# andi611/ZeroSpeech-TTS-without-T

Hardware: AMD Instinct MI355X
Metric: mel-frames/sec (train_ae, seg_len=128, enc_size=1024) (higher is better)
Workload: dtype bf16; 1 GPU; train_ae english hps seg_len=128 enc_size=1024 emb_size=1024 n_speakers=102 F=513, batch=256/GPU, dropout+Gumbel on, fwd+bwd+clip+Adam; global_batch=256, parallelism=dp1

## Files before the change

include/zs_amd.h:

```cpp
#ifndef ZS_AMD_H
#define ZS_AMD_H
#include <stddef.h>
#include <stdint.h>

#ifdef __cplusplus
extern "C" {
#endif

#define ZS_ABI_VERSION 1

enum { ZS_F32 = 0, ZS_BF16 = 1 };
enum { ZS_OK = 0, ZS_EINVAL = -1, ZS_ELAUNCH = -2, ZS_EWORKSPACE = -3 };
enum { ZS_PAD_ZERO = 0, ZS_PAD_REFLECT = 1 };
enum { ZS_ACT_NONE = 0, ZS_ACT_LRELU = 1, ZS_ACT_SIGMOID = 2, ZS_ACT_TANH = 3 };
enum { ZS_STORE_ROWS = 0, ZS_STORE_SPLIT2 = 1 };
enum { ZS_RES_NONE = 0, ZS_RES_IDENTITY = 1, ZS_RES_AVGPOOL2 = 2, ZS_RES_UPSAMPLE2 = 3 };

int zs_abi_version(void);
const char* zs_last_error(void);
int zs_set_option(const char* key, int value);
int zs_get_option(const char* key);

typedef struct {
  int32_t dtype;
  const void* A; int64_t lda; int64_t a_batch_stride;
  int32_t B, T_in, T_out;
  int32_t taps, stride, pad_left, pad_mode, gather;
  int32_t cin_pad;
  const void* W; int64_t ldw;
  int32_t N, n_pad;
  const float* bias;
  const float* pre_vec; int64_t pre_vec_ld; const int64_t* vec_idx;
  int32_t act; float slope;
  const void* dact_src; int64_t dact_ld;
  const void* add_src; int64_t add_ld; int32_t add_f32;
  void* out; int64_t ldc; int32_t out_f32; int32_t out_cols; int32_t store_mode;
  void* out2; int64_t ldc2; int32_t out2_cols; int32_t store_mode2;
  const float* vec2; int64_t vec2_ld;
  int32_t groups; int64_t a_gstride, w_gstride, out_gstride, bias_gstride;
  float* colsum; int64_t colsum_ld; int32_t colsum_col0;
  int32_t colsum_post;
  const int32_t* lengths; int32_t pad_right;
  int32_t w_in, w_out, taps_h;
} ZsGemmConv;
int zs_gemm_conv(const ZsGemmConv* p, void* stream);
enum { ZS_GEMM_PATH_P8 = 0, ZS_GEMM_PATH_RING_PP = 1, ZS_GEMM_PATH_RING = 2, ZS_GEMM_PATH_DMA64 = 3, ZS_GEMM_PATH_DMA128 = 4,
       ZS_GEMM_PATH_REG = 5 };
int zs_gemm_conv_path(const ZsGemmConv* p);

typedef struct {
  int32_t dtype;
  const void* dY; int64_t ldy; int32_t y_cols;
  const void* X; int64_t ldx; int64_t x_batch_stride; int32_t x_cols;
  int32_t B, T_in, T_out;
  int32_t taps, stride, pad_left, pad_mode;
  int32_t Cout, Cin;
  float* dW; int64_t so, si, sj;
  float* db;
  int32_t co_split2; int32_t accumulate;
  int32_t splits;
  void* workspace; size_t workspace_bytes;
  int32_t w_in, w_out, taps_h;
} ZsGemmWgrad;
size_t zs_gemm_wgrad_workspace_bytes(const ZsGemmWgrad* p);
int zs_gemm_wgrad(const ZsGemmWgrad* p, void* stream);
enum { ZS_WGRAD_PATH_P8 = 0, ZS_WGRAD_PATH_DMA = 1, ZS_WGRAD_PATH_REG = 2 };
int zs_gemm_wgrad_path(const ZsGemmWgrad* p, int32_t* splits, int32_t* rows_per_split);

typedef struct {
  int32_t dtype;
  const float* W; int64_t so, si, sj;
  int32_t Cout, Cin, taps;
  int32_t transpose, co_split2;
  int32_t inner_pad;
  void* dst; int64_t ldw;
  int32_t n_rows, n_cols, row_offset, col_offset;
  const int32_t* row_perm;
} ZsPackWeight;
int zs_pack_weight(const ZsPackWeight* p, void* stream);
int zs_pack_weight_batch(const ZsPackWeight* jobs, int32_t n, int32_t max_blocks, void* stream);

typedef struct {
  const float* src; float* dst;
  int32_t len, src_stride, dst_stride;
} ZsVecCopy;
int zs_copy_vec_batch(const ZsVecCopy* jobs, int32_t n, void* stream);

typedef struct {
  int32_t dtype;
  const void* src; int64_t ld_src; int32_t src_f32;
  void* dst; int64_t ld_dst; int32_t dst_f32; int32_t col_off;
  int64_t rows; int32_t cols, fill_cols;
  int32_t act; float slope;
  void* dst2; int64_t ld_dst2; int32_t col_off2, fill_cols2; int32_t act2; float slope2;
} ZsCastRows;
int zs_cast_rows(const ZsCastRows* p, void* stream);

typedef struct {
  int32_t dtype;
  const void* x; int64_t ldx;
  const float* vec; int64_t vec_ld; const int64_t* idx;
  void* out; int64_t ldo; int32_t B, T, C, fill_cols;
} ZsAddRowvec;
int zs_add_rowvec(const ZsAddRowvec* p, void* stream);

typedef struct {
  int32_t dtype;
  const void* x; int64_t ldx;
  void* out; int64_t ldo;
  void* out2; int64_t ldo2; const float* vec2; int64_t vec2_ld; int32_t vec2_cols; const int64_t* idx;
  float* mean; float* rstd;
  int32_t B, T, C; float eps;
  float drop_p; uint64_t seed; uint32_t stream_id; const uint8_t* mask; int64_t mask_ld;
  int32_t res_mode; const void* res; int64_t ldres; int32_t T_res; int32_t res_pad_mode;
  const uint64_t* seed_ptr;
  const int32_t* lengths; const int32_t* res_lengths;
  int32_t stats_given;
} ZsInstNormFwd;
int zs_instnorm_fwd(const ZsInstNormFwd* p, void* stream);

typedef struct {
  int32_t dtype;
  const void* dout; int64_t ldd;
  const void* x; int64_t ldx;
  const float* mean; const float* rstd;
  void* dz; int64_t ldz;
  int32_t B, T, C;
  float drop_p; uint64_t seed; uint32_t stream_id; const uint8_t* mask; int64_t mask_ld;
  float slope;
  const uint64_t* seed_ptr;
} ZsInstNormBwd;
int zs_instnorm_bwd(const ZsInstNormBwd* p, void* stream);

typedef struct {
  int32_t dtype;
  const void* gp; int64_t ldg; int32_t pad_left, pad_right, pad_mode;
  int32_t B, T, C;
  float* emb_sum; int64_t emb_ld; int32_t emb_cols;
  int32_t res_mode; const void* res; int64_t ldres;
  const void* dact_src; int64_t dact_ld; float slope;
  void* out; int64_t ldo; int32_t unshuffle;
} ZsGradCombine;
int zs_grad_combine(const ZsGradCombine* p, void* stream);
int zs_norm_decomposition(int32_t kernel, int32_t dtype, int32_t T, int32_t C);

typedef struct {
  const float* emb_sum; int64_t emb_ld; const int64_t* idx; int32_t B;
  float* demb; int64_t demb_ld; int32_t n_rows, C; int32_t accumulate;
} ZsEmbScatter;
int zs_emb_scatter(const ZsEmbScatter* p, void* stream);

typedef struct {
  int32_t dtype;
  const void* logits; int64_t ld; int32_t logits_f32;
  const float* noise; int32_t noise_kind; uint64_t seed;
  int64_t rows; int32_t E; float tau;
  void* bits; int64_t ld_bits; int32_t bits_fill_cols;
  float* bits_f32;
  float* y0;
  const uint64_t* seed_ptr;
} ZsMbvFwd;
int zs_mbv_fwd(const ZsMbvFwd* p, void* stream);
typedef struct {
  int32_t dtype;
  const void* dbits; int64_t ld_dbits;
  const float* y0; int64_t rows; int32_t E; float tau;
  void* dlogits; int64_t ld; int32_t fill_cols;
} ZsMbvBwd;
int zs_mbv_bwd(const ZsMbvBwd* p, void* stream);

enum { ZS_ENC_ONE_HOT = 0, ZS_ENC_BINARY = 1, ZS_ENC_CONTINUES = 2 };
typedef struct {
  int32_t dtype; int32_t mode;
  const void* logits; int64_t ld; int32_t logits_f32;
  const float* noise; int32_t noise_kind; uint64_t seed;
  int64_t rows; int32_t E; float tau; float slope;
  void* bits; int64_t ld_bits; int32_t bits_fill_cols;
  float* bits_f32;
  float* y;
  float* s;
  const uint64_t* seed_ptr;
} ZsGumbelStFwd;
int zs_gumbel_st_fwd(const ZsGumbelStFwd* p, void* stream);
typedef struct {
  int32_t dtype; int32_t mode;
  const void* dbits; int64_t ld_dbits;
  const float* y; int64_t ld_y;
  const float* s;
  int64_t rows; int32_t E; float tau; float slope;
  void* dlogits; int64_t ld; int32_t fill_cols;
} ZsGumbelStBwd;
int zs_gumbel_st_bwd(const ZsGumbelStBwd* p, void* stream);

typedef struct {
  int32_t dtype;
  int32_t B, T, H;
  const void* gi; int64_t ldgi;
  const void* whh; int64_t ldw; int32_t n_pad; int64_t w_gstride;
  const float* bhh; int64_t bhh_gstride;
  void* out; int64_t ldo; int32_t out_col;
  void* gates;
  float* work; size_t work_bytes;
  int32_t whh_interleaved;
  uint32_t* status;
  const float* bcast_vec; int64_t bcast_ld; const int64_t* bcast_idx; int32_t bcast_col;
  int32_t dir1_forward;
} ZsGruFwd;
size_t zs_gru_work_bytes(int32_t B, int32_t H);
int zs_gru_fwd(const ZsGruFwd* p, void* stream);
int zs_gru_check(const float* work, int32_t B, int32_t H, void* stream);

typedef struct {
  int32_t dtype;
  void* x; int64_t ld; int32_t col0, cols;
  int32_t B, T; const int32_t* lengths;
} ZsRowsReverse;
int zs_rows_reverse(const ZsRowsReverse* p, void* stream);
typedef struct {
  int32_t dtype;
  int32_t B, T, H;
  const void* dout; int64_t ldd; int32_t dout_col;
  const void* out; int64_t ldo; int32_t out_col;
  const void* gates;
  const void* whh_t; int64_t ldw; int32_t n_pad; int64_t w_gstride;
  void* dgi; int64_t ldgi;
  void* dgh; int64_t ldgh;
  float* work; size_t work_bytes;
  uint32_t* status;
} ZsGruBwd;
int zs_gru_bwd(const ZsGruBwd* p, void* stream);
enum { ZS_GRU_PATH_WIDE = 0, ZS_GRU_PATH_PERSIST = 1, ZS_GRU_PATH_STEP_FUSED = 2, ZS_GRU_PATH_STEP_GEMM = 3 };
int zs_gru_path(int32_t pass, int32_t dtype, int32_t B, int32_t T, int32_t H, int32_t whh_interleaved, int32_t wide_aligned);

typedef struct {
  int32_t dtype;
  const float* x_dec; int64_t ld_dec;
  const float* x; int64_t ldx;
  int64_t rows; int32_t F;
  void* dlogits; int64_t ldg; int32_t fill_cols;
  float* partial; float* loss_out; float grad_scale;
} ZsL1Loss;
int zs_l1_loss(const ZsL1Loss* p, void* stream);

int zs_sqnorm(const float* g, int64_t n, double* partial, float* out_sq, void* stream);

typedef struct {
  float* p; float* g; float* m; float* v; int64_t n;
  float lr, beta1, beta2, eps, bc1, bc2;
  const float* sumsq; float max_norm; int32_t write_clipped_grad;
  const int32_t* step_ptr;
  float grad_scale;
  int32_t max_blocks;
  float* ema;
  float ema_decay;
} ZsAdam;
int zs_adam_clip(const ZsAdam* p, void* stream);

int zs_sqnorm_stage1(const float* g, int64_t n, double* partial, void* stream);

enum { ZS_APJ_WEIGHT = 0, ZS_APJ_VECTOR = 1, ZS_APJ_RANGE = 2 };
typedef struct {
  void* dst; int64_t ldw; int64_t dst_elems;
  int32_t transpose, inner_pad, row_offset, col_offset, parity;
  int32_t vlen, src_offset, src_stride;
  const int32_t* row_inv;
} ZsAdamPackView;
typedef struct {
  int32_t kind, dtype;
  int64_t off, len;
  int32_t Cout, Cin, taps, co_split2;
  int32_t n_views, tile_start;
  ZsAdamPackView view[2];
} ZsAdamPackJob;
int zs_adam_pack_tiles(const ZsAdamPackJob* job);
int zs_adam_pack(const ZsAdam* a, const ZsAdamPackJob* jobs, const ZsAdamPackJob* jobs_dev, int32_t n, const double* sq_partial,
                 int32_t n_partial, void* stream);

int zs_host_fetch(const void* src, void* dst, size_t bytes, int32_t workgroups, void* stream);

typedef struct {
  const float* pool; const int32_t* speaker; const int64_t* first;
  int64_t* cursor;
  int64_t n; int32_t B, seg_len, F, rank, world;
  float* x; int64_t* c;
  int32_t advance;
} ZsPoolGather;
int zs_pool_gather(const ZsPoolGather* p, void* stream);

int zs_step_counters(uint64_t* seed, int32_t* step, void* stream);

typedef struct {
  const float* logits; int64_t ld; const int64_t* target; int32_t B, n_class;
  float* loss_out; float* dlogits; int64_t ldg; float grad_scale; int32_t* correct_out;
} ZsSoftmaxCE;
// ... 222 lines not shown
```

zerospeech-tts-without-t_amd/csrc/zs_gemm.hip:

```cpp
#include <stdlib.h>

#include <atomic>
#include <mutex>

#include "zs_common.h"

namespace {

constexpr int BM = 128, BN = 128, NT = 256;
constexpr int ROWB = 128;
constexpr int PITCH = 144;
constexpr int TILE_BYTES = BM * PITCH;

__device__ const uint4 zs_zero_line[8] = {};

__device__ __forceinline__ int xcd_remap(int bid, int nwg) {
  const int q = nwg >> 3, r = nwg & 7, xcd = bid & 7;
  return (xcd < r ? xcd * (q + 1) : r * (q + 1) + (xcd - r) * q) + (bid >> 3);
}

__device__ __forceinline__ int conv_src_row(int gather, int pad_mode, int stride, int pad_left, int T_in, int t,
                                            int j, bool& ok) {
  if (gather == 0) {
    int s = t * stride + j - pad_left;
    if (pad_mode == ZS_PAD_REFLECT) s = zs_reflect(s, T_in);
    ok = (s >= 0) && (s < T_in);
    return s;
  }
  int s = t - j;
  ok = false;
  if (s < 0) return 0;
  int q = s / stride;
  ok = (q * stride == s) && (q < T_in);
  return q;
}

struct Geom2 { int w_in, w_out, taps_h, h_in; unsigned mw, mt; };
__device__ __forceinline__ Geom2 make_geom2(int w_in, int w_out, int taps_h, int T_in) {
  Geom2 g;
  g.w_in = w_in; g.w_out = w_out; g.taps_h = taps_h;
  g.h_in = w_in > 0 ? T_in / w_in : 0;
  g.mw = w_in > 0 ? 0xffffffffu / (unsigned)w_out + 1u : 0u;
  g.mt = w_in > 0 ? 0xffffffffu / (unsigned)taps_h + 1u : 0u;
  return g;
}
__device__ __forceinline__ int conv_src_row_g(int gather, int pad_mode, int stride, int pad_left, int T_in, int t, int j, bool& ok,
                                              const Geom2& g) {
  if (g.w_in == 0) return conv_src_row(gather, pad_mode, stride, pad_left, T_in, t, j, ok);
  const int ho = g.w_out == 1 ? t : (int)__umulhi((unsigned)t, g.mw), wo = t - ho * g.w_out;
  const int kw = g.taps_h == 1 ? j : (int)__umulhi((unsigned)j, g.mt), kh = j - kw * g.taps_h;
  bool ok_h, ok_w;
  const int h = conv_src_row(gather, pad_mode, stride, pad_left, g.h_in, ho, kh, ok_h);
  const int w = conv_src_row(gather, pad_mode, stride, pad_left, g.w_in, wo, kw, ok_w);
  ok = ok_h && ok_w;
  return h * g.w_in + w;
}

__device__ __forceinline__ void conv_row_setup(const ZsGemmConv& p, int m, int M, int& rb, int& rt) {
  if (m >= M) { rb = -1; rt = 0; return; }
  const int b = m / p.T_out;
  rt = m - b * p.T_out;
  rb = b;
  if (p.lengths) {
    const int len = p.lengths[b];
    const int len_out = (len + p.pad_left + p.pad_right - p.taps) / p.stride + 1;
    rb = (rt < len_out) ? ((len << 16) | b) : -1;
  }
}
__device__ __forceinline__ int conv_row_b(const ZsGemmConv& p, int rb) { return p.lengths ? (rb & 0xffff) : rb; }
__device__ __forceinline__ int conv_row_tin(const ZsGemmConv& p, int rb) { return p.lengths ? (rb >> 16) : p.T_in; }

template <typename T> struct Mma;
template <> struct Mma<bf16_t> {
  static __device__ __forceinline__ void run(const uint4& a, const uint4& b, f32x16& c) {
    c = __builtin_amdgcn_mfma_f32_32x32x16_bf16(__builtin_bit_cast(bf16x8, a), __builtin_bit_cast(bf16x8, b), c, 0, 0, 0);
  }
};
template <> struct Mma<float> {
  static __device__ __forceinline__ void run(const uint4& a, const uint4& b, f32x16& c) {
    c = __builtin_amdgcn_mfma_f32_32x32x2f32(__uint_as_float(a.x), __uint_as_float(b.x), c, 0, 0, 0);
    c = __builtin_amdgcn_mfma_f32_32x32x2f32(__uint_as_float(a.y), __uint_as_float(b.y), c, 0, 0, 0);
    c = __builtin_amdgcn_mfma_f32_32x32x2f32(__uint_as_float(a.z), __uint_as_float(b.z), c, 0, 0, 0);
    c = __builtin_amdgcn_mfma_f32_32x32x2f32(__uint_as_float(a.w), __uint_as_float(b.w), c, 0, 0, 0);
  }
};

constexpr int CPITCH = 132;
constexpr int EPI_LDS_BYTES = BM * CPITCH * 4;

template <typename T, typename OT>
__device__ __forceinline__ void store_group(OT* base, int64_t row, int64_t ld, int col, int limit, bool aligned,
                                            const float (&v)[8]) {
  OT* d = base + row * ld + col;
  if (aligned && col + 8 <= limit) {
    store8<OT>(d, v);
  } else {
#pragma unroll
    for (int j = 0; j < 8; ++j)
      if (col + j < limit) Elem<OT>::st(d + j, v[j]);
  }
}

template <typename T, int NTHREADS, int ROWS = NTHREADS / 2>
__device__ __forceinline__ void epilogue_finish(const ZsGemmConv& p, const float* sC, int M, int m0, int n0, int tid, int g);

template <int NTHREADS, int ROWS = NTHREADS / 2>
__device__ __forceinline__ void epilogue_colsum(const ZsGemmConv& p, const float* sC, int M, int m0, int n0, int tid) {
  if (p.colsum == nullptr) return;
  const int ns = ROWS / p.T_out;
  for (int w = tid; w < ns * 128; w += NTHREADS) {
    const int col = w & 127, r0 = (w >> 7) * p.T_out;
    const int n = n0 + col, m = m0 + r0;
    if (n >= p.N || n < p.colsum_col0 || m >= M) continue;
    const float* q = sC + r0 * CPITCH + col;
    float a0 = 0.f, a1 = 0.f, a2 = 0.f, a3 = 0.f;
    int r = 0;
    if (p.colsum_post && (p.dact_src || p.add_src)) {
      for (; r < p.T_out; ++r) {
        float v = q[r * CPITCH];
        const int64_t mm = (int64_t)m + r;
        if (p.dact_src) v *= dlrelu_f(p.dtype == ZS_F32 ? ((const float*)p.dact_src)[mm * p.dact_ld + n] : bf2f(((const bf16_t*)p.dact_src)[mm * p.dact_ld + n]), p.slope);
        if (p.add_src) v += (p.add_f32 || p.dtype == ZS_F32) ? ((const float*)p.add_src)[mm * p.add_ld + n] : bf2f(((const bf16_t*)p.add_src)[mm * p.add_ld + n]);
        a0 += v;
      }
    }
    for (; r + 4 <= p.T_out; r += 4) {
      a0 += q[(r + 0) * CPITCH]; a1 += q[(r + 1) * CPITCH]; a2 += q[(r + 2) * CPITCH]; a3 += q[(r + 3) * CPITCH];
    }
    for (; r < p.T_out; ++r) a0 += q[r * CPITCH];
    p.colsum[(int64_t)(m / p.T_out) * p.colsum_ld + (n - p.colsum_col0)] += (a0 + a1) + (a2 + a3);
  }
}

template <typename T, int NTHREADS, int MI = 2>
__device__ __forceinline__ void gemm_epilogue(const ZsGemmConv& p, f32x16 (&acc)[MI][2], float* sC, int M, int m0, int n0,
                                              int wm, int wn, int tid, int g) {
  constexpr int ROWS = (NTHREADS / 2) * MI / 2;
  const int lane = tid & 63;
#pragma unroll
  for (int mi = 0; mi < MI; ++mi)
#pragma unroll
    for (int ni = 0; ni < 2; ++ni)
#pragma unroll
      for (int r = 0; r < 16; ++r) {
        const int row = wm * (32 * MI) + mi * 32 + (r & 3) + 8 * (r >> 2) + 4 * (lane >> 5);
        const int col = wn * 64 + ni * 32 + (lane & 31);
        sC[row * CPITCH + col] = acc[mi][ni][r];
      }
  __syncthreads();
  epilogue_colsum<NTHREADS, ROWS>(p, sC, M, m0, n0, tid);
  epilogue_finish<T, NTHREADS, ROWS>(p, sC, M, m0, n0, tid, g);
}

template <typename T, int NTHREADS, int ROWS>
__device__ __forceinline__ void epilogue_finish(const ZsGemmConv& p, const float* sC, int M, int m0, int n0, int tid, int g) {
  constexpr int ROWS_PER_PASS = NTHREADS / 16;
  constexpr int PASSES = ROWS / ROWS_PER_PASS;
  const int cg = tid & 15, rr0 = tid >> 4;
  const int n = n0 + cg * 8;
  if (n >= p.N && n >= p.out_cols && n >= p.out2_cols) return;
  const int half = p.N >> 1;
  const bool need_b = (p.pre_vec != nullptr) || (p.vec2 != nullptr);
  const int es = (int)sizeof(T);
  const bool al_out = p.out && ((((uintptr_t)p.out) | (uintptr_t)(p.ldc * (p.out_f32 ? 4 : es)) | (uintptr_t)(p.out_gstride * (p.out_f32 ? 4 : es))) & 15) == 0;
  const bool al_out2 = p.out2 && ((((uintptr_t)p.out2) | (uintptr_t)(p.ldc2 * es)) & 15) == 0;
  const bool al_dact = p.dact_src && ((((uintptr_t)p.dact_src) | (uintptr_t)(p.dact_ld * es)) & 15) == 0;
  const bool al_add = p.add_src && ((((uintptr_t)p.add_src) | (uintptr_t)(p.add_ld * (p.add_f32 ? 4 : es))) & 15) == 0;
  const bool split_ok = (half & 7) == 0;
  float bias[8];
#pragma unroll
  for (int j = 0; j < 8; ++j) bias[j] = (p.bias != nullptr && n + j < p.N) ? p.bias[(int64_t)g * p.bias_gstride + n + j] : 0.f;
  float* outf = (float*)p.out + (p.out_f32 ? (int64_t)g * p.out_gstride : 0);
  T* outt = (T*)p.out + (p.out_f32 ? 0 : (int64_t)g * p.out_gstride);

#pragma unroll 2
  for (int it = 0; it < PASSES; ++it) {
    const int row = rr0 + ROWS_PER_PASS * it;
    const int m = m0 + row;
    if (m >= M) break;
    float v[8];
    {
      const float4 x0 = *reinterpret_cast<const float4*>(sC + row * CPITCH + cg * 8);
      const float4 x1 = *reinterpret_cast<const float4*>(sC + row * CPITCH + cg * 8 + 4);
      v[0] = x0.x; v[1] = x0.y; v[2] = x0.z; v[3] = x0.w; v[4] = x1.x; v[5] = x1.y; v[6] = x1.z; v[7] = x1.w;
    }
    int b = 0;
    if (need_b) b = m / p.T_out;
#pragma unroll
    for (int j = 0; j < 8; ++j) v[j] += bias[j];
    if (p.pre_vec) {
      const float* pv = p.pre_vec + p.vec_idx[b] * p.pre_vec_ld + n;
#pragma unroll
      for (int j = 0; j < 8; ++j) if (n + j < p.N) v[j] += pv[j];
    }
    if (p.act == ZS_ACT_LRELU) {
#pragma unroll
      for (int j = 0; j < 8; ++j) v[j] = lrelu_f(v[j], p.slope);
    } else if (p.act == ZS_ACT_SIGMOID) {
#pragma unroll
      for (int j = 0; j < 8; ++j) v[j] = 1.f / (1.f + expf(-v[j]));
    } else if (p.act == ZS_ACT_TANH) {
#pragma unroll
      for (int j = 0; j < 8; ++j) v[j] = tanhf(v[j]);
    }
    if (p.dact_src) {
      const T* dp = (const T*)p.dact_src + (int64_t)m * p.dact_ld + n;
      float y[8];
      if (al_dact && n + 8 <= p.N) load8<T>(dp, y);
      else {
#pragma unroll
        for (int j = 0; j < 8; ++j) y[j] = (n + j < p.N) ? Elem<T>::ld(dp + j) : 0.f;
      }
#pragma unroll
      for (int j = 0; j < 8; ++j) v[j] *= dlrelu_f(y[j], p.slope);
    }
    if (p.add_src) {
      float y[8];
      if (p.add_f32) {
        const float* ap = (const float*)p.add_src + (int64_t)m * p.add_ld + n;
        if (al_add && n + 8 <= p.N) load8<float>(ap, y);
        else {
#pragma unroll
          for (int j = 0; j < 8; ++j) y[j] = (n + j < p.N) ? ap[j] : 0.f;
        }
      } else {
        const T* ap = (const T*)p.add_src + (int64_t)m * p.add_ld + n;
        if (al_add && n + 8 <= p.N) load8<T>(ap, y);
        else {
#pragma unroll
          for (int j = 0; j < 8; ++j) y[j] = (n + j < p.N) ? Elem<T>::ld(ap + j) : 0.f;
        }
      }
#pragma unroll
      for (int j = 0; j < 8; ++j) v[j] += y[j];
    }
#pragma unroll
    for (int j = 0; j < 8; ++j) if (n + j >= p.N) v[j] = 0.f;

    if (p.out) {
      if (p.store_mode == ZS_STORE_SPLIT2) {
        if (split_ok) {
          const int hi = n >= half;
          if (p.out_f32) store_group<T, float>(outf, 2 * (int64_t)m + hi, p.ldc, n - hi * half, half, al_out, v);
          else store_group<T, T>(outt, 2 * (int64_t)m + hi, p.ldc, n - hi * half, half, al_out, v);
        } else {
#pragma unroll
          for (int j = 0; j < 8; ++j)
            if (n + j < p.N) {
              const int hi = (n + j) >= half;
              const int64_t o = (2 * (int64_t)m + hi) * p.ldc + (n + j - hi * half);
              if (p.out_f32) outf[o] = v[j]; else Elem<T>::st(outt + o, v[j]);
            }
        }
      } else {
        if (p.out_f32) store_group<T, float>(outf, m, p.ldc, n, p.out_cols, al_out, v);
        else store_group<T, T>(outt, m, p.ldc, n, p.out_cols, al_out, v);
      }
    }
    if (p.out2) {
      const bool sp = p.store_mode2 == ZS_STORE_SPLIT2;
      if (sp && !split_ok) {
#pragma unroll
        for (int j = 0; j < 8; ++j)
          if (n + j < p.N) {
            const int hi = (n + j) >= half;
            const int oc = n + j - hi * half;
            float w = v[j];
            if (p.vec2) w += p.vec2[p.vec_idx[b] * p.vec2_ld + oc];
            Elem<T>::st((T*)p.out2 + (2 * (int64_t)m + hi) * p.ldc2 + oc, w);
          }
      } else {
        const int hi = sp ? (n >= half) : 0;
        const int oc = n - hi * half;
        const int64_t orow = sp ? (2 * (int64_t)m + hi) : (int64_t)m;
        const int limit = sp ? half : p.out2_cols;
        float w[8];
#pragma unroll
        for (int j = 0; j < 8; ++j) w[j] = v[j];
        if (p.vec2) {
          const float* pv = p.vec2 + p.vec_idx[b] * p.vec2_ld + oc;
#pragma unroll
          for (int j = 0; j < 8; ++j) if (n + j < p.N) w[j] += pv[j];
        }
        store_group<T, T>((T*)p.out2, orow, p.ldc2, oc, limit, al_out2, w);
      }
    }
  }
}

template <typename T>
__global__ __launch_bounds__(NT, 2) void gemm_conv_kernel(const ZsGemmConv p) {
  const Geom2 g2 = make_geom2(p.w_in, p.w_out, p.taps_h, p.T_in);
  constexpr int EPS = 16 / (int)sizeof(T);
  constexpr int KC = ROWB / (int)sizeof(T);
  extern __shared__ __attribute__((aligned(16))) unsigned char smem[];
  unsigned char* sA = smem;
  unsigned char* sB = smem + 2 * TILE_BYTES;

  const int tid = threadIdx.x, lane = tid & 63, wave = tid >> 6;
  const int wm = wave >> 1, wn = wave & 1;
  const int g = blockIdx.z;
  const T* __restrict__ A = (const T*)p.A + (int64_t)g * p.a_gstride;
  const T* __restrict__ W = (const T*)p.W + (int64_t)g * p.w_gstride;
  const int M = p.B * p.T_out;
  const int ntn = (p.N + BN - 1) / BN;
  const int ntm = (M + BM - 1) / BM;
  const int wg = xcd_remap(blockIdx.x, ntm * ntn);
  constexpr int GM = 8;
  const int per_group = GM * ntn;
  const int grp = wg / per_group;
  const int gm = min(GM, ntm - grp * GM);
  const int in_g = wg - grp * per_group;
  const int m0 = (grp * GM + in_g % gm) * BM, n0 = (in_g / gm) * BN;

  const int seg = tid & 7, r0 = tid >> 3;
  int rb[4], rt[4];
#pragma unroll
  for (int i = 0; i < 4; ++i) {
    int m = m0 + r0 + 32 * i;
    conv_row_setup(p, m, M, rb[i], rt[i]);
  }
  const int chunks_per_tap = p.cin_pad / KC;
  const T* zline = reinterpret_cast<const T*>(zs_zero_line) + seg * EPS;
  const T *pa0, *pa1, *pa2, *pa3;
  int inc0, inc1, inc2, inc3;
#define ZS_SET_TAP(i, ptr, inc)                                                                         \
  {                                                                                                     \
    bool ok = false; int srow = 0;                                                                      \
    if (rb[i] >= 0) srow = conv_src_row_g(p.gather, p.pad_mode, p.stride, p.pad_left, conv_row_tin(p, rb[i]), rt[i], tap, ok, g2); \
    ptr = ok ? (A + (int64_t)conv_row_b(p, rb[i]) * p.a_batch_stride + (int64_t)srow * p.lda + seg * EPS) : zline;       \
    inc = ok ? KC : 0;                                                                                  \
  }
  const T* pw0 = W + (int64_t)(n0 + r0) * p.ldw + seg * EPS;
  const int64_t wstep = (int64_t)32 * p.ldw;

  const int nk = p.taps * chunks_per_tap;
  uint4 Pa0, Pa1, Pa2, Pa3, Pb0, Pb1, Pb2, Pb3, Qa0, Qa1, Qa2, Qa3, Qb0, Qb1, Qb2, Qb3;
  int tap = 0, cit = 0;
  { ZS_SET_TAP(0, pa0, inc0) ZS_SET_TAP(1, pa1, inc1) ZS_SET_TAP(2, pa2, inc2) ZS_SET_TAP(3, pa3, inc3) }
  auto advance = [&]() {
    pw0 += KC;
    if (++cit == chunks_per_tap) {
      cit = 0; ++tap;
      if (tap < p.taps) { ZS_SET_TAP(0, pa0, inc0) ZS_SET_TAP(1, pa1, inc1) ZS_SET_TAP(2, pa2, inc2) ZS_SET_TAP(3, pa3, inc3) }
    } else {
      pa0 += inc0; pa1 += inc1; pa2 += inc2; pa3 += inc3;
    }
  };
#define ZS_GLOAD(S)                                                                                      \
  S##a0 = *reinterpret_cast<const uint4*>(pa0); S##a1 = *reinterpret_cast<const uint4*>(pa1);            \
  S##a2 = *reinterpret_cast<const uint4*>(pa2); S##a3 = *reinterpret_cast<const uint4*>(pa3);            \
  S##b0 = *reinterpret_cast<const uint4*>(pw0); S##b1 = *reinterpret_cast<const uint4*>(pw0 + wstep);    \
  S##b2 = *reinterpret_cast<const uint4*>(pw0 + 2 * wstep); S##b3 = *reinterpret_cast<const uint4*>(pw0 + 3 * wstep); \
  advance();
#define ZS_SWRITE(S, buf)                                                                                \
  {                                                                                                      \
// ... 287 lines not shown
      const int fly = (grp1 ? min(nk, 3) : min(nk, 2)) - 1;
      if (fly == 2) asm volatile("s_waitcnt vmcnt(12)" ::: "memory");
      else if (fly == 1) asm volatile("s_waitcnt vmcnt(6)" ::: "memory");
      else asm volatile("s_waitcnt vmcnt(0)" ::: "memory");
    }
    __builtin_amdgcn_s_barrier();
    if (grp1) __builtin_amdgcn_s_barrier();
    int stage = 0;
    for (int kt = 0; kt < nk; ++kt) {
      const unsigned sa = a_lane + (unsigned)(stage * RSTAGE), sb = b_lane + (unsigned)(stage * RSTAGE);
      u32x4_t fa[4][2], fb[4][2];
#pragma unroll
      for (int ks = 0; ks < 4; ++ks) {
        asm volatile("ds_read_b128 %0, %1" : "=v"(fa[ks][0]) : "v"(sa + koff[ks]));
        asm volatile("ds_read_b128 %0, %1 offset:4096" : "=v"(fa[ks][1]) : "v"(sa + koff[ks]));
        asm volatile("ds_read_b128 %0, %1" : "=v"(fb[ks][0]) : "v"(sb + koff[ks]));
        asm volatile("ds_read_b128 %0, %1 offset:4096" : "=v"(fb[ks][1]) : "v"(sb + koff[ks]));
      }
      int s2 = stage + 2; if (s2 >= 3) s2 -= 3;
      if (!grp1 && kt + 2 < nk) dma(s2);
      asm volatile("s_waitcnt lgkmcnt(0)" ::: "memory");
      if (grp1) {
        if (kt + 2 < nk) asm volatile("s_waitcnt vmcnt(6)" ::: "memory");
        else asm volatile("s_waitcnt vmcnt(0)" ::: "memory");
      }
      __builtin_amdgcn_s_barrier();
      __builtin_amdgcn_sched_barrier(0);
      const bool more1 = grp1 && (kt + 3 < nk);
      __builtin_amdgcn_s_setprio(1);
#pragma unroll
      for (int ks = 0; ks < 4; ++ks) {
#pragma unroll
        for (int mi = 0; mi < 2; ++mi)
#pragma unroll
          for (int ni = 0; ni < 2; ++ni) {
            const uint4 ua = make_uint4(fa[ks][mi].x, fa[ks][mi].y, fa[ks][mi].z, fa[ks][mi].w);
            const uint4 ub = make_uint4(fb[ks][ni].x, fb[ks][ni].y, fb[ks][ni].z, fb[ks][ni].w);
            Mma<T>::run(ua, ub, acc[mi][ni]);
          }
        if (more1 && ks < 3) {
          __builtin_amdgcn_sched_barrier(0);
          dma_piece(stage, 2 * ks);
          dma_piece(stage, 2 * ks + 1);
          __builtin_amdgcn_sched_barrier(0);
        }
      }
      __builtin_amdgcn_s_setprio(0);
      if (more1) dma_advance();
      if (!grp1) {
        if (kt + 2 < nk) asm volatile("s_waitcnt vmcnt(6)" ::: "memory");
        else asm volatile("s_waitcnt vmcnt(0)" ::: "memory");
      }
      __builtin_amdgcn_s_barrier();
      __builtin_amdgcn_sched_barrier(0);
      if (++stage == 3) stage = 0;
    }
    if (!grp1) __builtin_amdgcn_s_barrier();
  } else {
  dma(0);
  if (nk > 1) dma(1);
  int stage = 0;
  for (int kt = 0; kt < nk; ++kt) {
    if (kt + 1 < nk) asm volatile("s_waitcnt vmcnt(6)" ::: "memory");
    else asm volatile("s_waitcnt vmcnt(0)" ::: "memory");
    __builtin_amdgcn_s_barrier();
    const unsigned sa = a_lane + (unsigned)(stage * RSTAGE), sb = b_lane + (unsigned)(stage * RSTAGE);
    u32x4_t fa[4][2], fb[4][2];
#pragma unroll
    for (int ks = 0; ks < 4; ++ks) {
      asm volatile("ds_read_b128 %0, %1" : "=v"(fa[ks][0]) : "v"(sa + koff[ks]));
      asm volatile("ds_read_b128 %0, %1 offset:4096" : "=v"(fa[ks][1]) : "v"(sa + koff[ks]));
      asm volatile("ds_read_b128 %0, %1" : "=v"(fb[ks][0]) : "v"(sb + koff[ks]));
      asm volatile("ds_read_b128 %0, %1 offset:4096" : "=v"(fb[ks][1]) : "v"(sb + koff[ks]));
    }
    const bool more = kt + 2 < nk;
    int s2 = stage + 2; if (s2 >= 3) s2 -= 3;
    asm volatile("s_waitcnt lgkmcnt(0)" ::: "memory");
    __builtin_amdgcn_sched_barrier(0);
#pragma unroll
    for (int ks = 0; ks < 4; ++ks) {
#pragma unroll
      for (int mi = 0; mi < 2; ++mi)
#pragma unroll
        for (int ni = 0; ni < 2; ++ni) {
          const uint4 ua = make_uint4(fa[ks][mi].x, fa[ks][mi].y, fa[ks][mi].z, fa[ks][mi].w);
          const uint4 ub = make_uint4(fb[ks][ni].x, fb[ks][ni].y, fb[ks][ni].z, fb[ks][ni].w);
          Mma<T>::run(ua, ub, acc[mi][ni]);
        }
      if (more && ks < 3) {
        __builtin_amdgcn_sched_barrier(0);
        dma_piece(s2, 2 * ks);
        dma_piece(s2, 2 * ks + 1);
        __builtin_amdgcn_sched_barrier(0);
      }
    }
    if (more) dma_advance();
    __builtin_amdgcn_sched_barrier(0);
    if (++stage == 3) stage = 0;
  }
  }
  asm volatile("s_waitcnt vmcnt(0)" ::: "memory");
  __syncthreads();
  gemm_epilogue<T, RNT>(p, acc, reinterpret_cast<float*>(smem), M, m0, n0, wm, wn, tid, g);
}

constexpr int PBM = 256, PBN = 256, PNT = 512;
constexpr int PSTAGE = (PBM + PBN) * 128;
constexpr int P8_EPI = 256 * CPITCH * 4;
constexpr int P8_LDS = (2 * PSTAGE > P8_EPI) ? 2 * PSTAGE : P8_EPI;

#define ZS_DSR(dst, addr, off) asm volatile("ds_read_b128 %0, %1 offset:" #off : "=v"(dst) : "v"(addr))
#define ZS_P8_DMA(cond, src, dst)                                                \
  __builtin_amdgcn_sched_barrier(0);                                             \
  if (cond) __builtin_amdgcn_global_load_lds((gptr_t)(src), (lptr_t)(dst), 16, 0, 0); \
  __builtin_amdgcn_sched_barrier(0);
typedef __attribute__((ext_vector_type(4))) float f32x4_m;
template <typename T> struct Mma16;
template <> struct Mma16<bf16_t> {
  static __device__ __forceinline__ void run(const uint4& a, const uint4& b, f32x4_m& c) {
    c = __builtin_amdgcn_mfma_f32_16x16x32_bf16(__builtin_bit_cast(bf16x8, a), __builtin_bit_cast(bf16x8, b), c, 0, 0, 0);
  }
};
template <> struct Mma16<float> {
  static __device__ __forceinline__ void run(const uint4& a, const uint4& b, f32x4_m& c) {
    c = __builtin_amdgcn_mfma_f32_16x16x4f32(__uint_as_float(a.x), __uint_as_float(b.x), c, 0, 0, 0);
    c = __builtin_amdgcn_mfma_f32_16x16x4f32(__uint_as_float(a.y), __uint_as_float(b.y), c, 0, 0, 0);
    c = __builtin_amdgcn_mfma_f32_16x16x4f32(__uint_as_float(a.z), __uint_as_float(b.z), c, 0, 0, 0);
    c = __builtin_amdgcn_mfma_f32_16x16x4f32(__uint_as_float(a.w), __uint_as_float(b.w), c, 0, 0, 0);
  }
};
#define ZS_M16_READ_A(o0, o1, o2, o3)                                            \
  ZS_DSR(fa00, sa + koff0, o0); ZS_DSR(fa01, sa + koff1, o0); ZS_DSR(fa10, sa + koff0, o1); ZS_DSR(fa11, sa + koff1, o1); \
  ZS_DSR(fa20, sa + koff0, o2); ZS_DSR(fa21, sa + koff1, o2); ZS_DSR(fa30, sa + koff0, o3); ZS_DSR(fa31, sa + koff1, o3);
#define ZS_M16_READ_B(f0, f1, f2, f3, o0, o1)                                    \
  ZS_DSR(f0, sb + koff0, o0); ZS_DSR(f1, sb + koff1, o0); ZS_DSR(f2, sb + koff0, o1); ZS_DSR(f3, sb + koff1, o1);
#define ZS_M16_MMA(a, b, cc) Mma16<T>::run(make_uint4(a.x, a.y, a.z, a.w), make_uint4(b.x, b.y, b.z, b.w), cc)
#define ZS_M16_QUAD(cq, b0, b1, b2, b3, cond, src0, dst0, src1, dst1)            \
  __builtin_amdgcn_s_setprio(1);                                                 \
  ZS_M16_MMA(fa00, b0, cq[0][0]); ZS_M16_MMA(fa00, b2, cq[0][1]); ZS_M16_MMA(fa10, b0, cq[1][0]); ZS_M16_MMA(fa10, b2, cq[1][1]); \
  ZS_P8_DMA(cond, src0, dst0)                                                    \
  ZS_M16_MMA(fa20, b0, cq[2][0]); ZS_M16_MMA(fa20, b2, cq[2][1]); ZS_M16_MMA(fa30, b0, cq[3][0]); ZS_M16_MMA(fa30, b2, cq[3][1]); \
  ZS_M16_MMA(fa01, b1, cq[0][0]); ZS_M16_MMA(fa01, b3, cq[0][1]);                \
  ZS_P8_DMA(cond, src1, dst1)                                                    \
  ZS_M16_MMA(fa11, b1, cq[1][0]); ZS_M16_MMA(fa11, b3, cq[1][1]); ZS_M16_MMA(fa21, b1, cq[2][0]); ZS_M16_MMA(fa21, b3, cq[2][1]); \
  ZS_M16_MMA(fa31, b1, cq[3][0]); ZS_M16_MMA(fa31, b3, cq[3][1]);                \
  __builtin_amdgcn_s_setprio(0);

__host__ __device__ __forceinline__ bool al16(const void* q, int64_t pitch_bytes) { return ((((uintptr_t)q) | (uintptr_t)pitch_bytes) & 15) == 0; }

__host__ __device__ __forceinline__ bool p8_regs_epilogue_ok(const ZsGemmConv& p) {
  const int half = p.N >> 1;
  const bool split = (p.out && p.store_mode == ZS_STORE_SPLIT2) || (p.out2 && p.store_mode2 == ZS_STORE_SPLIT2);
  return (p.out == nullptr || (!p.out_f32 && al16(p.out, p.ldc * 2) && ((p.out_gstride * 2) & 15) == 0 && (p.out_cols & 7) == 0)) &&
         (p.out2 == nullptr || (al16(p.out2, p.ldc2 * 2) && (p.out2_cols & 7) == 0 && p.dact_src == nullptr && p.add_src == nullptr)) &&
         (p.dact_src == nullptr || al16(p.dact_src, p.dact_ld * 2)) &&
         (p.add_src == nullptr || (!p.add_f32 && al16(p.add_src, p.add_ld * 2))) &&
         ((p.pre_vec == nullptr && p.vec2 == nullptr) || (p.T_out & 15) == 0) && (!split || (half & 7) == 0) &&
         (p.act == ZS_ACT_NONE || p.act == ZS_ACT_LRELU) &&
         (p.colsum == nullptr || ((PBM % p.T_out) == 0 && p.out2 == nullptr));
}

template <bool HAS2>
__device__ __forceinline__ void p8_regs_epilogue(const ZsGemmConv& p, f32x4_m (&c)[2][2][4][2], unsigned char* smem, int M, int m0, int n0,
                                                 int tid, int lane, int wr, int wc, int g) {
  constexpr int PT = 264;
  unsigned short* sT = reinterpret_cast<unsigned short*>(smem);
  const int colb = wc * 64 + (lane & 15);
  const int rbase = wr * 128 + 4 * (lane >> 4);
  const int half = p.N >> 1;
  int64_t bsel[2][4];
  const bool need_b = p.pre_vec != nullptr || p.vec2 != nullptr;
#pragma unroll
  for (int mq = 0; mq < 2; ++mq)
#pragma unroll
    for (int mt = 0; mt < 4; ++mt) {
      const int mb = m0 + wr * 128 + mq * 64 + mt * 16;
      bsel[mq][mt] = (need_b && mb < M) ? p.vec_idx[mb / p.T_out] : 0;
    }
#pragma unroll
  for (int nq = 0; nq < 2; ++nq)
#pragma unroll
    for (int nt = 0; nt < 2; ++nt) {
      const int col = colb + nq * 32 + nt * 16;
      const int n = n0 + col;
      const bool cval = n < p.N;
      const float bv = (p.bias != nullptr && cval) ? p.bias[(int64_t)g * p.bias_gstride + n] : 0.f;
      float pv[2][4];
#pragma unroll
      for (int mq = 0; mq < 2; ++mq)
#pragma unroll
        for (int mt = 0; mt < 4; ++mt) pv[mq][mt] = bv;
      if (p.pre_vec != nullptr && cval) {
#pragma unroll
        for (int mq = 0; mq < 2; ++mq)
#pragma unroll
          for (int mt = 0; mt < 4; ++mt) pv[mq][mt] += p.pre_vec[bsel[mq][mt] * p.pre_vec_ld + n];
      }
#pragma unroll
      for (int mq = 0; mq < 2; ++mq)
#pragma unroll
        for (int mt = 0; mt < 4; ++mt)
#pragma unroll
          for (int i4 = 0; i4 < 4; ++i4) {
            float v = c[mq][nq][mt][nt][i4] + pv[mq][mt];
            if (p.act == ZS_ACT_LRELU) v = lrelu_f(v, p.slope);
            if (!cval) v = 0.f;
            if constexpr (HAS2) c[mq][nq][mt][nt][i4] = v;
            sT[(rbase + mq * 64 + mt * 16 + i4) * PT + col] = f2bf(v);
          }
    }
  __syncthreads();

  const bool cs_post = !HAS2 && p.colsum != nullptr && p.colsum_post && (p.dact_src != nullptr || p.add_src != nullptr);
  auto colsum_pass = [&]() {
    const int ns = PBM / p.T_out;
    const int col = tid & 255, n = n0 + col, hs = tid >> 8;
    const int s0 = ns >= 2 ? hs * (ns >> 1) : 0, s1 = ns >= 2 ? s0 + (ns >> 1) : (hs == 0 ? 1 : 0);
    if (n < p.N && n >= p.colsum_col0) {
      for (int s = s0; s < s1; ++s) {
        const int r0 = s * p.T_out, m = m0 + r0;
        if (m >= M) break;
        float a0 = 0.f, a1 = 0.f, a2 = 0.f, a3 = 0.f;
        const unsigned short* q = sT + r0 * PT + col;
        int r = 0;
        for (; r + 4 <= p.T_out; r += 4) {
          a0 += bf2f(q[(r + 0) * PT]); a1 += bf2f(q[(r + 1) * PT]); a2 += bf2f(q[(r + 2) * PT]); a3 += bf2f(q[(r + 3) * PT]);
        }
        for (; r < p.T_out; ++r) a0 += bf2f(q[r * PT]);
        float* d = p.colsum + (int64_t)(m / p.T_out) * p.colsum_ld + (n - p.colsum_col0);
        *d += (a0 + a1) + (a2 + a3);
      }
    }
  };
  if (!HAS2 && p.colsum != nullptr && !cs_post) colsum_pass();

  const int c8 = (tid & 31) * 8, r0 = tid >> 5;
  const int n = n0 + c8;
  if (p.out != nullptr) {
    unsigned short* outp = (unsigned short*)p.out + (int64_t)g * p.out_gstride;
    const bool sp = p.store_mode == ZS_STORE_SPLIT2;
    const int hi = sp ? (n >= half) : 0;
    const int oc = n - hi * half;
    const bool cok = sp ? (n < p.N) : (n < p.out_cols);
    const bool second = p.dact_src != nullptr || p.add_src != nullptr;
    if (cok && !second) {
#pragma unroll 8
      for (int it = 0; it < 16; ++it) {
        const int row = r0 + 16 * it;
        const int m = m0 + row;
        if (m < M) {
          const uint4 w = *reinterpret_cast<const uint4*>(sT + row * PT + c8);
          const int64_t orow = sp ? 2 * (int64_t)m + hi : (int64_t)m;
          *reinterpret_cast<uint4*>(outp + orow * p.ldc + oc) = w;
        }
      }
    } else if (!HAS2 && cok) {
      const bf16_t* dsrc = (const bf16_t*)p.dact_src;
      const bf16_t* asrc = (const bf16_t*)p.add_src;
      const bool tail = n + 8 > p.N;
#pragma unroll 1
      for (int it0 = 0; it0 < 16; it0 += 8) {
        Raw8<bf16_t> rd[8], ra[8];
        uint4 w[8];
#pragma unroll
        for (int u = 0; u < 8; ++u) {
          const int row = r0 + 16 * (it0 + u);
          const int m = min(m0 + row, M - 1);
          if (dsrc) rd[u].ld(dsrc + (int64_t)m * p.dact_ld + n);
          if (asrc) ra[u].ld(asrc + (int64_t)m * p.add_ld + n);
          w[u] = *reinterpret_cast<const uint4*>(sT + row * PT + c8);
        }
#pragma unroll
        for (int u = 0; u < 8; ++u) {
          const int row = r0 + 16 * (it0 + u);
          const int m = m0 + row;
          if (m < M) {
            float v[8], y[8];
            Raw8<bf16_t> rw; rw.a = w[u]; rw.cvt(v);
            if (dsrc) {
              rd[u].cvt(y);
#pragma unroll
              for (int j = 0; j < 8; ++j) v[j] *= dlrelu_f(y[j], p.slope);
            }
            if (asrc) {
              ra[u].cvt(y);
#pragma unroll
              for (int j = 0; j < 8; ++j) v[j] += y[j];
            }
            if (tail) {
#pragma unroll
              for (int j = 0; j < 8; ++j) if (n + j >= p.N) v[j] = 0.f;
            }
            const int64_t orow = sp ? 2 * (int64_t)m + hi : (int64_t)m;
            store8<bf16_t>(outp + orow * p.ldc + oc, v);
            if (cs_post) store8<bf16_t>(sT + row * PT + c8, v);
          }
        }
      }
    }
  }
  if (cs_post) {
    __syncthreads();
    colsum_pass();
  }
  if constexpr (HAS2) {
    __syncthreads();
    const bool sp = p.store_mode2 == ZS_STORE_SPLIT2;
#pragma unroll
    for (int nq = 0; nq < 2; ++nq)
#pragma unroll
      for (int nt = 0; nt < 2; ++nt) {
        const int col = colb + nq * 32 + nt * 16;
        const int nn = n0 + col;
        const bool cval = nn < p.N;
        const int ocv = sp ? (nn >= half ? nn - half : nn) : nn;
        float ev[2][4];
#pragma unroll
        for (int mq = 0; mq < 2; ++mq)
#pragma unroll
          for (int mt = 0; mt < 4; ++mt) ev[mq][mt] = 0.f;
        if (p.vec2 != nullptr && cval) {
#pragma unroll
          for (int mq = 0; mq < 2; ++mq)
#pragma unroll
            for (int mt = 0; mt < 4; ++mt) ev[mq][mt] = p.vec2[bsel[mq][mt] * p.vec2_ld + ocv];
        }
#pragma unroll
        for (int mq = 0; mq < 2; ++mq)
#pragma unroll
          for (int mt = 0; mt < 4; ++mt)
#pragma unroll
            for (int i4 = 0; i4 < 4; ++i4)
              sT[(rbase + mq * 64 + mt * 16 + i4) * PT + col] = f2bf(c[mq][nq][mt][nt][i4] + ev[mq][mt]);
      }
    __syncthreads();
    unsigned short* outp = (unsigned short*)p.out2;
    const int hi = sp ? (n >= half) : 0;
    const int oc = n - hi * half;
    const bool cok = sp ? (n < p.N) : (n < p.out2_cols);
    if (cok) {
#pragma unroll 8
      for (int it = 0; it < 16; ++it) {
        const int row = r0 + 16 * it;
        const int m = m0 + row;
        if (m < M) {
          const uint4 w = *reinterpret_cast<const uint4*>(sT + row * PT + c8);
          const int64_t orow = sp ? 2 * (int64_t)m + hi : (int64_t)m;
          *reinterpret_cast<uint4*>(outp + orow * p.ldc2 + oc) = w;
        }
      }
    }
  }
}

template <typename T>
__global__ __launch_bounds__(PNT, 2) void gemm_conv_p8m16_kernel(const ZsGemmConv p) {
  const Geom2 g2 = make_geom2(p.w_in, p.w_out, p.taps_h, p.T_in);
  constexpr int EPS = 16 / (int)sizeof(T);
  constexpr int KC = ROWB / (int)sizeof(T);
  extern __shared__ __attribute__((aligned(16))) unsigned char smem[];
  typedef __attribute__((address_space(1))) const void* gptr_t;
  typedef __attribute__((address_space(3))) void* lptr_t;
  const int tid = threadIdx.x, lane = tid & 63, wave = __builtin_amdgcn_readfirstlane(tid >> 6);
  const int wr = wave >> 2, wc = wave & 3;
  const int g = blockIdx.z;
  const T* __restrict__ A = (const T*)p.A + (int64_t)g * p.a_gstride;
  const T* __restrict__ W = (const T*)p.W + (int64_t)g * p.w_gstride;
  const int M = p.B * p.T_out;
  const int ntn = (p.N + PBN - 1) / PBN;
  const int ntm = (M + PBM - 1) / PBM;
  const int wg = xcd_remap(blockIdx.x, ntm * ntn);
  constexpr int GM = 4;
  const int per_group = GM * ntn;
  const int grp = wg / per_group;
  const int gm = min(GM, ntm - grp * GM);
  const int in_g = wg - grp * per_group;
  const int m0 = (grp * GM + in_g % gm) * PBM, n0 = (in_g / gm) * PBN;

  const int lrow = lane >> 3, slot = lane & 7;
  int rb[4], rt[4], lseg[4];
#pragma unroll
  for (int j = 0; j < 4; ++j) {
    const int r = (j >> 1) * 128 + wave * 16 + (j & 1) * 8 + lrow;
    lseg[j] = slot ^ ((r >> 1) & 7);
    const int m = m0 + r;
    conv_row_setup(p, m, M, rb[j], rt[j]);
  }
  const int chunks_per_tap = p.cin_pad / KC;
  const T* zline = reinterpret_cast<const T*>(zs_zero_line);
  const T *pa0, *pa1, *pa2, *pa3;
  int inc0, inc1, inc2, inc3;
#define ZS_SET_TAP(i, ptr, inc)                                                                         \
  {                                                                                                     \
    bool ok = false; int srow = 0;                                                                      \
    if (rb[i] >= 0) srow = conv_src_row_g(p.gather, p.pad_mode, p.stride, p.pad_left, conv_row_tin(p, rb[i]), rt[i], tap, ok, g2); \
    ptr = ok ? (A + (int64_t)conv_row_b(p, rb[i]) * p.a_batch_stride + (int64_t)srow * p.lda + lseg[i] * EPS) : (zline + lseg[i] * EPS); \
    inc = ok ? KC : 0;                                                                                  \
  }
  const int nk = p.taps * chunks_per_tap;
  int tap = 0, cit = 0;
  { ZS_SET_TAP(0, pa0, inc0) ZS_SET_TAP(1, pa1, inc1) ZS_SET_TAP(2, pa2, inc2) ZS_SET_TAP(3, pa3, inc3) }
  auto advance_a = [&]() {
    if (++cit == chunks_per_tap) {
      cit = 0; ++tap;
      if (tap < p.taps) { ZS_SET_TAP(0, pa0, inc0) ZS_SET_TAP(1, pa1, inc1) ZS_SET_TAP(2, pa2, inc2) ZS_SET_TAP(3, pa3, inc3) }
    } else {
      pa0 += inc0; pa1 += inc1; pa2 += inc2; pa3 += inc3;
    }
  };
#undef ZS_SET_TAP
  const T* pw0 = W + (int64_t)(n0 + wave * 16 + lrow) * p.ldw + lseg[0] * EPS;
  const T* pw1 = W + (int64_t)(n0 + wave * 16 + 8 + lrow) * p.ldw + lseg[1] * EPS;
  const int64_t whalf = (int64_t)128 * p.ldw;

  unsigned char* const ldsA = smem + wave * 2048;
  unsigned char* const ldsB = smem + 32768 + wave * 2048;

  f32x4_m c[2][2][4][2];
#pragma unroll
  for (int i0 = 0; i0 < 2; ++i0)
#pragma unroll
    for (int i1 = 0; i1 < 2; ++i1)
#pragma unroll
      for (int i2 = 0; i2 < 4; ++i2)
#pragma unroll
        for (int i3 = 0; i3 < 2; ++i3) c[i0][i1][i2][i3] = f32x4_m{0.f, 0.f, 0.f, 0.f};

  const int frow = lane & 15, fh = lane >> 4, fx = (frow >> 1) & 7;
  const unsigned lds0 = (unsigned)(uintptr_t)(__attribute__((address_space(3))) unsigned char*)smem;
  const unsigned a_lane = lds0 + (unsigned)((wr * 128 + frow) * 128);
  const unsigned b_lane = lds0 + (unsigned)(32768 + (wc * 64 + frow) * 128);
  const unsigned koff0 = (unsigned)(((0 + fh) ^ fx) * 16), koff1 = (unsigned)(((4 + fh) ^ fx) * 16);
  const int grp1 = wr;

  __builtin_amdgcn_global_load_lds((gptr_t)pa0, (lptr_t)(ldsA), 16, 0, 0);
  __builtin_amdgcn_global_load_lds((gptr_t)pa1, (lptr_t)(ldsA + 1024), 16, 0, 0);
  __builtin_amdgcn_global_load_lds((gptr_t)pa2, (lptr_t)(ldsA + 16384), 16, 0, 0);
  __builtin_amdgcn_global_load_lds((gptr_t)pa3, (lptr_t)(ldsA + 16384 + 1024), 16, 0, 0);
  advance_a();
  __builtin_amdgcn_global_load_lds((gptr_t)pw0, (lptr_t)(ldsB), 16, 0, 0);
  __builtin_amdgcn_global_load_lds((gptr_t)pw1, (lptr_t)(ldsB + 1024), 16, 0, 0);
  __builtin_amdgcn_global_load_lds((gptr_t)(pw0 + whalf), (lptr_t)(ldsB + 16384), 16, 0, 0);
  __builtin_amdgcn_global_load_lds((gptr_t)(pw1 + whalf), (lptr_t)(ldsB + 16384 + 1024), 16, 0, 0);
  pw0 += KC; pw1 += KC;
  if (nk > 1) {
    __builtin_amdgcn_global_load_lds((gptr_t)pw0, (lptr_t)(ldsB + PSTAGE), 16, 0, 0);
    __builtin_amdgcn_global_load_lds((gptr_t)pw1, (lptr_t)(ldsB + PSTAGE + 1024), 16, 0, 0);
    __builtin_amdgcn_global_load_lds((gptr_t)(pw0 + whalf), (lptr_t)(ldsB + PSTAGE + 16384), 16, 0, 0);
    __builtin_amdgcn_global_load_lds((gptr_t)(pw1 + whalf), (lptr_t)(ldsB + PSTAGE + 16384 + 1024), 16, 0, 0);
    pw0 += KC; pw1 += KC;
    asm volatile("s_waitcnt vmcnt(4)" ::: "memory");
  } else {
    asm volatile("s_waitcnt vmcnt(0)" ::: "memory");
  }
  __builtin_amdgcn_s_barrier();
  if (grp1) __builtin_amdgcn_s_barrier();

  u32x4_t fa00, fa01, fa10, fa11, fa20, fa21, fa30, fa31;
  u32x4_t fb00, fb01, fb02, fb03, fb10, fb11, fb12, fb13;
// ... 824 lines not shown
  for (int e = 0; e < 4; ++e) {
    const int ci = c4 * 4 + e;
    if (ci < p.Cin) {
      float* q = d + (int64_t)ci * p.si;
      *q = p.accumulate ? (*q + r[e]) : r[e];
    }
  }
}

constexpr int WRT_LDS_FLOATS = 1024;

__global__ __launch_bounds__(256) void wgrad_reduce_taps_kernel(const ZsGemmWgrad p, int splits, int cout_r, int cin_r, int c4n,
                                                                int nblk, int nmain) {
  __shared__ float sT[WRT_LDS_FLOATS];
  const int64_t sstride = (int64_t)cout_r * p.taps * cin_r;
  if ((int)blockIdx.x >= nmain) { wgrad_reduce_bias(p, splits, cout_r, sstride, (int)blockIdx.x - nmain); return; }
  const int co = (int)blockIdx.x / nblk, blk = (int)blockIdx.x - co * nblk;
  const int ci0 = blk * 4 * c4n;
  const int taps = p.taps;
  const float* wrow = (const float*)p.workspace + (int64_t)wgrad_co_perm(p, co) * taps * cin_r + ci0;
  for (int it = (int)threadIdx.x; it < c4n * taps; it += 256) {
    const int j = it / c4n, c = it - j * c4n;
    if (ci0 + 4 * c >= p.Cin) continue;
    const float4 acc = wgrad_sum_splits(wrow + (int64_t)j * cin_r + 4 * c, splits, sstride);
    sT[(4 * c + 0) * taps + j] = acc.x; sT[(4 * c + 1) * taps + j] = acc.y;
    sT[(4 * c + 2) * taps + j] = acc.z; sT[(4 * c + 3) * taps + j] = acc.w;
  }
  __syncthreads();
  const int n = min(4 * c4n, p.Cin - ci0) * taps;
  float* d = p.dW + (int64_t)co * p.so + (int64_t)ci0 * taps;
  for (int i = (int)threadIdx.x; i < n; i += 256) d[i] = p.accumulate ? (d[i] + sT[i]) : sT[i];
}

Knob g_dma64("gemm_dma64", "ZS_GEMM_DMA64", 1);
Knob g_dma64_max_tiles("gemm_dma64_max_tiles", "ZS_GEMM_DMA64_MAX_TILES", 256);
Knob g_wgrad_p8("wgrad_p8", "ZS_WGRAD_P8", 1);
Knob g_wgrad_wgs("wgrad_wgs", "ZS_WGRAD_WGS", 256);
Knob g_wgrad_wgs128("wgrad_wgs128", "ZS_WGRAD_WGS128", 448);
Knob g_wgrad_slab_cost("wgrad_slab_cost", "ZS_WGRAD_SLAB_COST", 13);
Knob g_wgrad_alone("wgrad_alone", "ZS_WGRAD_ALONE", 0);
Knob g_wgrad_wgs128_alone("wgrad_wgs128_alone", "ZS_WGRAD_WGS128_ALONE", 448);
Knob g_wgrad_slab_cost_alone("wgrad_slab_cost_alone", "ZS_WGRAD_SLAB_COST_ALONE", 13);
Knob g_wgrad_dma("wgrad_dma", "ZS_WGRAD_DMA", 1);
Knob g_wgrad_reduce_taps("wgrad_reduce_taps", "ZS_WGRAD_REDUCE_TAPS", 1);
Knob g_wgrad_waste("wgrad_p8_waste", "ZS_WGRAD_P8_WASTE", 135);

struct WgradPlan { int p8, dma, splits, tile, co_tiles, ci_tiles, cout_r, cin_r, rows_per_split; };

WgradPlan wgrad_plan(const ZsGemmWgrad* p) {
  WgradPlan w;
  const int wgrad_p8 = g_wgrad_p8.get();
  const bool alone = g_wgrad_alone.get() != 0;
  const int64_t M = (int64_t)p->B * p->T_out;
  const int64_t t256 = (int64_t)((p->Cout + 255) / 256) * p->taps * ((p->Cin + 255) / 256);
  const double waste = (double)(((p->Cout + 255) / 256) * 256) * (((p->Cin + 255) / 256) * 256) / ((double)p->Cout * p->Cin);
  w.p8 = wgrad_p8 && p->dtype == ZS_BF16 && waste <= 0.01 * (double)g_wgrad_waste.get() && M >= 2048 && (wgrad_p8 > 1 || t256 * M >= (int64_t)16 * 8192);
  if (wgrad_p8 > 1 && p->dtype == ZS_BF16) w.p8 = 1;
  w.dma = !w.p8 && p->dtype == ZS_BF16 && g_wgrad_dma.get() != 0;
  w.tile = w.p8 ? 256 : 128;
  w.co_tiles = (p->Cout + w.tile - 1) / w.tile; w.ci_tiles = (p->Cin + w.tile - 1) / w.tile;
  w.cout_r = w.co_tiles * w.tile; w.cin_r = w.ci_tiles * w.tile;
  const int64_t tiles = (int64_t)w.co_tiles * p->taps * w.ci_tiles;
  if (p->splits > 0) {
    w.splits = p->splits;
  } else if (w.p8) {
    const int64_t kt = (M + 63) / 64;
    const int wgs_knob = g_wgrad_wgs.get();
    const int64_t wgs = wgs_knob > 0 ? wgs_knob : 256;
    const double slab_cost = (double)(alone ? g_wgrad_slab_cost_alone.get() : g_wgrad_slab_cost.get());
    double best = 1e30; int bs = 1;
    for (int sp = 1; sp <= 64 && (int64_t)sp * 4 <= kt; ++sp) {
      const double rounds = (double)((tiles * sp + wgs - 1) / wgs);
      const double cost = rounds * ((double)((kt + sp - 1) / sp) + slab_cost);
      if (cost < best - 1e-9) { best = cost; bs = sp; }
    }
    w.splits = bs;
  } else {
    const int knob = alone ? g_wgrad_wgs128_alone.get() : g_wgrad_wgs128.get();
    const int64_t target = knob > 0 ? knob : 448;
    int64_t sp = (target + tiles - 1) / tiles;
    int64_t maxs = (M + 255) / 256;
    if (sp > maxs) sp = maxs;
    if (sp > 1024) sp = 1024;
    if (sp < 1) sp = 1;
    w.splits = (int)sp;
  }
  const int gran = w.p8 ? 64 : WK;
  int rps = (int)((M + w.splits - 1) / w.splits);
  w.rows_per_split = ((rps + gran - 1) / gran) * gran;
  return w;
}

bool aligned16(const void* p) { return (((uintptr_t)p) & 15) == 0; }

Knob g_use_dma("gemm_dma", "ZS_GEMM_DMA", 1), g_use_ring("gemm_ring", "ZS_GEMM_RING", 1),
    g_ring_min_tiles("gemm_ring_min_tiles", "ZS_GEMM_RING_MIN_TILES", 256), g_use_pp("gemm_pp", "ZS_GEMM_PP", 1), g_use_p8("gemm_p8", "ZS_GEMM_P8", 1),
    g_p8_min_tiles("gemm_p8_min_tiles", "ZS_GEMM_P8_MIN_TILES", 200);

std::once_flag g_lds_attr_once;
void set_lds_attrs() {
  const void* big[] = {reinterpret_cast<const void*>(gemm_conv_p8m16_kernel<float>), reinterpret_cast<const void*>(gemm_conv_p8m16_kernel<bf16_t>),
                       reinterpret_cast<const void*>(gemm_wgrad_p8_kernel)};
  for (const void* f : big) (void)hipFuncSetAttribute(f, hipFuncAttributeMaxDynamicSharedMemorySize, P8_LDS);
  const void* ring[] = {reinterpret_cast<const void*>(gemm_conv_ring_kernel<float, 0>), reinterpret_cast<const void*>(gemm_conv_ring_kernel<bf16_t, 0>),
                        reinterpret_cast<const void*>(gemm_conv_ring_kernel<float, 1>), reinterpret_cast<const void*>(gemm_conv_ring_kernel<bf16_t, 1>)};
  for (const void* f : ring) (void)hipFuncSetAttribute(f, hipFuncAttributeMaxDynamicSharedMemorySize, RING_LDS);
}

struct ConvPlan {
  int path;
  int regs;
  int64_t wgs;
  int groups;
};
int gemm_conv_plan(const ZsGemmConv* p, ConvPlan& pl) {
  ZS_REQUIRE(p && p->A && p->W && (p->out || p->out2), "zs_gemm_conv: null operand");
  ZS_REQUIRE(p->dtype == ZS_F32 || p->dtype == ZS_BF16, "zs_gemm_conv: bad dtype %d", p->dtype);
  const int es = p->dtype == ZS_F32 ? 4 : 2;
  const int kc = 128 / es;
  ZS_REQUIRE(p->B > 0 && p->T_in > 0 && p->T_out > 0 && p->N > 0 && p->taps > 0 && p->stride > 0, "zs_gemm_conv: bad sizes");
  ZS_REQUIRE(p->cin_pad > 0 && p->cin_pad % kc == 0, "zs_gemm_conv: cin_pad %d must be a multiple of %d (one 128-byte chunk)", p->cin_pad, kc);
  ZS_REQUIRE(p->ldw >= (int64_t)p->taps * p->cin_pad && (p->ldw * es) % 16 == 0, "zs_gemm_conv: ldw %lld < taps*cin_pad",
             (long long)p->ldw);
  ZS_REQUIRE(p->n_pad % 128 == 0 && p->n_pad >= p->N, "zs_gemm_conv: n_pad %d must be a multiple of 128 >= N %d", p->n_pad, p->N);
  ZS_REQUIRE(aligned16(p->A) && aligned16(p->W) && (p->lda * es) % 16 == 0 && (p->a_batch_stride * es) % 16 == 0 &&
                 (p->a_gstride * es) % 16 == 0 && (p->w_gstride * es) % 16 == 0,
             "zs_gemm_conv: operands must be 16-byte aligned (A=%p lda=%lld)", p->A, (long long)p->lda);
  if (p->w_in > 0) {
    ZS_REQUIRE((int64_t)p->T_out * p->w_out < (1ll << 32), "zs_gemm_conv: 2-D image too large (T_out %d x w_out %d)", p->T_out, p->w_out);
    ZS_REQUIRE(p->w_out > 0 && p->taps_h > 0 && p->taps % p->taps_h == 0 && p->T_in % p->w_in == 0 && p->T_out % p->w_out == 0 && !p->lengths,
               "zs_gemm_conv: 2-D geometry (w_in %d, w_out %d, taps_h %d, taps %d, T_in %d, T_out %d)", p->w_in, p->w_out, p->taps_h, p->taps,
               p->T_in, p->T_out);
    if (p->gather == 0 && p->pad_mode == ZS_PAD_REFLECT) {
      const int h_in = p->T_in / p->w_in, h_out = p->T_out / p->w_out, taps_w = p->taps / p->taps_h;
      const int pr_h = (h_out - 1) * p->stride + p->taps_h - 1 - p->pad_left - (h_in - 1);
      const int pr_w = (p->w_out - 1) * p->stride + taps_w - 1 - p->pad_left - (p->w_in - 1);
      ZS_REQUIRE(p->pad_left < h_in && pr_h < h_in && p->pad_left < p->w_in && pr_w < p->w_in,
                 "zs_gemm_conv: Padding size should be less than the corresponding input dimension (2-D: pad %d, H %d, W %d)", p->pad_left, h_in, p->w_in);
    }
  } else if (p->gather == 0 && p->pad_mode == ZS_PAD_REFLECT) {
    const int pad_r = (p->T_out - 1) * p->stride + p->taps - 1 - p->pad_left - (p->T_in - 1);
    ZS_REQUIRE(p->pad_left < p->T_in && pad_r < p->T_in,
               "zs_gemm_conv: Padding size should be less than the corresponding input dimension (pad %d/%d, T %d)",
               p->pad_left, pad_r, p->T_in);
  }
  if (p->store_mode == ZS_STORE_SPLIT2 || (p->out2 && p->store_mode2 == ZS_STORE_SPLIT2))
    ZS_REQUIRE(p->N % 2 == 0, "zs_gemm_conv: SPLIT2 needs even N");
  ZS_REQUIRE(!(p->pre_vec || p->vec2) || p->vec_idx, "zs_gemm_conv: vec_idx missing");
  ZS_REQUIRE(!p->colsum || (128 % p->T_out == 0 && p->colsum_col0 >= 0 && p->colsum_col0 < p->N && !p->bias && !p->pre_vec &&
                            p->act == ZS_ACT_NONE && p->groups <= 1),
             "zs_gemm_conv: colsum needs T_out (%d) to divide 128, 0 <= colsum_col0 < N and no bias / pre_vec / activation / groups", p->T_out);
  ZS_REQUIRE(!p->lengths || (p->gather == 0 && p->B < 65536 && p->T_in < 32768 && p->pad_right >= 0 && p->colsum == nullptr),
             "zs_gemm_conv: lengths (ragged batch) needs gather 0, B < 65536, T_in < 32768, pad_right >= 0 and no colsum");
  pl.groups = p->groups > 0 ? p->groups : 1;
  pl.regs = 0;
  const int64_t M = (int64_t)p->B * p->T_out;
  const int64_t ntn = (p->N + BN - 1) / BN;
  const int64_t tiles = ((M + BM - 1) / BM) * ntn;
  ZS_REQUIRE(tiles < (1ll << 31), "zs_gemm_conv: grid too large");
  const int use_dma = g_use_dma.get(), use_ring = g_use_ring.get(), use_p8 = g_use_p8.get(), use_pp = g_use_pp.get();
  const int64_t ring_tiles = ((M + RBM - 1) / RBM) * ntn;
  const int64_t p8_tiles = ((M + PBM - 1) / PBM) * ((p->N + PBN - 1) / PBN);
  const int64_t tiles64 = ((M + 63) / 64) * ntn;
  if (use_dma && use_p8 && p->n_pad % PBN == 0 && p8_tiles >= g_p8_min_tiles.get() && p8_tiles < (1ll << 31)) {
    pl.path = ZS_GEMM_PATH_P8; pl.wgs = p8_tiles;
    pl.regs = p->dtype == ZS_BF16 && p8_regs_epilogue_ok(*p);
  } else if (use_dma && use_ring && ring_tiles >= g_ring_min_tiles.get() && ring_tiles < (1ll << 31)) {
    pl.path = use_pp ? ZS_GEMM_PATH_RING_PP : ZS_GEMM_PATH_RING; pl.wgs = ring_tiles;
  } else if (use_dma && g_dma64.get() && tiles * 2 <= g_dma64_max_tiles.get() && tiles64 < (1ll << 31) &&
             (p->colsum == nullptr || 64 % p->T_out == 0)) {
    pl.path = ZS_GEMM_PATH_DMA64; pl.wgs = tiles64;
  } else {
    pl.path = use_dma ? ZS_GEMM_PATH_DMA128 : ZS_GEMM_PATH_REG; pl.wgs = tiles;
  }
  return ZS_OK;
}

struct WgradLaunch {
  WgradPlan w;
  int kernel;
  int reduce_taps;
  int64_t wgs;
  int c4n, nblk;
  int nmain, nbias;
};
int gemm_wgrad_plan(const ZsGemmWgrad* p, WgradLaunch& pl) {
  ZS_REQUIRE(p && p->dY && p->X && p->dW && p->workspace, "zs_gemm_wgrad: null operand");
  ZS_REQUIRE(aligned16(p->workspace), "zs_gemm_wgrad: workspace must be 16-byte aligned");
  ZS_REQUIRE(p->dtype == ZS_F32 || p->dtype == ZS_BF16, "zs_gemm_wgrad: bad dtype");
  const int es = p->dtype == ZS_F32 ? 4 : 2;
  ZS_REQUIRE(p->B > 0 && p->T_in > 0 && p->T_out > 0 && p->Cout > 0 && p->Cin > 0 && p->taps > 0 && p->stride > 0,
             "zs_gemm_wgrad: bad sizes");
  ZS_REQUIRE(aligned16(p->dY) && aligned16(p->X) && (p->ldy * es) % 16 == 0 && (p->ldx * es) % 16 == 0 &&
                 (p->x_batch_stride * es) % 16 == 0 && (p->y_cols * es) % 16 == 0 && (p->x_cols * es) % 16 == 0,
             "zs_gemm_wgrad: operands must be 16-byte aligned");
  ZS_REQUIRE(p->y_cols <= p->ldy && p->x_cols <= p->ldx && p->Cout <= p->y_cols && p->Cin <= p->x_cols, "zs_gemm_wgrad: column bounds");
  ZS_REQUIRE(!p->co_split2 || p->Cout % 2 == 0, "zs_gemm_wgrad: SPLIT2 needs even Cout");
  ZS_REQUIRE(p->w_in == 0 || (p->w_in > 0 && p->w_out > 0 && p->taps_h > 0 && p->taps % p->taps_h == 0 && p->T_in % p->w_in == 0 &&
                              p->T_out % p->w_out == 0 && (int64_t)p->T_out * p->w_out < (1ll << 32)),
             "zs_gemm_wgrad: 2-D geometry (w_in %d, w_out %d, taps_h %d, taps %d, T_in %d, T_out %d)", p->w_in, p->w_out, p->taps_h, p->taps,
             p->T_in, p->T_out);
  pl.w = wgrad_plan(p);
  const WgradPlan& w = pl.w;
  pl.kernel = w.p8 ? ZS_WGRAD_PATH_P8 : (w.dma ? ZS_WGRAD_PATH_DMA : ZS_WGRAD_PATH_REG);
  pl.wgs = (int64_t)w.co_tiles * p->taps * w.ci_tiles * w.splits;
  ZS_REQUIRE(pl.wgs < (1ll << 31), "zs_gemm_wgrad: grid too large");
  pl.nbias = p->db ? (p->Cout + 255) / 256 : 0;
  pl.reduce_taps = g_wgrad_reduce_taps.get() && p->taps > 1 && p->taps <= 256 && p->si == p->taps && p->sj == 1;
  pl.c4n = pl.nblk = 0;
  if (pl.reduce_taps) {
    pl.c4n = 256 / p->taps;
    pl.nblk = (p->Cin + 4 * pl.c4n - 1) / (4 * pl.c4n);
    ZS_REQUIRE((int64_t)p->Cout * pl.nblk + pl.nbias < (1ll << 31), "zs_gemm_wgrad: reduce grid too large");
    pl.nmain = p->Cout * pl.nblk;
  } else {
    const int64_t relems = (int64_t)p->Cout * p->taps * ((p->Cin + 3) / 4);
    const int64_t nmain = (relems + 255) / 256;
    ZS_REQUIRE(nmain + pl.nbias < (1ll << 31), "zs_gemm_wgrad: reduce grid too large");
    pl.nmain = (int)nmain;
  }
  return ZS_OK;
}

}

extern "C" int zs_gemm_conv_path(const ZsGemmConv* p) {
  ConvPlan pl;
  const int rc = gemm_conv_plan(p, pl);
  return rc != ZS_OK ? rc : (pl.path | pl.regs << 8);
}

extern "C" int zs_gemm_conv(const ZsGemmConv* p, void* stream) {
  ConvPlan pl;
  const int rc = gemm_conv_plan(p, pl);
  if (rc != ZS_OK) return rc;
  const dim3 grid((unsigned)pl.wgs, 1, (unsigned)pl.groups);
  const bool f32 = p->dtype == ZS_F32;
  hipStream_t s = (hipStream_t)stream;
  std::call_once(g_lds_attr_once, set_lds_attrs);
  switch (pl.path) {
    case ZS_GEMM_PATH_P8:
      if (f32) hipLaunchKernelGGL(gemm_conv_p8m16_kernel<float>, grid, dim3(PNT), P8_LDS, s, *p);
      else hipLaunchKernelGGL(gemm_conv_p8m16_kernel<bf16_t>, grid, dim3(PNT), P8_LDS, s, *p);
      break;
    case ZS_GEMM_PATH_RING_PP:
      if (f32) hipLaunchKernelGGL((gemm_conv_ring_kernel<float, 1>), grid, dim3(RNT), RING_LDS, s, *p);
      else hipLaunchKernelGGL((gemm_conv_ring_kernel<bf16_t, 1>), grid, dim3(RNT), RING_LDS, s, *p);
      break;
    case ZS_GEMM_PATH_RING:
      if (f32) hipLaunchKernelGGL((gemm_conv_ring_kernel<float, 0>), grid, dim3(RNT), RING_LDS, s, *p);
      else hipLaunchKernelGGL((gemm_conv_ring_kernel<bf16_t, 0>), grid, dim3(RNT), RING_LDS, s, *p);
      break;
    case ZS_GEMM_PATH_DMA64: {
      const size_t lds = (2 * 64 * 128 + 2 * DTILE > EPI_LDS_BYTES / 2) ? 2 * 64 * 128 + 2 * DTILE : EPI_LDS_BYTES / 2;
      if (f32) hipLaunchKernelGGL((gemm_conv_dma_kernel<float, 64>), grid, dim3(NT), lds, s, *p);
      else hipLaunchKernelGGL((gemm_conv_dma_kernel<bf16_t, 64>), grid, dim3(NT), lds, s, *p);
      break;
    }
    case ZS_GEMM_PATH_DMA128: {
      const size_t lds = (4 * DTILE > EPI_LDS_BYTES) ? 4 * DTILE : EPI_LDS_BYTES;
      if (f32) hipLaunchKernelGGL((gemm_conv_dma_kernel<float, 128>), grid, dim3(NT), lds, s, *p);
      else hipLaunchKernelGGL((gemm_conv_dma_kernel<bf16_t, 128>), grid, dim3(NT), lds, s, *p);
      break;
    }
    default: {
      const size_t lds = 4 * TILE_BYTES;
      if (f32) hipLaunchKernelGGL(gemm_conv_kernel<float>, grid, dim3(NT), lds, s, *p);
      else hipLaunchKernelGGL(gemm_conv_kernel<bf16_t>, grid, dim3(NT), lds, s, *p);
    }
  }
  return zs_check_launch("zs_gemm_conv");
}

extern "C" size_t zs_gemm_wgrad_workspace_bytes(const ZsGemmWgrad* p) {
  if (!p) return 0;
  const WgradPlan w = wgrad_plan(p);
  return (size_t)w.splits * ((size_t)w.cout_r * p->taps * w.cin_r + w.cout_r) * sizeof(float);
}

extern "C" int zs_gemm_wgrad_path(const ZsGemmWgrad* p, int32_t* splits, int32_t* rows_per_split) {
  WgradLaunch pl;
  const int rc = gemm_wgrad_plan(p, pl);
  if (rc != ZS_OK) return rc;
  if (splits) *splits = pl.w.splits;
  if (rows_per_split) *rows_per_split = pl.w.rows_per_split;
  return pl.kernel | pl.reduce_taps << 8;
}

extern "C" int zs_gemm_wgrad(const ZsGemmWgrad* p, void* stream) {
  WgradLaunch pl;
  int rc = gemm_wgrad_plan(p, pl);
  if (rc != ZS_OK) return rc;
  const WgradPlan& w = pl.w;
  const int splits = w.splits, ci_tiles = w.ci_tiles, cout_r = w.cout_r, cin_r = w.cin_r;
  const int rows_per_split = w.rows_per_split;
  const size_t need = (size_t)splits * ((size_t)cout_r * p->taps * cin_r + cout_r) * sizeof(float);
  if (p->workspace_bytes < need) {
    zs_set_error("zs_gemm_wgrad: workspace %zu < %zu bytes", p->workspace_bytes, need);
    return ZS_EWORKSPACE;
  }
  hipStream_t s = (hipStream_t)stream;
  const dim3 grid((unsigned)pl.wgs, 1, 1);
  std::call_once(g_lds_attr_once, set_lds_attrs);
  if (pl.kernel == ZS_WGRAD_PATH_P8) {
    hipLaunchKernelGGL(gemm_wgrad_p8_kernel, grid, dim3(PNT), P8_LDS, s, *p, ci_tiles, rows_per_split, cout_r, cin_r);
  } else if (p->dtype == ZS_F32) {
// ... 30 lines not shown
```

zerospeech-tts-without-t_amd/csrc/zs_norm.hip:

```cpp
#include <stdlib.h>

#include "zs_common.h"

namespace {

constexpr int RPT = 8;
struct Narrow { static constexpr int NTN = 256, CHUNK = 64, RG = 32; };
struct Wide8 { static constexpr int NTN = 256, CHUNK = 256, RG = 8; };
constexpr int RGN = 32;

template <typename S>
__device__ __forceinline__ void colreduce(const float (&pv)[RGN / S::RG][8], float (&out)[8], float* red, float* tot, int cg, int rg, int tid) {
  constexpr int CHUNK = S::CHUNK, RG = S::RG, NP = RGN / RG;
#pragma unroll
  for (int j = 0; j < NP; ++j)
#pragma unroll
    for (int k = 0; k < 8; ++k) red[(rg + RG * j) * CHUNK + cg * 8 + k] = pv[j][k];
  __syncthreads();
  for (int c = tid; c < CHUNK; c += S::NTN) {
    float s = 0.f;
#pragma unroll 8
    for (int r = 0; r < RGN; ++r) s += red[r * CHUNK + c];
    tot[c] = s;
  }
// ... 141 lines not shown
    }
  }
}

template <typename T, typename S>
__global__ __launch_bounds__(S::NTN) void instnorm_bwd_kernel(const ZsInstNormBwd p) {
  constexpr int CHUNK = S::CHUNK, RG = S::RG, CGN = S::CHUNK / 8, NP = RGN / RG;
  __shared__ float red[RGN * CHUNK];
  __shared__ float tot[CHUNK];
  const int tid = threadIdx.x, cg = tid % CGN, rg = tid / CGN;
  const int b = blockIdx.y, c0 = blockIdx.x * CHUNK + cg * 8;
  const bool cvalid = c0 < p.C;
  float mean[8], rstd[8];
#pragma unroll
  for (int k = 0; k < 8; ++k) {
    mean[k] = cvalid ? p.mean[(int64_t)b * p.C + c0 + k] : 0.f;
    rstd[k] = cvalid ? p.rstd[(int64_t)b * p.C + c0 + k] : 0.f;
  }
  const float inv_keep = p.drop_p > 0.f ? 1.f / (1.f - p.drop_p) : 1.f;
  const uint64_t seed = p.seed + (p.seed_ptr ? *p.seed_ptr : 0ull);
  Raw8<T> g[RPT], xv[RPT];
  float pg[NP][8], pgx[NP][8], sg[8], sgx[8];
#pragma unroll
  for (int j = 0; j < NP; ++j)
#pragma unroll
    for (int k = 0; k < 8; ++k) { pg[j][k] = 0.f; pgx[j][k] = 0.f; }
#pragma unroll
  for (int i = 0; i < RPT; ++i) {
    const int t = rg + RG * i;
    g[i].zero(); xv[i].zero();
    if (cvalid && t < p.T) {
      const int64_t row = (int64_t)b * p.T + t;
      g[i].ld((const T*)p.dout + row * p.ldd + c0);
      xv[i].ld((const T*)p.x + row * p.ldx + c0);
    }
  }
#pragma unroll
  for (int i = 0; i < RPT; ++i) {
    const int t = rg + RG * i;
    if (cvalid && t < p.T) {
      const int64_t row = (int64_t)b * p.T + t;
      float gf[8], xf[8];
      g[i].cvt(gf); xv[i].cvt(xf);
#pragma unroll
      for (int k = 0; k < 8; ++k) {
        gf[k] *= keep_scale(p.mask, p.mask_ld, p.drop_p, seed, p.stream_id, row, c0 + k, p.C, inv_keep);
        const float xh = (xf[k] - mean[k]) * rstd[k];
        pg[i % NP][k] += gf[k]; pgx[i % NP][k] += gf[k] * xh;
      }
    }
  }
  colreduce<S>(pg, sg, red, tot, cg, rg, tid);
  colreduce<S>(pgx, sgx, red, tot, cg, rg, tid);
  if (!cvalid) return;
  const float invT = 1.f / (float)p.T;
#pragma unroll
  for (int i = 0; i < RPT; ++i) {
    const int t = rg + RG * i;
    if (t >= p.T) continue;
    const int64_t row = (int64_t)b * p.T + t;
    float o[8], gf[8], xf[8];
    g[i].cvt(gf); xv[i].cvt(xf);
#pragma unroll
    for (int k = 0; k < 8; ++k) {
      gf[k] *= keep_scale(p.mask, p.mask_ld, p.drop_p, seed, p.stream_id, row, c0 + k, p.C, inv_keep);
      const float xh = (xf[k] - mean[k]) * rstd[k];
      const float dx = rstd[k] * (gf[k] - sg[k] * invT - xh * (sgx[k] * invT));
      o[k] = dx * dlrelu_f(xf[k], p.slope);
    }
    store8<T>((T*)p.dz + row * p.ldz + c0, o);
  }
}

template <typename T, typename S>
__global__ __launch_bounds__(S::NTN) void grad_combine_kernel(const ZsGradCombine p) {
  constexpr int CHUNK = S::CHUNK, RG = S::RG, CGN = S::CHUNK / 8, NP = RGN / RG;
  __shared__ float red[RGN * CHUNK];
  __shared__ float tot[CHUNK];
  const int tid = threadIdx.x, cg = tid % CGN, rg = tid / CGN;
  const int b = blockIdx.y, c0 = blockIdx.x * CHUNK + cg * 8;
  const bool cvalid = c0 < p.C;
  const int Tp = p.T + p.pad_left + p.pad_right;
  const T* gp = (const T*)p.gp;
  float v[RPT][8];
  float ps[NP][8], s[8];
#pragma unroll
  for (int j = 0; j < NP; ++j)
#pragma unroll
    for (int k = 0; k < 8; ++k) ps[j][k] = 0.f;
#pragma unroll
  for (int i = 0; i < RPT; ++i) {
    const int t = rg + RG * i;
#pragma unroll
    for (int k = 0; k < 8; ++k) v[i][k] = 0.f;
    if (cvalid && t < p.T) {
      const T* base = gp + (int64_t)b * Tp * p.ldg + c0;
      load8<T>(base + (int64_t)(t + p.pad_left) * p.ldg, v[i]);
      if (p.pad_mode == ZS_PAD_REFLECT) {
        if (t >= 1 && t <= p.pad_left) {
          float r[8]; load8<T>(base + (int64_t)(p.pad_left - t) * p.ldg, r);
#pragma unroll
          for (int k = 0; k < 8; ++k) v[i][k] += r[k];
        }
        if (t <= p.T - 2 && t >= p.T - 1 - p.pad_right) {
          float r[8]; load8<T>(base + (int64_t)(p.pad_left + 2 * (p.T - 1) - t) * p.ldg, r);
#pragma unroll
          for (int k = 0; k < 8; ++k) v[i][k] += r[k];
        }
      }
#pragma unroll
      for (int k = 0; k < 8; ++k) ps[i % NP][k] += v[i][k];
    }
  }
  if (p.emb_sum) {
    colreduce<S>(ps, s, red, tot, cg, rg, tid);
    if (cvalid && rg == 0) {
#pragma unroll
      for (int k = 0; k < 8; ++k)
        if (c0 + k < p.emb_cols) p.emb_sum[(int64_t)b * p.emb_ld + c0 + k] += s[k];
    }
  }
  if (!cvalid || p.out == nullptr) return;
  const T* res = (const T*)p.res;
  const T* da = (const T*)p.dact_src;
#pragma unroll
  for (int i = 0; i < RPT; ++i) {
    const int t = rg + RG * i;
    if (t >= p.T) continue;
    float o[8];
#pragma unroll
    for (int k = 0; k < 8; ++k) o[k] = v[i][k];
    if (p.res_mode == ZS_RES_IDENTITY) {
      float r[8]; load8<T>(res + ((int64_t)b * p.T + t) * p.ldres + c0, r);
#pragma unroll
      for (int k = 0; k < 8; ++k) o[k] += r[k];
    } else if (p.res_mode == ZS_RES_AVGPOOL2) {
      float r[8]; load8<T>(res + ((int64_t)b * (p.T >> 1) + (t >> 1)) * p.ldres + c0, r);
#pragma unroll
      for (int k = 0; k < 8; ++k) o[k] += 0.5f * r[k];
    } else if (p.res_mode == ZS_RES_UPSAMPLE2) {
      float r0[8], r1[8];
      load8<T>(res + ((int64_t)b * 2 * p.T + 2 * t) * p.ldres + c0, r0);
      load8<T>(res + ((int64_t)b * 2 * p.T + 2 * t + 1) * p.ldres + c0, r1);
#pragma unroll
      for (int k = 0; k < 8; ++k) o[k] += r0[k] + r1[k];
    }
    int64_t orow = (int64_t)b * p.T + t; int ocol = c0;
    if (p.unshuffle) { orow = (int64_t)b * (p.T >> 1) + (t >> 1); ocol = (t & 1) * p.C + c0; }
    if (da) {
      float y[8]; load8<T>(da + orow * p.dact_ld + ocol, y);
#pragma unroll
      for (int k = 0; k < 8; ++k) o[k] *= dlrelu_f(y[k], p.slope);
    }
    store8<T>((T*)p.out + orow * p.ldo + ocol, o);
  }
}

bool al16(const void* p) { return (((uintptr_t)p) & 15) == 0; }

Knob g_norm_wide("norm_wide", nullptr, 1, knob_flag);
Knob g_norm_lim0("norm_lim0", nullptr, 64, knob_raw), g_norm_lim1("norm_lim1", nullptr, 32, knob_raw), g_norm_lim2("norm_lim2", nullptr, 64, knob_raw);
bool norm_wide(int dtype, int T, int C, int max_T) {
  return g_norm_wide.get() != 0 && dtype == ZS_BF16 && T <= max_T && T <= Wide8::RG * RPT && C >= Wide8::CHUNK;
}

#define ZS_NORM_LAUNCH(KERNEL, MAXT)                                                                                        \
  do {                                                                                                                      \
    if (norm_wide(p->dtype, p->T, p->C, MAXT)) {                                                                            \
      dim3 grid((p->C + Wide8::CHUNK - 1) / Wide8::CHUNK, p->B);                                                            \
      hipLaunchKernelGGL((KERNEL<bf16_t, Wide8>), grid, dim3(Wide8::NTN), 0, (hipStream_t)stream, *p);                      \
    } else {                                                                                                                \
      dim3 grid((p->C + Narrow::CHUNK - 1) / Narrow::CHUNK, p->B);                                                          \
      if (p->dtype == ZS_F32) hipLaunchKernelGGL((KERNEL<float, Narrow>), grid, dim3(Narrow::NTN), 0, (hipStream_t)stream, *p); \
      else hipLaunchKernelGGL((KERNEL<bf16_t, Narrow>), grid, dim3(Narrow::NTN), 0, (hipStream_t)stream, *p);                \
    }                                                                                                                       \
  } while (0)

}

extern "C" int zs_instnorm_fwd(const ZsInstNormFwd* p, void* stream) {
  ZS_REQUIRE(p && p->x && p->out, "zs_instnorm_fwd: null operand");
  ZS_REQUIRE(!p->stats_given || (p->mean && p->rstd), "zs_instnorm_fwd: stats_given needs mean and rstd");
  ZS_REQUIRE(p->dtype == ZS_F32 || p->dtype == ZS_BF16, "zs_instnorm_fwd: bad dtype");
  const int es = p->dtype == ZS_F32 ? 4 : 2;
  ZS_REQUIRE(p->B > 0 && p->T > 0 && p->T <= Narrow::RG * RPT && p->C > 0 && p->C % 8 == 0, "zs_instnorm_fwd: need 0<T<=256 (T=%d), C%%8==0 (C=%d)", p->T, p->C);
  ZS_REQUIRE(al16(p->x) && al16(p->out) && (p->ldx * es) % 16 == 0 && (p->ldo * es) % 16 == 0, "zs_instnorm_fwd: alignment");
  ZS_REQUIRE(!p->out2 || (al16(p->out2) && (p->ldo2 * es) % 16 == 0 && (!p->vec2 || p->idx)), "zs_instnorm_fwd: out2");
  ZS_REQUIRE((p->mean == nullptr) == (p->rstd == nullptr), "zs_instnorm_fwd: mean/rstd");
  if (p->res_mode != ZS_RES_NONE) {
    ZS_REQUIRE(p->res && al16(p->res) && (p->ldres * es) % 16 == 0, "zs_instnorm_fwd: residual");
    if (p->res_mode == ZS_RES_UPSAMPLE2) ZS_REQUIRE(p->T_res * 2 == p->T, "zs_instnorm_fwd: upsample T_res %d vs T %d", p->T_res, p->T);
    if (p->res_mode == ZS_RES_AVGPOOL2) ZS_REQUIRE((p->T_res + 1) / 2 == p->T && p->T_res >= 2, "zs_instnorm_fwd: avgpool T_res %d vs T %d", p->T_res, p->T);
  }
  ZS_REQUIRE(p->drop_p >= 0.f && p->drop_p < 1.f, "zs_instnorm_fwd: drop_p");
  ZS_NORM_LAUNCH(instnorm_fwd_kernel, g_norm_lim0.get());
  return zs_check_launch("zs_instnorm_fwd");
}

extern "C" int zs_instnorm_bwd(const ZsInstNormBwd* p, void* stream) {
  ZS_REQUIRE(p && p->dout && p->x && p->mean && p->rstd && p->dz, "zs_instnorm_bwd: null operand");
  ZS_REQUIRE(p->dtype == ZS_F32 || p->dtype == ZS_BF16, "zs_instnorm_bwd: bad dtype");
  const int es = p->dtype == ZS_F32 ? 4 : 2;
  ZS_REQUIRE(p->B > 0 && p->T > 0 && p->T <= Narrow::RG * RPT && p->C > 0 && p->C % 8 == 0, "zs_instnorm_bwd: sizes");
  ZS_REQUIRE(al16(p->dout) && al16(p->x) && al16(p->dz) && (p->ldd * es) % 16 == 0 && (p->ldx * es) % 16 == 0 && (p->ldz * es) % 16 == 0,
             "zs_instnorm_bwd: alignment");
  ZS_NORM_LAUNCH(instnorm_bwd_kernel, g_norm_lim1.get());
  return zs_check_launch("zs_instnorm_bwd");
}

extern "C" int zs_grad_combine(const ZsGradCombine* p, void* stream) {
  ZS_REQUIRE(p && p->gp && (p->out || p->emb_sum), "zs_grad_combine: null operand");
  ZS_REQUIRE(p->dtype == ZS_F32 || p->dtype == ZS_BF16, "zs_grad_combine: bad dtype");
  const int es = p->dtype == ZS_F32 ? 4 : 2;
  ZS_REQUIRE(p->B > 0 && p->T > 0 && p->T <= Narrow::RG * RPT && p->C > 0 && p->C % 8 == 0, "zs_grad_combine: sizes T=%d C=%d", p->T, p->C);
  ZS_REQUIRE(p->pad_left >= 0 && p->pad_right >= 0 && (p->pad_mode != ZS_PAD_REFLECT || (p->pad_left < p->T && p->pad_right < p->T)),
             "zs_grad_combine: pads");
  ZS_REQUIRE(al16(p->gp) && (p->ldg * es) % 16 == 0 && (!p->out || (al16(p->out) && (p->ldo * es) % 16 == 0)), "zs_grad_combine: alignment");
  if (p->res_mode != ZS_RES_NONE) {
    ZS_REQUIRE(p->res && al16(p->res) && (p->ldres * es) % 16 == 0, "zs_grad_combine: residual");
    ZS_REQUIRE(p->res_mode != ZS_RES_AVGPOOL2 || p->T % 2 == 0, "zs_grad_combine: avgpool backward needs even T");
  }
  ZS_REQUIRE(!p->unshuffle || (p->T % 2 == 0 && (p->C * es) % 16 == 0), "zs_grad_combine: unshuffle");
  ZS_REQUIRE(!p->dact_src || (al16(p->dact_src) && (p->dact_ld * es) % 16 == 0), "zs_grad_combine: dact");
  ZS_NORM_LAUNCH(grad_combine_kernel, g_norm_lim2.get());
  return zs_check_launch("zs_grad_combine");
}

extern "C" int zs_norm_decomposition(int32_t kernel, int32_t dtype, int32_t T, int32_t C) {
  ZS_REQUIRE(kernel >= 0 && kernel <= 2, "zs_norm_decomposition: kernel 0 (fwd), 1 (bwd) or 2 (combine)");
  const int lim = kernel == 0 ? g_norm_lim0.get() : kernel == 1 ? g_norm_lim1.get() : g_norm_lim2.get();
  return norm_wide(dtype, T, C, lim) ? 1 : 0;
}
```

zerospeech-tts-without-t_amd/engine.py:

```python
import functools
import os
import torch

from . import _lib as L
from .layers import (Act, ConvLayer, GruLayer, cast_rows, colsum_ok, fork_side, grad_combine, instnorm_bwd, instnorm_fwd, join_side,
                     next_uid, pack_operands, rup, weight_operand)

LRELU = L.ZS_ACT_LRELU


def _half_up(t):
    return (t + 1) // 2


def _norm_stats(ctx, training, prefix, key, n):
    if not training:
        return None, None
    return ctx.f32(prefix + 'mean' + key, n), ctx.f32(prefix + 'rstd' + key, n)


def ragged_lengths(who, lengths, training, B, T, lo):
    if training:
        raise L.ZsError('%s: ragged batches are an inference feature' % who)
    l0 = torch.as_tensor(lengths, dtype=torch.int32).reshape(-1)
    if l0.numel() != B or int(l0.max()) > T or int(l0.min()) < lo:
        raise L.ZsError('%s: lengths must be %d values in [%d, %d]' % (who, B, lo, T))
    return l0


GUMBEL_MODES = {'one_hot': L.ZS_ENC_ONE_HOT, 'binary': L.ZS_ENC_BINARY, 'continues': L.ZS_ENC_CONTINUES}


def linear_width(enc_mode, E):
    return {'multilabel_binary': 2 * E, 'binary': E * E}.get(enc_mode, E)


def operands_of(layers):
    w, v = [], []
    for l in layers:
        lw, lv = l.operands()
        w += lw
        v += lv
    return w, v


class EncoderEngine(object):
    def __init__(self, ctx, P, G, c_in, c_h1, c_h2, c_h3, enc_size, ns, dp, seg_len, enc_mode='multilabel_binary'):
        self.ctx = ctx
        self.uid = next_uid()
        self.c_in, self.c1, self.c2, self.H, self.E = c_in, c_h1, c_h2, c_h3, enc_size
        self.mode = enc_mode
        self.n_lin = linear_width(enc_mode, enc_size)
        self.ns, self.dp = float(ns), float(dp)
        self.pad_mode = L.ZS_PAD_REFLECT if seg_len >= 64 else L.ZS_PAD_ZERO
        if c_h1 % 8 or c_h2 % 8:
            raise ValueError('c_h1 and c_h2 must be multiples of 8 (16-byte rows)')
        mk = functools.partial(ConvLayer.from_params, ctx, P, G, pad_mode=self.pad_mode)
        self.conv1s = [mk('conv1s.%d' % i) for i in range(7)]
        self.conv2 = mk('conv2')
        self.convs = [(mk('conv%d' % a), mk('conv%d' % b, stride=2)) for a, b in ((3, 4), (5, 6), (7, 8))]
        self.dense = [(mk('dense%d' % a), mk('dense%d' % b)) for a, b in ((1, 2), (3, 4))]
        self.gru = GruLayer(ctx, P, G, 'RNN.', name='enc%d' % self.uid)
        self.linear = mk('linear')
        self.layers = self.conv1s + [self.conv2] + [l for p in self.convs for l in p] + [l for p in self.dense for l in p] + \
            [self.linear]
        self.ncat = 7 * c_h1 + c_in
        self.tape = None
        self.tapes = {}
        self.bank_d = None
        self.adam_plan = None

    def operands(self):
        w, v = operands_of(self.layers + [self.gru])
        if self.bank_d is not None:
            w += self._bank_d_operands()
        return w, v

    def pack(self):
        with L.pack_batch(self.ctx.stream):
            pack_operands(self.ctx, *self.operands())

    def forward(self, x, training, noise=None, noise_kind=2, seed=0, drop_masks=None, seed_ptr=None, lengths=None, tape=None):
        c, ns = self.ctx, self.ns
        B, T, F = x.shape
        Ls = [None] * 4
        if lengths is not None:
            l0 = ragged_lengths('EncoderEngine', lengths, training, B, T, 9)
            l1 = (l0 + 1) // 2; l2 = (l1 + 1) // 2; l3 = (l2 + 1) // 2
            self.last_lengths = l3
            ld = torch.stack([l0, l1, l2, l3]).to(c.device, non_blocking=True)
            Ls = [ld[i] for i in range(4)]
        assert F == self.c_in and x.dtype == torch.float32 and x.is_contiguous()
        st = c.stream
        c1, c2, H, E = self.c1, self.c2, self.H, self.E
        dp = self.dp if training else 0.0
        masks = drop_masks if drop_masks is not None else [None] * 6
        Ts = [T, _half_up(T), _half_up(_half_up(T)), _half_up(_half_up(_half_up(T)))]
        T4 = Ts[3]
        ksfx = '' if tape is None else '_' + str(tape)
        tag = '_%d_%d_%d' % (self.uid, B, T) + ksfx
        tp = {'B': B, 'T': T, 'Ts': Ts, 'training': training, 'seed': seed, 'masks': masks, 'dp': dp, 'seed_ptr': seed_ptr,
              'tag': tag, 'ksfx': ksfx}
        drop = dict(p=dp, seed=seed, seed_ptr=seed_ptr)
        skey = lambda k, Tk: '%d_%d_%d_%d' % (self.uid, k, B, Tk) + ksfx

        xin = c.act('e_xin' + tag, B, T, F)
        cat = c.act('e_cat' + tag, B, T, self.ncat)
        cast_rows(c, L.ptr(x), F, xin, dst2=cat, col_off2=7 * c1, act2=LRELU, slope2=ns)
        if c.overlap_wgrad and B * T >= 4096:
            sts = fork_side(c.device)
            for i, l in enumerate(self.conv1s):
                with torch.cuda.stream(sts[i % len(sts)]):
                    l.fwd(xin, out=cat.sub(i * c1, c1), act=LRELU, slope=ns, lengths=Ls[0])
            join_side(c.device)
        else:
            for i, l in enumerate(self.conv1s):
                l.fwd(xin, out=cat.sub(i * c1, c1), act=LRELU, slope=ns, lengths=Ls[0])
        y2 = c.act('e_y2' + tag, B, T, c2)
        self.conv2.fwd(cat, out=y2, act=LRELU, slope=ns)
        a = c.act('e_a0' + tag, B, T, c2)
        mean, rstd = _norm_stats(c, training, 'e_', skey(0, T), B * y2.ld)
        instnorm_fwd(c, y2, a, mean, rstd, self.pad_mode, lengths=Ls[0], stream_id=1, mask=masks[0], **drop)
        tp.update(xin=xin, cat=cat, y2=y2, a0=a, st0=(mean, rstd, 0), blocks=[], dense=[])
        for i, (la, lb) in enumerate(self.convs):
            ya = c.act('e_ya%d' % i + tag, B, Ts[i], c2)
            la.fwd(a, out=ya, act=LRELU, slope=ns, lengths=Ls[i])
            yb = c.act('e_yb%d' % i + tag, B, Ts[i + 1], c2)
            lb.fwd(ya, out=yb, act=LRELU, slope=ns, lengths=Ls[i])
            an = c.act('e_a%d' % (i + 1) + tag, B, Ts[i + 1], c2)
            k = 1 + i
            mean, rstd = _norm_stats(c, training, 'e_', skey(k, Ts[i + 1]), B * yb.ld)
            instnorm_fwd(c, yb, an, mean, rstd, self.pad_mode, res_mode=L.ZS_RES_AVGPOOL2, res=a, lengths=Ls[i + 1],
                         res_lengths=Ls[i], stream_id=k + 1, mask=masks[k], **drop)
            tp['blocks'].append((a, ya, yb, (mean, rstd, k)))
            a = an
        cat2 = c.act('e_cat2' + tag, B, T4, c2 + 2 * H)
        for j, (la, lb) in enumerate(self.dense):
            d1 = c.act('e_d1%d' % j + tag, B, T4, c2)
            la.fwd(a, out=d1, act=LRELU, slope=ns)
            d2 = c.act('e_d2%d' % j + tag, B, T4, c2)
            lb.fwd(d1, out=d2, act=LRELU, slope=ns)
            out = c.act('e_do%d' % j + tag, B, T4, c2) if j == 0 else Act(cat2.t, B, T4, c2, cat2.ld, 0, rup(c2, 32))
            k = 4 + j
            mean, rstd = _norm_stats(c, training, 'e_', skey(k, T4), B * d2.ld)
            instnorm_fwd(c, d2, out, mean, rstd, self.pad_mode, res_mode=L.ZS_RES_IDENTITY, res=a, lengths=Ls[3], stream_id=k + 1,
                         mask=masks[k], **drop)
            tp['dense'].append((a, d1, d2, (mean, rstd, k)))
            a = out
        gi = c.act('e_gi' + tag, B, T4, 6 * H)
        gates = c.raw('e_gates' + tag, B * T4 * 8 * H, c.tdt) if training else None
        self.gru.fwd(a, cat2, c2, gi, gates, lengths=Ls[3])
        logits = c.act('e_logits' + tag, B, T4, self.n_lin, dtype=torch.float32)
        self.linear.fwd(cat2, out=logits, out_f32=True)
        bits = c.act('e_bits' + tag, B, T4, E)
        bits_f32 = c.f32('e_bitsf' + tag, B * T4 * E)
        s = None
        if self.mode == 'multilabel_binary':
            y0 = c.f32('e_y0' + tag, B * T4 * E)
            L.call('zs_mbv_fwd', 'ZsMbvFwd', st, dtype=c.dt, logits=logits.ptr(), ld=logits.ld, logits_f32=1,
                   noise=L.ptr(noise), noise_kind=noise_kind, seed=seed, seed_ptr=seed_ptr, rows=B * T4, E=E, tau=0.1, bits=bits.ptr(),
                   ld_bits=bits.ld, bits_fill_cols=bits.ld, bits_f32=L.ptr(bits_f32), y0=L.ptr(y0))
        else:
            soft = self.mode != 'continues'
            y0 = c.f32('e_y0' + tag, B * T4 * self.n_lin) if (training and soft) else None
            s = c.f32('e_s' + tag, B * T4 * E) if (training and self.mode == 'binary') else None
            L.call('zs_gumbel_st_fwd', 'ZsGumbelStFwd', st, dtype=c.dt, mode=GUMBEL_MODES[self.mode], logits=logits.ptr(),
                   ld=logits.ld, logits_f32=1, noise=(L.ptr(noise) if soft else None), noise_kind=noise_kind, seed=seed,
                   seed_ptr=seed_ptr, rows=B * T4, E=E, tau=0.1, slope=self.ns, bits=bits.ptr(), ld_bits=bits.ld,
                   bits_fill_cols=bits.ld, bits_f32=L.ptr(bits_f32), y=L.ptr(y0), s=L.ptr(s))
        tp.update(cat2=cat2, gates=gates, y0=y0, s=s, T4=T4, gru_in=a, logits=logits, bits_f32=bits_f32)
        self.tape = tp
        self.tapes[tape] = tp
        return bits, bits_f32[:B * T4 * E].view(B, T4, E), logits

    def backward(self, dbits, dlogits_extra=None):
        self.backward_main(dbits, dlogits_extra)
        self.backward_bank()

    def backward_main(self, dbits, dlogits_extra=None, param_grads=True, tape=None):
        c, ns = self.ctx, self.ns
        tp = self.tape if tape is None else self.tapes[tape]
        assert tp is not None and tp['training']
        pg = param_grads
        B, T, Ts, T4 = tp['B'], tp['T'], tp['Ts'], tp['T4']
        c1, c2, H, E = self.c1, self.c2, self.H, self.E
        st = c.stream
        tag = tp['tag']
        cat2 = tp['cat2']
        drop, masks = dict(p=tp['dp'], seed=tp['seed'], seed_ptr=tp['seed_ptr']), tp['masks']
        dlog = c.act('e_dlog' + tag, B, T4, self.n_lin)
        if dbits is not None:
            if self.mode == 'multilabel_binary':
                L.call('zs_mbv_bwd', 'ZsMbvBwd', st, dtype=c.dt, dbits=dbits.ptr(), ld_dbits=dbits.ld, y0=L.ptr(tp['y0']),
                       rows=B * T4, E=E, tau=0.1, dlogits=dlog.ptr(), ld=dlog.ld, fill_cols=dlog.ld)
            else:
                cont = self.mode == 'continues'
                y, ld_y = (tp['logits'].ptr(), tp['logits'].ld) if cont else (L.ptr(tp['y0']), self.n_lin)
                L.call('zs_gumbel_st_bwd', 'ZsGumbelStBwd', st, dtype=c.dt, mode=GUMBEL_MODES[self.mode], dbits=dbits.ptr(),
                       ld_dbits=dbits.ld, y=y, ld_y=ld_y, s=L.ptr(tp['s']), rows=B * T4, E=E, tau=0.1, slope=ns,
                       dlogits=dlog.ptr(), ld=dlog.ld, fill_cols=dlog.ld)
            if dlogits_extra is not None:
                dlog.t[:B * T4 * dlog.ld].add_(dlogits_extra.t[:B * T4 * dlogits_extra.ld])
        else:
            dlog = dlogits_extra
        if pg:
            self.linear.wgrad(dlog, cat2)
        dcat2 = c.act('e_dcat2' + tag, B, T4, cat2.C)
        self.linear.dgrad(dlog, T4, dcat2)
        dgi = c.act('e_dgi' + tag, B, T4, 6 * H)
        dgh = c.act('e_dgh' + tag, B, T4, 6 * H)
        gin = tp['gru_in']
        da = c.act('e_da_d' + tag, B, T4, c2)
        self.gru.bwd(dcat2, c2, cat2, c2, tp['gates'], gin, dgi, dgh, da, add_src=dcat2, param_grads=pg)
        for j in (1, 0):
            la, lb = self.dense[j]
            xin, d1, d2, (mean, rstd, k) = tp['dense'][j]
            dz2 = c.act('e_dz2%d' % j + tag, B, T4, c2)
            instnorm_bwd(c, da, d2, mean, rstd, dz2, ns, stream_id=k + 1, mask=masks[k], **drop)
            if pg:
                lb.wgrad(dz2, d1)
            dz1 = c.act('e_dz1%d' % j + tag, B, T4, c2)
            lb.dgrad(dz2, T4, dz1, dact_src=d1, slope=ns)
            if pg:
                la.wgrad(dz1, xin)
            dn = c.act('e_da_d%d' % j + tag, B, T4, c2)
            la.dgrad(dz1, T4, dn, add_src=da)
            da = dn
        for i in (2, 1, 0):
            la, lb = self.convs[i]
            a, ya, yb, (mean, rstd, k) = tp['blocks'][i]
            dzb = c.act('e_dzb%d' % i + tag, B, Ts[i + 1], c2)
            instnorm_bwd(c, da, yb, mean, rstd, dzb, ns, stream_id=k + 1, mask=masks[k], **drop)
            if pg:
                lb.wgrad(dzb, ya)
            gp = c.act('e_gp%d' % i + tag, B, Ts[i] + 4, c2)
            lb.dgrad(dzb, Ts[i], gp)
            dza = c.act('e_dza%d' % i + tag, B, Ts[i], c2)
            grad_combine(c, gp, Ts[i], 2, 2, self.pad_mode, gp.ld, dza, ns, dact=ya)
            if pg:
                la.wgrad(dza, a)
            la.dgrad(dza, Ts[i], gp)
            dn = c.act('e_da%d' % i + tag, B, Ts[i], c2)
            grad_combine(c, gp, Ts[i], 2, 2, self.pad_mode, gp.ld, dn, ns, res_mode=L.ZS_RES_AVGPOOL2, res=da)
            da = dn
        y2, cat, xin = tp['y2'], tp['cat'], tp['xin']
        dz = c.act('e_dzy2' + tag, B, T, c2)
        mean, rstd, k = tp['st0']
        instnorm_bwd(c, da, y2, mean, rstd, dz, ns, stream_id=k + 1, mask=masks[k], **drop)
        dcat = c.act('e_dcat' + tag, B, T, self.ncat)
        if not pg:
            self.conv2.dgrad(dz, T, dcat, dact_src=cat, slope=ns)
            return dcat
        self.conv2.wgrad(dz, cat)
        self.conv2.dgrad(dz, T, dcat, dact_src=cat, slope=ns, n_cols=7 * c1)
        self._bank = (dcat, xin)

    BANK_PAD = 3

    def _bank_d_operands(self):
        c, c1 = self.ctx, self.c1
        ld, cp = self.bank_d_ld, self.bank_d_cp
        ops = []
        for i, l in enumerate(self.conv1s):
            k = l.k
            raw = [dict(dtype=c.dt, W=L.ptr(l.w, j), so=self.c_in * k, si=k, sj=1, Cout=c1, Cin=self.c_in, taps=1, transpose=1,
                        co_split2=0, inner_pad=c1, dst=L.ptr(self.bank_d), ldw=ld, n_rows=self.bank_d_rows, n_cols=c1, row_offset=0,
                        col_offset=(j + self.BANK_PAD - k // 2) * cp + i * c1) for j in range(k)]
            ops.append(weight_operand(l.w, c1, self.c_in, k, (self.c_in * k, k, 1), [], raw=raw))
        return ops

    def _bank_operand(self):
        if self.bank_d is None:
            c = self.ctx
            self.bank_d_cp = rup(7 * self.c1, c.kc)
            self.bank_d_ld = 7 * self.bank_d_cp
            self.bank_d_rows = rup(self.c_in, 128)
            self.bank_d = torch.zeros(self.bank_d_rows * self.bank_d_ld + 512, dtype=c.tdt, device=c.device)
            self.adam_plan = None
            with L.pack_batch(c.stream):
                pack_operands(c, self._bank_d_operands(), [])
        return self.bank_d

    def backward_input(self, dbits=None, dlogits=None, tape=None):
        if dbits is None and dlogits is None:
            raise ValueError('backward_input: dbits or dlogits')
        tp = self.tape if tape is None else self.tapes[tape]
        dcat = self.backward_main(dbits, dlogits, param_grads=False, tape=tape)
        c = self.ctx
        B, T, P = tp['B'], tp['T'], self.BANK_PAD
        W = self._bank_operand()
        if dcat.ld < self.bank_d_cp:
            raise L.ZsError('backward_input: concatenation rows of %d columns < K chunk %d' % (dcat.ld, self.bank_d_cp))
        g = c.act('e_gbank' + tp['tag'], B, T + 2 * P, self.c_in, dtype=torch.float32)
        L.call('zs_gemm_conv', 'ZsGemmConv', c.stream, dtype=c.dt, A=dcat.ptr(), lda=dcat.ld, a_batch_stride=T * dcat.ld, B=B, T_in=T,
               T_out=T + 2 * P, taps=7, stride=1, pad_left=0, pad_mode=L.ZS_PAD_ZERO, gather=1, cin_pad=self.bank_d_cp, W=L.ptr(W),
               ldw=self.bank_d_ld, N=self.c_in, n_pad=self.bank_d_rows, act=L.ZS_ACT_NONE, out=g.ptr(), ldc=g.ld,
               out_cols=g.ld, store_mode=L.ZS_STORE_ROWS, groups=1, out_f32=1)
        n = B * T * self.c_in
        dx = c.f32('e_dx' + tp['tag'], n)[:n].view(B, T, self.c_in)
        L.call('zs_enc_dx_fold', 'ZsEncDxFold', c.stream, dtype=c.dt, g=g.ptr(), ldg=g.ld, pass_through=dcat.ptr(7 * self.c1), ld_pass=dcat.ld, B=B, T=T, C=self.c_in, pad=P,
               pad_mode=self.pad_mode, dx=L.ptr(dx), ldx=self.c_in)
        return dx

    def backward_bank(self):
        dcat, xin = self._bank
        for i, l in enumerate(self.conv1s):
            l.wgrad(dcat.sub(i * self.c1, self.c1), xin)


class DecoderEngine(object):
    def __init__(self, ctx, P, G, c_in, c_out, c_h, c_a, ns, seg_len, output_mask=False):
        self.ctx = ctx
        self.uid = next_uid()
        self.E, self.F, self.ch, self.n_spk = c_in, c_out, c_h, c_a
        self.ns = float(ns)
        self.pad_mode = L.ZS_PAD_REFLECT if seg_len >= 64 else L.ZS_PAD_ZERO
        self.out_act = L.ZS_ACT_TANH if output_mask else L.ZS_ACT_SIGMOID
        if c_h % 32:
            raise ValueError('Decoder c_h must be a multiple of 32 (got %d)' % c_h)
        mk = functools.partial(ConvLayer.from_params, ctx, P, G, pad_mode=self.pad_mode)
        self.input_emb = mk('input_emb')
        self.convs = [(mk('conv%d' % a, split2=True), mk('conv%d' % b)) for a, b in ((1, 2), (3, 4), (5, 6))]
        self.dense = [(mk('dense%d' % a), mk('dense%d' % b)) for a, b in ((1, 2), (3, 4))]
        self.gru = GruLayer(ctx, P, G, 'RNN.', name='dec%d' % self.uid)
        self.dense5 = mk('dense5')
        self.linear = mk('linear')
        self.emb = [P['emb%d.weight' % i] for i in range(1, 6)]
        self.gemb = [G['emb%d.weight' % i] for i in range(1, 6)]
        self.e_dense, self.e_rnn = 3, 4
        self.layers = [self.input_emb] + [l for p in self.convs for l in p] + [l for p in self.dense for l in p] + \
            [self.dense5, self.linear]
        self.tape = None

    def operands(self):
        return operands_of(self.layers + [self.gru])

    def pack(self):
        with L.pack_batch(self.ctx.stream):
            pack_operands(self.ctx, *self.operands())

    def forward(self, bits, cidx, training, lengths=None):
        c, ns, ch = self.ctx, self.ns, self.ch
        B, T0 = bits.B, bits.T
        Ls = [None] * 4
        if lengths is not None:
            l0 = ragged_lengths('DecoderEngine', lengths, training, B, T0, 2)
            ld = torch.stack([l0, 2 * l0, 4 * l0, 8 * l0]).to(c.device, non_blocking=True)
            Ls = [ld[i] for i in range(4)]
        tag = '_%d_%d_%d' % (self.uid, B, T0)
        st = c.stream
        emb = self.emb
        tp = {'B': B, 'T0': T0, 'training': training, 'cidx': cidx, 'bits': bits, 'blocks': [], 'dense': []}
        x = c.act('d_x0' + tag, B, T0, ch)
        xe = c.act('d_xe0' + tag, B, T0, ch)
        self.input_emb.fwd(bits, out=x, out2=xe, vec2=emb[0], idx=cidx)
        T = T0
        for i, (la, lb) in enumerate(self.convs):
            ya = c.act('d_ya%d' % i + tag, B, T, 2 * ch) if training else None
            s = c.act('d_s%d' % i + tag, B, 2 * T, ch)
            la.fwd(xe, out=ya, act=LRELU, slope=ns, out2=s, vec2=emb[i], idx=cidx, store_mode2=L.ZS_STORE_SPLIT2, lengths=Ls[i])
            yb = c.act('d_yb%d' % i + tag, B, 2 * T, ch)
            lb.fwd(s, out=yb, act=LRELU, slope=ns, lengths=Ls[i + 1])
            xn = c.act('d_x%d' % (i + 1) + tag, B, 2 * T, ch)
            xen = c.act('d_xe%d' % (i + 1) + tag, B, 2 * T, ch)
            nxt = emb[i + 1] if i < 2 else emb[3]
            stt = _norm_stats(c, training, 'd_', '%d_c%d_%d_%d' % (self.uid, i, B, 2 * T), B * yb.ld)
            instnorm_fwd(c, yb, xn, *stt, self.pad_mode, res_mode=L.ZS_RES_UPSAMPLE2, res=x, lengths=Ls[i + 1], out2=xen, vec2=nxt,
                         idx=cidx)
            tp['blocks'].append((x, xe, ya, s, yb, stt, T))
            x, xe, T = xn, xen, 2 * T
        return self._fwd_dense(tp, x, xe, cidx, T, tag, B, training, Ls[3])

    def _fwd_dense(self, tp, x, xe, cidx, T, tag, B, training, lengths):
        c, ns, ch, emb = self.ctx, self.ns, self.ch, self.emb
        ed, er = self.e_dense, self.e_rnn
        cat3 = c.act('d_cat3' + tag, B, T, 3 * ch)
        for j, (la, lb) in enumerate(self.dense):
            y1 = c.act('d_y1%d' % j + tag, B, T, ch)
            y1e = c.act('d_y1e%d' % j + tag, B, T, ch)
            la.fwd(xe, out=y1, act=LRELU, slope=ns, out2=y1e, vec2=emb[ed], idx=cidx)
            y2 = c.act('d_y2%d' % j + tag, B, T, ch)
            lb.fwd(y1e, out=y2, act=LRELU, slope=ns)
            xn = c.act('d_dx%d' % j + tag, B, T, ch) if j == 0 else Act(cat3.t, B, T, ch, cat3.ld, 0, ch)
            xen = c.act('d_dxe%d' % j + tag, B, T, ch)
            stt = _norm_stats(c, training, 'd_', '%d_d%d_%d_%d' % (self.uid, j, B, T), B * y2.ld)
            instnorm_fwd(c, y2, xn, *stt, self.pad_mode, res_mode=L.ZS_RES_IDENTITY, res=x, lengths=lengths, out2=xen,
                         vec2=(emb[ed] if j == 0 else emb[er]), idx=cidx)
            tp['dense'].append((x, xe, y1, y1e, y2, stt))
            x, xe = xn, xen
        H = ch // 2
        gi = c.act('d_gi' + tag, B, T, 6 * H)
        gates = c.raw('d_gates' + tag, B * T * 8 * H, c.tdt) if training else None
        self.gru.fwd(xe, cat3, ch, gi, gates, bcast=(emb[er], cidx, 2 * ch), lengths=lengths)
        h5 = c.act('d_h5' + tag, B, T, ch)
        self.dense5.fwd(cat3, out=h5, act=LRELU, slope=ns)
        return self._fwd_tail(c, tp, h5, cat3, gates, xe, T, tag, B)

    def _fwd_tail(self, c, tp, h5, cat3, gates, xe, T, tag, B):
        xdec = c.act('d_xdec' + tag, B, T, self.F, dtype=torch.float32)
        self.linear.fwd(h5, out=xdec, act=self.out_act, out_f32=True)
        tp.update(cat3=cat3, gates=gates, gru_in=xe, h5=h5, T=T)
        self.tape = tp
        return xdec

    def backward(self, dlogit, need_dbits=True):
        self.backward_head(dlogit)
        return self.backward_convs(need_dbits)

    def backward_head(self, dlogit):
        c, ns, ch, tp = self.ctx, self.ns, self.ch, self.tape
        assert tp is not None and tp['training']
        B, T0, T = tp['B'], tp['T0'], tp['T']
        tag = '_%d_%d_%d' % (self.uid, B, T0)
        cat3, h5 = tp['cat3'], tp['h5']
        H = ch // 2
        ed, er = self.e_dense, self.e_rnn
        self._embsum = c.f32('d_embsum' + tag, 6 * B * ch)
        self._embsum.zero_()
        self.linear.wgrad(dlogit, h5)
        dz5 = c.act('d_dz5' + tag, B, T, ch)
        fuse = colsum_ok(T) and os.environ.get('ZS_FUSE_COLSUM', '1') == '1'
        esum = lambda k: L.ptr(self._embsum, k * B * ch)
        slot = lambda k, col0=0: (esum(k), ch, col0)
        thin5 = fuse and ch % 128 == 0 and os.environ.get('ZS_THIN_EMB5', '1') == '1'
        self.linear.dgrad(dlogit, T, dz5, dact_src=h5, slope=ns, colsum=(slot(5) if thin5 else None), colsum_post=True)
        self.dense5.wgrad(dz5, cat3)
        dcat3 = c.act('d_dcat3' + tag, B, T, 3 * ch)
        if thin5:
            self.dense5.dgrad(dz5, T, dcat3, n_cols=2 * ch)
            s32 = Act(self._embsum, B, 1, ch, ch, 5 * B * ch)
            sT = c.act('d_s5' + tag, B, 1, ch)
            cast_rows(c, s32.ptr(), ch, sT)
            slot4 = Act(self._embsum, B, 1, ch, ch, er * B * ch)
            self.dense5.dgrad(sT, 1, slot4, add_src=slot4, out_f32=True, add_f32=True, n_cols=ch, n_off=2 * ch)
        elif fuse:
            self.dense5.dgrad(dz5, T, dcat3, colsum=slot(er, 2 * ch), out_cols=2 * ch)
        else:
            self.dense5.dgrad(dz5, T, dcat3)
            grad_combine(c, dcat3.sub(2 * ch, ch), T, 0, 0, self.pad_mode, ch, None, ns, emb_sum=esum(er))
        dgi = c.act('d_dgi' + tag, B, T, 6 * H)
        dgh = c.act('d_dgh' + tag, B, T, 6 * H)
        gp = c.act('d_gpA' + tag, B, T + 2, ch)
        gpv = Act(gp.t, B, T, ch, gp.ld)
        dx = c.act('d_dxA' + tag, B, T, ch)
        if fuse:
            self.gru.bwd(dcat3, ch, cat3, ch, tp['gates'], tp['gru_in'], dgi, dgh, dx, add_src=dcat3.sub(0, ch), colsum=slot(er))
        else:
            self.gru.bwd(dcat3, ch, cat3, ch, tp['gates'], tp['gru_in'], dgi, dgh, gpv)
            grad_combine(c, gpv, T, 0, 0, self.pad_mode, ch, dx, ns, emb_sum=esum(er), res_mode=L.ZS_RES_IDENTITY, res=dcat3.sub(0, ch))
        for j in (1, 0):
            la, lb = self.dense[j]
            xin, xe, y1, y1e, y2, stt = tp['dense'][j]
            dz2 = c.act('d_dz2%d' % j + tag, B, T, ch)
            instnorm_bwd(c, dx, y2, *stt, dz2, ns)
            lb.wgrad(dz2, y1e)
            dz1 = c.act('d_dz1%d' % j + tag, B, T, ch)
            if fuse:
                lb.dgrad(dz2, T, dz1, dact_src=y1, slope=ns, colsum=slot(ed))
            else:
                lb.dgrad(dz2, T, gpv)
                grad_combine(c, gpv, T, 0, 0, self.pad_mode, ch, dz1, ns, emb_sum=esum(ed), dact=y1)
            la.wgrad(dz1, xe)
            dn = c.act('d_dxD%d' % j + tag, B, T, ch)
            if fuse:
                la.dgrad(dz1, T, dn, add_src=dx, colsum=slot(ed))
            else:
                la.dgrad(dz1, T, gpv)
                grad_combine(c, gpv, T, 0, 0, self.pad_mode, ch, dn, ns, emb_sum=esum(ed), res_mode=L.ZS_RES_IDENTITY, res=dx)
            dx = dn
        self._bw = (dx, gp, tag)

    def backward_convs(self, need_dbits=True):
        c, ns, ch, tp = self.ctx, self.ns, self.ch, self.tape
        dx, gp, tag = self._bw
        B, T0 = tp['B'], tp['T0']
        for i in (2, 1, 0):
            la, lb = self.convs[i]
            xin, xe, ya, s, yb, stt, Ti = tp['blocks'][i]
            esum = L.ptr(self._embsum, i * B * ch)
            T2 = 2 * Ti
            dzb = c.act('d_dzb%d' % i + tag, B, T2, ch)
            instnorm_bwd(c, dx, yb, *stt, dzb, ns)
            lb.wgrad(dzb, s)
            gp2 = Act(gp.t, B, T2 + 2, ch, gp.ld)
            lb.dgrad(dzb, T2, gp2)
            dza = c.act('d_dza%d' % i + tag, B, Ti, 2 * ch)
            grad_combine(c, gp2, T2, 1, 1, self.pad_mode, ch, dza, ns, emb_sum=esum, dact=ya, unshuffle=1)
            la.wgrad(dza, xe)
            gp1 = Act(gp.t, B, Ti + 2, ch, gp.ld)
            la.dgrad(dza, Ti, gp1)
            dn = c.act('d_dxC%d' % i + tag, B, Ti, ch)
            grad_combine(c, gp1, Ti, 1, 1, self.pad_mode, ch, dn, ns, emb_sum=esum, res_mode=L.ZS_RES_UPSAMPLE2,
                         res=dx)
            dx = dn
        sts = fork_side(c.device) if c.overlap_wgrad else None
        for k in range(5):
            st_k = sts[k % len(sts)].cuda_stream if sts is not None else c.stream
            L.call('zs_emb_scatter', 'ZsEmbScatter', st_k, emb_sum=L.ptr(self._embsum, k * B * ch), emb_ld=ch,
                   idx=L.ptr(tp['cidx']), B=B, demb=L.ptr(self.gemb[k]), demb_ld=ch, n_rows=self.n_spk, C=ch, accumulate=0)
        bits = tp['bits']
        self.input_emb.wgrad(dx, bits)
        dbits = None
        if need_dbits:
            dbits = c.act('d_dbits' + tag, B, T0, self.E)
            self.input_emb.dgrad(dx, T0, dbits)
        return dbits


class PatcherEngine(DecoderEngine):

    def __init__(self, ctx, P, G, c_in, c_out, c_h, c_a, ns):
        self.ctx = ctx
        self.uid = next_uid()
        self.E, self.F, self.ch, self.n_spk = c_in, c_out, c_h, c_a
        self.ns = float(ns)
        self.pad_mode = L.ZS_PAD_ZERO
        self.out_act = L.ZS_ACT_SIGMOID
        if c_h % 32:
            raise ValueError('Spectrogram_Patcher c_h must be a multiple of 32 (got %d)' % c_h)
        mk = functools.partial(ConvLayer.from_params, ctx, P, G, pad_mode=self.pad_mode)
        self.input_layer = mk('input_layer')
        self.dense = [(mk('dense%d' % a), mk('dense%d' % b)) for a, b in ((1, 2), (3, 4))]
        self.gru = GruLayer(ctx, P, G, 'RNN.', name='sp%d' % self.uid)
        self.dense5 = mk('dense5')
        self.linear = mk('linear')
        self.emb = [P['emb1.weight'], P['emb2.weight']]
        self.gemb = [G['emb1.weight'], G['emb2.weight']]
        self.e_dense, self.e_rnn = 0, 1
        self.layers = [self.input_layer] + [l for p in self.dense for l in p] + [self.dense5, self.linear]
        self.tape = None

    def forward(self, xd, cidx, training, lengths=None):
        c, ch = self.ctx, self.ch
        B, T = xd.B, xd.T
        ln = None
        if lengths is not None:
            ln = ragged_lengths('PatcherEngine', lengths, training, B, T, 1).to(c.device, non_blocking=True)
        tag = '_%d_%d_%d' % (self.uid, B, T)
        xin = c.act('p_xin' + tag, B, T, self.E)
        cast_rows(c, xd.ptr(), xd.ld, xin)
        tp = {'B': B, 'T0': T, 'training': training, 'cidx': cidx, 'xin': xin, 'dense': []}
        x = c.act('d_x0' + tag, B, T, ch)
        xe = c.act('d_xe0' + tag, B, T, ch)
        self.input_layer.fwd(xin, out=x, out2=xe, vec2=self.emb[0], idx=cidx)
        return self._fwd_dense(tp, x, xe, cidx, T, tag, B, training, ln)

    def backward(self, dlogit, need_dbits=False):
        if need_dbits:
            raise L.ZsError('PatcherEngine: the gradient w.r.t. the input spectrogram is not computed')
        self.backward_head(dlogit)
        dx, _, _ = self._bw
        c, tp, B, ch = self.ctx, self.tape, self.tape['B'], self.ch
        for k in range(2):
            L.call('zs_emb_scatter', 'ZsEmbScatter', c.stream, emb_sum=L.ptr(self._embsum, k * B * ch), emb_ld=ch, idx=L.ptr(tp['cidx']),
                   B=B, demb=L.ptr(self.gemb[k]), demb_ld=ch, n_rows=self.n_spk, C=ch, accumulate=0)
        self.input_layer.wgrad(dx, tp['xin'])
        return None


class ClassifierEngine(object):

    def __init__(self, ctx, P, G, c_in, c_h, n_class, dp, ns, seg_len):
        self.ctx, self.uid = ctx, next_uid()
        self.c_in, self.c_h, self.n_class = c_in, c_h, n_class
        self.ns, self.dp = float(ns), float(dp)
        self.pad_mode = L.ZS_PAD_REFLECT if seg_len >= 64 else L.ZS_PAD_ZERO
        mk = functools.partial(ConvLayer.from_params, ctx, P, G, pad_mode=self.pad_mode)
        self.blocks = [(mk('conv1'), mk('conv2'), False), (mk('conv3'), mk('conv4'), True), (mk('conv5'), mk('conv6'), True),
                       (mk('conv7'), mk('conv8'), False)]
        self.conv9 = mk('conv9', padded=False)
        self.layers = [l for b in self.blocks for l in b[:2]] + [self.conv9]
        self.tape = None

    def operands(self):
        return operands_of(self.layers)

    def pack(self):
        with L.pack_batch(self.ctx.stream):
            pack_operands(self.ctx, *self.operands())

    def forward(self, x, training, seed=0, drop_masks=None):
        c, ns = self.ctx, self.ns
        B, T = x.B, x.T
        if T != self.conv9.k:
            raise L.ZsError('SpeakerClassifier expects %d encoded frames (got %d)' % (self.conv9.k, T))
        tag = '_%d_%d_%d' % (self.uid, B, T)
        dp = self.dp if training else 0.0
        masks = drop_masks if drop_masks is not None else [None] * 4
        tp = {'B': B, 'T': T, 'training': training, 'seed': seed, 'masks': masks, 'dp': dp, 'x': x, 'blocks': []}
        a = x
        for i, (la, lb, res) in enumerate(self.blocks):
            ya = c.act('c_ya%d' % i + tag, B, T, la.Cout)
            la.fwd(a, out=ya, act=LRELU, slope=ns)
            yb = c.act('c_yb%d' % i + tag, B, T, lb.Cout)
            lb.fwd(ya, out=yb, act=LRELU, slope=ns)
            out = c.act('c_o%d' % i + tag, B, T, lb.Cout)
            mean, rstd = _norm_stats(c, training, 'c_', '%d' % i + tag, B * yb.ld)
            instnorm_fwd(c, yb, out, mean, rstd, self.pad_mode, res_mode=(L.ZS_RES_IDENTITY if res else L.ZS_RES_NONE),
                         res=(a if res else None), p=dp, seed=seed, stream_id=20 + i, mask=masks[i])
            tp['blocks'].append((a, ya, yb, (mean, rstd, i), res))
            a = out
        logits = c.act('c_logits' + tag, B, 1, self.n_class, dtype=torch.float32)
        self.conv9.fwd(a, out=logits, out_f32=True)
        tp['last'] = a
        self.tape = tp
        return logits

    def backward(self, dlogits_f32, ld, need_dx=True, param_grads=True):
        c, ns, tp = self.ctx, self.ns, self.tape
        B, T = tp['B'], tp['T']
        tag = '_%d_%d_%d' % (self.uid, B, T)
        dl = c.act('c_dl' + tag, B, 1, self.n_class)
        cast_rows(c, L.ptr(dlogits_f32), ld, dl)
        if param_grads:
            self.conv9.wgrad(dl, tp['last'])
        da = c.act('c_da_last' + tag, B, T, self.conv9.Cin)
        self.conv9.dgrad(dl, T, da)
        for i in (3, 2, 1, 0):
            la, lb, _ = self.blocks[i]
            a, ya, yb, stt, res = tp['blocks'][i]
            mean, rstd, k = stt
            dzb = c.act('c_dzb%d' % i + tag, B, T, lb.Cout)
            instnorm_bwd(c, da, yb, mean, rstd, dzb, ns, p=tp['dp'], seed=tp['seed'], stream_id=20 + k, mask=tp['masks'][k])
            if param_grads:
                lb.wgrad(dzb, ya)
            gp = c.act('c_gp%d' % i + tag, B, T + lb.pad_l + lb.pad_r, lb.Cin)
            lb.dgrad(dzb, T, gp)
            dza = c.act('c_dza%d' % i + tag, B, T, la.Cout)
            grad_combine(c, gp, T, lb.pad_l, lb.pad_r, self.pad_mode, gp.ld, dza, ns, dact=ya)
            if param_grads:
                la.wgrad(dza, a)
            if i == 0 and not need_dx:
                return None
            gp2 = c.act('c_gq%d' % i + tag, B, T + la.pad_l + la.pad_r, la.Cin)
            la.dgrad(dza, T, gp2)
            dn = c.act('c_da%d' % i + tag, B, T, la.Cin)
            grad_combine(c, gp2, T, la.pad_l, la.pad_r, self.pad_mode, gp2.ld, dn, ns, res_mode=(L.ZS_RES_IDENTITY if res else L.ZS_RES_NONE),
                         res=(da if res else None))
            da = dn
        return da
# ... 1 lines not shown
```

zerospeech-tts-without-t_amd/layers.py:

```python
import ctypes
import os

import torch

from . import _lib as L


def colsum_ok(T):
    return T > 0 and 128 % T == 0


def rup(x, m):
    return (x + m - 1) // m * m


DTYPES = {'fp32': (L.ZS_F32, torch.float32), 'bf16': (L.ZS_BF16, torch.bfloat16)}
SLACK = 512
EPS_IN = 1e-5


class Act(object):
    __slots__ = ('t', 'B', 'T', 'C', 'ld', 'off', 'cols')

    def __init__(self, t, B, T, C, ld, off=0, cols=None):
        self.t, self.B, self.T, self.C, self.ld, self.off = t, B, T, C, ld, off
        self.cols = cols if cols is not None else ld

    @property
    def rows(self):
        return self.B * self.T

    def ptr(self, col=0):
        return self.t.data_ptr() + (self.off + col) * self.t.element_size()

    def sub(self, col, C, cols=None):
        return Act(self.t, self.B, self.T, C, self.ld, self.off + col, cols if cols is not None else C)

    def view2d(self):
        return self.t[self.off:self.off + self.rows * self.ld].view(self.rows, self.ld) if self.off == 0 else \
            self.t[self.off - (self.off % self.ld):][:self.rows * self.ld].view(self.rows, self.ld)

    def valid(self):
        base = self.t[self.off:self.off + (self.rows - 1) * self.ld + self.C]
        return torch.as_strided(base, (self.B, self.T, self.C), (self.T * self.ld, self.ld, 1))


_SIDE = {}
N_SIDE = max(1, int(os.environ.get('ZS_SIDE_STREAMS', '4')))
HW_QUEUES = int(os.environ.get('GPU_MAX_HW_QUEUES') or 4)
MULTI_STREAM = HW_QUEUES >= 4


def side_stream(device):
    key = (device.type, device.index)
    if key not in _SIDE:
        _SIDE[key] = {'streams': [torch.cuda.Stream(device) for _ in range(N_SIDE)], 'used': False, 'next': 0, 'ws': [None] * N_SIDE}
    return _SIDE[key]


def side_events(device):
    sd = side_stream(device)
    evs = []
    for st in sd['streams']:
        ev = torch.cuda.Event()
        ev.record(st)
        evs.append(ev)
    return evs


def fork_side(device):
    sd = side_stream(device)
    ev = torch.cuda.Event()
    ev.record(torch.cuda.current_stream(device))
    for st in sd['streams']:
        st.wait_event(ev)
    sd['used'] = True
    return sd['streams']


def join_side(device):
    sd = side_stream(device)
    if sd['used']:
        cur = torch.cuda.current_stream(device)
        for ev in side_events(device):
            cur.wait_event(ev)
        sd['used'] = False
    sd['next'] = 0


_OPT = {}


def opt_stream(device):
    key = (device.type, device.index)
    if key not in _OPT:
        _OPT[key] = torch.cuda.Stream(device)
    return _OPT[key]


_STATUS = {}


def device_status(device):
    device = torch.device(device)
    key = (device.type, device.index if device.index is not None else torch.cuda.current_device())
    if key not in _STATUS:
        _STATUS[key] = torch.zeros(4, dtype=torch.int32, device=device)
    return _STATUS[key]


def check_status(device):
    st = device_status(device)
    v = int(st[0].item())
    if v:
        st.zero_()
        raise L.ZsError('persistent GRU %s timed out waiting for its workgroup group: the results since the last check are '
                        'invalid (status 0x%x; is another process holding CUs of this GPU?)' %
                        (' and '.join(n for b, n in ((1, 'forward'), (2, 'BPTT')) if v & b), v))


_COPY = {}


def copy_stream(device):
    key = (device.type, device.index)
    if key not in _COPY:
        _COPY[key] = torch.cuda.Stream(device)
    return _COPY[key]


class Ctx(object):

    def __init__(self, device, dtype='fp32'):
        if dtype not in DTYPES:
            raise ValueError('dtype must be fp32 or bf16')
        self.device = torch.device(device)
        if self.device.type != 'cuda':
            raise L.ZsError('zs_amd runs on an MI355X only (device %s requested); there is no CPU path' % device)
        L.lib()
        self.dtype_name = dtype
        self.dt, self.tdt = DTYPES[dtype]
        self.es = 4 if dtype == 'fp32' else 2
        self.kc = 128 // self.es
        self._bufs = {}
        self._ws = None
        self.pin_wgrad_streams = False
        self.status = device_status(self.device)
        self.overlap_wgrad = os.environ.get('ZS_OVERLAP_WGRAD', '1' if MULTI_STREAM else '0') == '1'
        L.set_option('wgrad_alone', 0 if self.overlap_wgrad else 1)

    @property
    def stream(self):
        return torch.cuda.current_stream(self.device).cuda_stream

    def raw(self, name, n, dtype, zero=True):
        key = (name, n, dtype)
        t = self._bufs.get(key)
        if t is None:
            t = torch.zeros(n + SLACK, dtype=dtype, device=self.device)
            self._bufs[key] = t
        return t

    def act(self, name, B, T, C, ld=None, dtype=None):
        ld = ld if ld is not None else rup(C, 32)
        dtype = dtype if dtype is not None else self.tdt
        return Act(self.raw(name, B * T * ld, dtype), B, T, C, ld)

    def f32(self, name, n):
        return self.raw(name, n, torch.float32)

    def workspace(self, nbytes):
        if self._ws is None or self._ws.numel() < nbytes:
            if self._ws is not None:
                torch.cuda.synchronize(self.device)
            self._ws = torch.empty(int(nbytes * 1.25) + 1024, dtype=torch.uint8, device=self.device)
        return self._ws

    def release(self):
        self._bufs.clear()
        self._ws = None

    def check_status(self):
        check_status(self.device)


def weight_view(dst, transpose, inner_pad, ldw, n_rows, n_cols, dst_off=0, row_offset=0, col_offset=0, parity=False, row_perm=None):
    return dict(dst=dst, dst_off=dst_off, transpose=transpose, inner_pad=inner_pad, ldw=ldw, n_rows=n_rows, n_cols=n_cols,
                row_offset=row_offset, col_offset=col_offset, parity=parity, row_perm=row_perm)


def weight_operand(w, Cout, Cin, taps, strides, views, co_split2=0, raw=None):
    return dict(w=w, Cout=Cout, Cin=Cin, taps=taps, strides=tuple(strides), views=views, co_split2=int(co_split2), raw=raw or [])


def vector_operand(src, copies):
    return dict(src=src, copies=copies)


def pack_operands(ctx, weights, vectors):
    st = ctx.stream
    for op in weights:
        so, si, sj = op['strides']
        common = dict(dtype=ctx.dt, so=so, si=si, Cout=op['Cout'], Cin=op['Cin'], co_split2=op['co_split2'])
        for v in op['views']:
            kw = dict(common, transpose=v['transpose'], inner_pad=v['inner_pad'], dst=L.ptr(v['dst'], v['dst_off']), ldw=v['ldw'],
                      n_rows=v['n_rows'], row_offset=v['row_offset'], row_perm=L.ptr(v['row_perm']))
            if v['parity']:
                ne, no = (op['taps'] + 1) // 2, op['taps'] // 2
                L.call('zs_pack_weight', 'ZsPackWeight', st, W=L.ptr(op['w']), sj=2 * sj, taps=ne, n_cols=ne * v['inner_pad'],
                       col_offset=v['col_offset'], **kw)
                L.call('zs_pack_weight', 'ZsPackWeight', st, W=L.ptr(op['w'], sj), sj=2 * sj, taps=no, n_cols=no * v['inner_pad'],
                       col_offset=v['col_offset'] + ne * v['inner_pad'], **kw)
            else:
                L.call('zs_pack_weight', 'ZsPackWeight', st, W=L.ptr(op['w']), sj=sj, taps=op['taps'], n_cols=v['n_cols'],
                       col_offset=v['col_offset'], **kw)
        for kw in op['raw']:
            L.call('zs_pack_weight', 'ZsPackWeight', st, **kw)
    for vc in vectors:
        for cp in vc['copies']:
            L.vec_copy(cp['dst'][cp['dst_off']:cp['dst_off'] + cp['n']], vc['src'][cp['src_offset']:], st, src_stride=cp['src_stride'],
                       n=cp['n'])


class PlanCtx(object):

    def __init__(self, dtype='bf16'):
        self.device = torch.device('meta')
        self.dtype_name = dtype
        self.dt, self.tdt = DTYPES[dtype]
        self.es = 4 if dtype == 'fp32' else 2
        self.kc = 128 // self.es


class ConvLayer(object):

    def __init__(self, ctx, weight, bias, gweight, gbias, stride=1, split2=False, pad_mode=L.ZS_PAD_REFLECT, name='', padded=True,
                 strides=None):
        self.ctx, self.name = ctx, name
        self.w, self.b, self.gw, self.gb = weight, bias, gweight, gbias
        self.Cout, self.Cin = weight.shape[0], weight.shape[1]
        self.k = weight.shape[2] if weight.dim() == 3 else 1
        self.stride, self.split2, self.pad_mode = stride, split2, pad_mode
        self.pad_l = self.k // 2 if padded else 0
        self.pad_r = (self.k - 1 - self.k // 2) if padded else 0
        self.so, self.si, self.sj = (self.Cin * self.k, self.k, 1) if weight.dim() == 3 else (self.Cin, 1, 0)
        if strides is not None:
            self.so, self.si, self.sj = strides
        kc = ctx.kc
        self.cin_pad, self.cout_pad = rup(self.Cin, kc), rup(self.Cout, kc)
        self.ldw, self.n_pad = self.k * self.cin_pad, rup(self.Cout, 128)
        self.ldw_d, self.n_pad_d = self.k * self.cout_pad, rup(self.Cin, 128)
        dev, tdt = ctx.device, ctx.tdt
        self.wf = torch.zeros(self.n_pad * self.ldw + SLACK, dtype=tdt, device=dev)
        self.wd = torch.zeros(self.n_pad_d * self.ldw_d + SLACK, dtype=tdt, device=dev)
        self.bias_p = torch.zeros(self.Cout, dtype=torch.float32, device=dev) if (split2 and bias is not None) else None
        self.sid = next_sid()
        self.parity = (stride == 2 and self.k > 1)

    @classmethod
    def from_params(cls, ctx, P, G, name, pad_mode, **kw):
        return cls(ctx, P[name + '.weight'], P[name + '.bias'], G[name + '.weight'], G[name + '.bias'], pad_mode=pad_mode, name=name, **kw)

    def operands(self):
        views = [weight_view(self.wf, 0, self.cin_pad, self.ldw, self.n_pad, self.ldw),
                 weight_view(self.wd, 1, self.cout_pad, self.ldw_d, self.n_pad_d, self.ldw_d, parity=self.parity)]
        w = [weight_operand(self.w, self.Cout, self.Cin, self.k, (self.so, self.si, self.sj), views, co_split2=self.split2)]
        v = []
        if self.bias_p is not None:
            h = self.Cout // 2
            v = [vector_operand(self.b, [dict(dst=self.bias_p, dst_off=0, n=h, src_offset=0, src_stride=2),
                                         dict(dst=self.bias_p, dst_off=h, n=h, src_offset=1, src_stride=2)])]
        return w, v

    def pack(self):
        pack_operands(self.ctx, *self.operands())

    def bias_ptr(self):
        if self.b is None:
            return None
        return L.ptr(self.bias_p if self.bias_p is not None else self.b)

    def t_out(self, T_in):
        return (T_in + self.pad_l + self.pad_r - self.k) // self.stride + 1

    def fwd(self, A, out=None, act=L.ZS_ACT_NONE, slope=0.0, out_f32=False, out_cols=None, store_mode=L.ZS_STORE_ROWS,
            out2=None, vec2=None, idx=None, store_mode2=L.ZS_STORE_ROWS, out2_cols=None, pre_vec=None, bias=True, lengths=None):
        c = self.ctx
        T_out = self.t_out(A.T)
        kw = dict(dtype=c.dt, A=A.ptr(), lda=A.ld, a_batch_stride=A.T * A.ld, B=A.B, T_in=A.T, T_out=T_out, taps=self.k,
                  stride=self.stride, pad_left=self.pad_l, pad_mode=self.pad_mode, gather=0, cin_pad=self.cin_pad,
                  W=L.ptr(self.wf), ldw=self.ldw, N=self.Cout, n_pad=self.n_pad, bias=(self.bias_ptr() if bias else None), act=act,
                  slope=slope, groups=1)
        if pre_vec is not None:
            kw.update(pre_vec=L.ptr(pre_vec), pre_vec_ld=pre_vec.shape[1], vec_idx=L.ptr(idx))
        if lengths is not None and self.k > 1:
            kw.update(lengths=L.ptr(lengths), pad_right=self.pad_r)
        if out is not None:
            kw.update(out=out.ptr(), ldc=out.ld, out_f32=int(out_f32), store_mode=store_mode,
                      out_cols=out_cols if out_cols is not None else (min(out.cols, rup(self.Cout, 32)) if store_mode == L.ZS_STORE_ROWS else self.Cout // 2))
        if out2 is not None:
            kw.update(out2=out2.ptr(), ldc2=out2.ld, store_mode2=store_mode2,
                      out2_cols=out2_cols if out2_cols is not None else (min(out2.cols, rup(self.Cout, 32)) if store_mode2 == L.ZS_STORE_ROWS else self.Cout // 2))
            if vec2 is not None:
                kw.update(vec2=L.ptr(vec2), vec2_ld=vec2.shape[1], vec_idx=L.ptr(idx))
        L.call('zs_gemm_conv', 'ZsGemmConv', c.stream, **kw)
        return T_out

    def dgrad(self, dY, T_x, out, dact_src=None, slope=0.0, add_src=None, out_f32=False, add_f32=False, colsum=None, out_cols=None,
              n_cols=None, n_off=0, colsum_post=False):
        c = self.ctx
        Tp = T_x + self.pad_l + self.pad_r
        if self.parity:
            if dact_src is not None or add_src is not None or colsum is not None or n_cols is not None or n_off:
                raise ValueError('stride-2 dgrad: dact_src, add_src, colsum, n_cols and n_off are not supported')
            return self._dgrad_parity(dY, Tp, out, out_f32, out_cols)
        N, n_pad = self.Cin, self.n_pad_d
        if n_cols is not None and (n_cols < self.Cin or n_off):
            N = n_cols
            n_pad = rup(n_cols, 256) if n_off + rup(n_cols, 256) <= self.n_pad_d else rup(n_cols, 128)
            if n_off + n_pad > self.n_pad_d:
                raise ValueError('dgrad: channel block [%d, %d) does not fit the packed weight (%d rows)' % (n_off, n_off + n_cols, self.n_pad_d))
        kw = dict(dtype=c.dt, A=dY.ptr(), lda=dY.ld, a_batch_stride=dY.T * dY.ld, B=dY.B, T_in=dY.T, T_out=Tp, taps=self.k,
                  stride=self.stride, pad_left=0, pad_mode=L.ZS_PAD_ZERO, gather=1, cin_pad=self.cout_pad,
                  W=L.ptr(self.wd, n_off * self.ldw_d), ldw=self.ldw_d, N=N, n_pad=n_pad, act=L.ZS_ACT_NONE, slope=slope,
                  out=out.ptr(), ldc=out.ld, out_cols=(out_cols if out_cols is not None else min(out.cols, rup(N, 32))),
                  store_mode=L.ZS_STORE_ROWS, groups=1, out_f32=int(out_f32))
        if dact_src is not None:
            kw.update(dact_src=dact_src.ptr(), dact_ld=dact_src.ld)
        if add_src is not None:
            kw.update(add_src=add_src.ptr(), add_ld=add_src.ld, add_f32=int(add_f32))
        if colsum is not None:
            kw.update(colsum=colsum[0], colsum_ld=colsum[1], colsum_col0=colsum[2], colsum_post=int(colsum_post))
        L.call('zs_gemm_conv', 'ZsGemmConv', c.stream, **kw)
        return Tp

    def _dgrad_parity(self, dY, Tp, out, out_f32, out_cols):
        c = self.ctx
        Te = Tp + (Tp & 1)
        if out.T != Te:
            raise ValueError('stride-2 dgrad: the output needs %d rows per sample (padded domain %d rounded up to even), got %d' % (Te, Tp, out.T))
        ne = (self.k + 1) // 2
        for par, taps in ((0, ne), (1, self.k // 2)):
            kw = dict(dtype=c.dt, A=dY.ptr(), lda=dY.ld, a_batch_stride=dY.T * dY.ld, B=dY.B, T_in=dY.T, T_out=Te // 2, taps=taps,
                      stride=1, pad_left=0, pad_mode=L.ZS_PAD_ZERO, gather=1, cin_pad=self.cout_pad,
                      W=L.ptr(self.wd, par * ne * self.cout_pad), ldw=self.ldw_d, N=self.Cin, n_pad=self.n_pad_d, act=L.ZS_ACT_NONE,
                      out=out.ptr(par * out.ld), ldc=2 * out.ld, out_cols=(out_cols if out_cols is not None else min(out.cols, rup(self.Cin, 32))),
                      store_mode=L.ZS_STORE_ROWS, groups=1, out_f32=int(out_f32))
            L.call('zs_gemm_conv', 'ZsGemmConv', c.stream, **kw)
        return Tp

    def wgrad(self, dY, X, accumulate=False, bias=True):
        c = self.ctx
        es = c.es
        y_cols = min(dY.cols, rup(self.Cout, 16 // es))
        x_cols = min(X.cols, rup(self.Cin, 16 // es))
        kw = dict(dtype=c.dt, dY=dY.ptr(), ldy=dY.ld, y_cols=y_cols, X=X.ptr(), ldx=X.ld, x_batch_stride=X.T * X.ld,
                  x_cols=x_cols, B=X.B, T_in=X.T, T_out=dY.T, taps=self.k, stride=self.stride, pad_left=self.pad_l,
                  pad_mode=self.pad_mode, Cout=self.Cout, Cin=self.Cin, dW=L.ptr(self.gw), so=self.so, si=self.si, sj=self.sj,
                  db=(L.ptr(self.gb) if bias else None), co_split2=int(self.split2), accumulate=int(accumulate), splits=0)
        wgrad_call(c, kw, self.sid)


class Conv2dLayer(object):

    def __init__(self, ctx, weight, bias, gweight, gbias, stride=2, pad_mode=L.ZS_PAD_REFLECT, name='', dgrad_only=False):
        self.ctx, self.name = ctx, name
        self.w, self.b, self.gw, self.gb = weight, bias, gweight, gbias
        self.Cout, self.Cin, self.k = weight.shape[0], weight.shape[1], weight.shape[2]
        if weight.dim() != 4 or weight.shape[3] != self.k or stride not in (1, 2):
            raise ValueError('Conv2dLayer: square kernels, stride 1 or 2')
        self.stride, self.pad_mode, self.pad = stride, pad_mode, self.k // 2
        self.taps = self.k * self.k
        kc = ctx.kc
        self.cin_pad, self.cout_pad = rup(self.Cin, kc), rup(self.Cout, kc)
        self.ldw, self.n_pad, self.n_pad_d = self.taps * self.cin_pad, rup(self.Cout, 128), rup(self.Cin, 128)
        dev, tdt = ctx.device, ctx.tdt
        self.wf = None if dgrad_only else torch.zeros(self.n_pad * self.ldw + SLACK, dtype=tdt, device=dev)
        self.nt = [(self.k + 1) // 2, self.k // 2] if stride == 2 else [self.k]
        self.wd = {}
        for ph in range(len(self.nt)):
            for pw in range(len(self.nt)):
                ld = self.nt[ph] * self.nt[pw] * self.cout_pad
                self.wd[(ph, pw)] = (torch.zeros(self.n_pad_d * ld + SLACK, dtype=tdt, device=dev), ld)
        self.sid = next_sid()

    def out_hw(self, H, W):
        return (H + 2 * self.pad - self.k) // self.stride + 1, (W + 2 * self.pad - self.k) // self.stride + 1

    def operands(self):
        c, k = self.ctx, self.k
        common = dict(dtype=c.dt, so=self.Cin * self.taps, si=self.taps, Cout=self.Cout, Cin=self.Cin, co_split2=0)
        views = []
        if self.wf is not None:
            views.append(weight_view(self.wf, 0, self.cin_pad, self.ldw, self.n_pad, self.ldw))
        raw = []
        step = self.stride
        for (ph, pw), (buf, ld) in self.wd.items():
            nh, nw = self.nt[ph], self.nt[pw]
            for kwp in range(nw):
                raw.append(dict(common, transpose=1, inner_pad=self.cout_pad, dst=L.ptr(buf), ldw=ld, n_rows=self.n_pad_d,
                                n_cols=nh * self.cout_pad, col_offset=kwp * nh * self.cout_pad,
                                W=L.ptr(self.w, (pw + step * kwp) * k + ph), sj=step, taps=nh))
        return [weight_operand(self.w, self.Cout, self.Cin, self.taps, (self.Cin * self.taps, self.taps, 1), views, raw=raw)], []

    def pack(self):
        pack_operands(self.ctx, *self.operands())

    def fwd(self, X, H, W, out, act=L.ZS_ACT_NONE, slope=0.0, bias=True, out_f32=False):
        c = self.ctx
        Ho, Wo = self.out_hw(H, W)
        if self.wf is None:
            raise ValueError('Conv2dLayer.fwd: built with dgrad_only')
        if X.T != H * W or out.T != Ho * Wo or X.B != out.B:
            raise ValueError('Conv2dLayer.fwd: rows %d x %d for an image of %d x %d, output %d x %d' % (X.B, X.T, H, W, out.B, out.T))
        L.call('zs_gemm_conv', 'ZsGemmConv', c.stream, dtype=c.dt, A=X.ptr(), lda=X.ld, a_batch_stride=X.T * X.ld, B=X.B, T_in=H * W,
               T_out=Ho * Wo, taps=self.taps, stride=self.stride, pad_left=self.pad, pad_mode=self.pad_mode, gather=0, cin_pad=self.cin_pad,
               W=L.ptr(self.wf), ldw=self.ldw, N=self.Cout, n_pad=self.n_pad, bias=(L.ptr(self.b) if (bias and self.b is not None) else None),
               act=act, slope=slope, groups=1, out=out.ptr(), ldc=out.ld, out_f32=int(out_f32), store_mode=L.ZS_STORE_ROWS,
               out_cols=min(out.cols, rup(self.Cout, 32)), w_in=W, w_out=Wo, taps_h=self.k)
        return Ho, Wo

    def wgrad(self, dY, X, H, W, accumulate=False, bias=True):
        c, es = self.ctx, self.ctx.es
        Ho, Wo = self.out_hw(H, W)
        kw = dict(dtype=c.dt, dY=dY.ptr(), ldy=dY.ld, y_cols=min(dY.cols, rup(self.Cout, 16 // es)), X=X.ptr(), ldx=X.ld,
                  x_batch_stride=X.T * X.ld, x_cols=min(X.cols, rup(self.Cin, 16 // es)), B=X.B, T_in=H * W, T_out=Ho * Wo, taps=self.taps,
                  stride=self.stride, pad_left=self.pad, pad_mode=self.pad_mode, Cout=self.Cout, Cin=self.Cin, dW=L.ptr(self.gw),
                  so=self.Cin * self.taps, si=self.taps, sj=1, db=(L.ptr(self.gb) if bias else None), co_split2=0,
                  accumulate=int(accumulate), splits=0, w_in=W, w_out=Wo, taps_h=self.k)
        wgrad_call(c, kw, self.sid)

    def padded_hw(self, H, W):
        Ho, Wo = self.out_hw(H, W)
        return (Ho - 1) * self.stride + self.k, (Wo - 1) * self.stride + self.k

    def dgrad(self, dY, H, W, out, name, add=None, fill_cols=None):
        c = self.ctx
        if self.stride != 2:
            raise ValueError('Conv2dLayer.dgrad: stride 2 only')
        Ho, Wo = self.out_hw(H, W)
        Hp, Wp = self.padded_hw(H, W)
        g = {}
        for (ph, pw), (buf, ld) in self.wd.items():
            Hc, Wc = (Hp - ph + 1) // 2, (Wp - pw + 1) // 2
            gq = c.act('%s_q%d%d' % (name, ph, pw), dY.B, Hc * Wc, self.Cin)
            L.call('zs_gemm_conv', 'ZsGemmConv', c.stream, dtype=c.dt, A=dY.ptr(), lda=dY.ld, a_batch_stride=dY.T * dY.ld, B=dY.B,
                   T_in=Ho * Wo, T_out=Hc * Wc, taps=self.nt[ph] * self.nt[pw], stride=1, pad_left=0, pad_mode=L.ZS_PAD_ZERO, gather=1,
                   cin_pad=self.cout_pad, W=L.ptr(buf), ldw=ld, N=self.Cin, n_pad=self.n_pad_d, act=L.ZS_ACT_NONE, out=gq.ptr(), ldc=gq.ld,
                   out_cols=min(gq.cols, rup(self.Cin, 32)), store_mode=L.ZS_STORE_ROWS, groups=1, out_f32=0, w_in=Wo, w_out=Wc,
                   taps_h=self.nt[ph])
            g[(ph, pw)] = gq
        g00 = g[(0, 0)]
        L.call('zs_conv2d_unpad', 'ZsConv2dUnpad', c.stream, dtype=c.dt, g00=g00.ptr(), g01=g[(0, 1)].ptr(), g10=g[(1, 0)].ptr(),
               g11=g[(1, 1)].ptr(), ldg=g00.ld, B=dY.B, H=H, W=W, C=rup(self.Cin, 8), Hp=Hp, Wp=Wp, pad=self.pad, pad_mode=self.pad_mode,
               add=(add.ptr() if add is not None else None), ldadd=(add.ld if add is not None else 0), out=out.ptr(), ldo=out.ld,
               fill_cols=(fill_cols if fill_cols is not None else out.ld))


_SID = [0]
_UID = [0]


def next_sid():
    _SID[0] += 1
    return _SID[0]


def next_uid():
    _UID[0] += 1
    return _UID[0]


def side_launch(ctx, sid, need):
    if not ctx.overlap_wgrad:
        return ctx.stream, ctx.workspace(need)
    sd = side_stream(ctx.device)
    if sid is not None and ctx.pin_wgrad_streams:
        i = sid % len(sd['streams'])
    else:
        i = sd['next']
        sd['next'] = (i + 1) % len(sd['streams'])
    ws = sd['ws'][i]
    if ws is None or ws.numel() < need:
        if any(w is not None for w in sd['ws']):
            torch.cuda.synchronize(ctx.device)
        size = int(need * 1.25) + 1024
        sd['ws'] = [torch.empty(size, dtype=torch.uint8, device=ctx.device) for _ in sd['streams']]
        ws = sd['ws'][i]
    ev = torch.cuda.Event()
    ev.record(torch.cuda.current_stream(ctx.device))
    sd['streams'][i].wait_event(ev)
    sd['used'] = True
    return sd['streams'][i].cuda_stream, ws


def wgrad_call(ctx, kw, sid=None):
    S = L.STRUCTS['ZsGemmWgrad']
    s = S()
    for k, v in kw.items():
        if v is not None:
            setattr(s, k, v)
    need = L.lib().zs_gemm_wgrad_workspace_bytes(ctypes.byref(s))
    stream, ws = side_launch(ctx, sid, need)
    s.workspace = ws.data_ptr()
    s.workspace_bytes = ws.numel()
    L.check(L.lib().zs_gemm_wgrad(ctypes.byref(s), ctypes.c_void_p(stream)), 'zs_gemm_wgrad')


def instnorm_fwd(ctx, x, out, mean, rstd, pad_mode, res_mode=L.ZS_RES_NONE, res=None, lengths=None, res_lengths=None, p=0.0,
                 seed=0, stream_id=0, mask=None, seed_ptr=None, out2=None, vec2=None, idx=None):
    L.call('zs_instnorm_fwd', 'ZsInstNormFwd', ctx.stream, dtype=ctx.dt, x=x.ptr(), ldx=x.ld, out=out.ptr(), ldo=out.ld,
           out2=(out2.ptr() if out2 is not None else None), ldo2=(out2.ld if out2 is not None else 0), vec2=L.ptr(vec2),
           vec2_ld=(vec2.shape[1] if vec2 is not None else 0), vec2_cols=(vec2.shape[1] if vec2 is not None else 0), idx=L.ptr(idx),
           mean=L.ptr(mean), rstd=L.ptr(rstd), B=x.B, T=x.T, C=x.ld, eps=EPS_IN, drop_p=p, seed=seed, stream_id=stream_id,
           mask=L.ptr(mask), mask_ld=(mask.shape[-1] if mask is not None else 0), res_mode=res_mode,
           res=(res.ptr() if res is not None else None), ldres=(res.ld if res is not None else 0), T_res=(res.T if res is not None else 0),
           res_pad_mode=pad_mode, seed_ptr=seed_ptr, lengths=L.ptr(lengths), res_lengths=L.ptr(res_lengths))


def instnorm_bwd(ctx, dout, x, mean, rstd, dz, slope, p=0.0, seed=0, stream_id=0, mask=None, seed_ptr=None):
    L.call('zs_instnorm_bwd', 'ZsInstNormBwd', ctx.stream, dtype=ctx.dt, dout=dout.ptr(), ldd=dout.ld, x=x.ptr(), ldx=x.ld,
           mean=L.ptr(mean), rstd=L.ptr(rstd), dz=dz.ptr(), ldz=dz.ld, B=x.B, T=x.T, C=x.ld, drop_p=p, seed=seed, stream_id=stream_id,
           mask=L.ptr(mask), mask_ld=(mask.shape[-1] if mask is not None else 0), slope=slope, seed_ptr=seed_ptr)


def grad_combine(ctx, gp, T, pad_l, pad_r, pad_mode, C, out, slope, res_mode=L.ZS_RES_NONE, res=None, dact=None, emb_sum=None,
                 unshuffle=0):
    L.call('zs_grad_combine', 'ZsGradCombine', ctx.stream, dtype=ctx.dt, gp=gp.ptr(), ldg=gp.ld, pad_left=pad_l, pad_right=pad_r,
           pad_mode=pad_mode, B=gp.B, T=T, C=C, emb_sum=emb_sum, emb_ld=(C if emb_sum is not None else 0),
           emb_cols=(C if emb_sum is not None else 0), res_mode=res_mode, res=(res.ptr() if res is not None else None),
           ldres=(res.ld if res is not None else 0), dact_src=(dact.ptr() if dact is not None else None),
           dact_ld=(dact.ld if dact is not None else 0), slope=slope, out=(out.ptr() if out is not None else None),
           ldo=(out.ld if out is not None else 0), unshuffle=unshuffle)


def cast_rows(ctx, src, ld_src, dst, dst_f32=False, dst2=None, col_off2=0, act2=L.ZS_ACT_NONE, slope2=0.0):
    L.call('zs_cast_rows', 'ZsCastRows', ctx.stream, dtype=ctx.dt, src=src, ld_src=ld_src, src_f32=1, dst=dst.ptr(), ld_dst=dst.ld,
           dst_f32=int(dst_f32), col_off=0, rows=dst.rows, cols=dst.C, fill_cols=dst.ld, act=L.ZS_ACT_NONE,
           dst2=(dst2.ptr() if dst2 is not None else None), ld_dst2=(dst2.ld if dst2 is not None else 0), col_off2=col_off2,
           fill_cols2=(dst2.ld - col_off2 if dst2 is not None else 0), act2=act2, slope2=slope2)


class GruLayer(object):

    def __init__(self, ctx, P, G, prefix, name=''):
        self.ctx, self.name = ctx, name
        sfx = ['', '_reverse']
        self.w_ih = [P[prefix + 'weight_ih_l0' + s] for s in sfx]
        self.w_hh = [P[prefix + 'weight_hh_l0' + s] for s in sfx]
        self.b_ih = [P[prefix + 'bias_ih_l0' + s] for s in sfx]
        self.b_hh = [P[prefix + 'bias_hh_l0' + s] for s in sfx]
        self.gw_ih = [G[prefix + 'weight_ih_l0' + s] for s in sfx]
        self.gw_hh = [G[prefix + 'weight_hh_l0' + s] for s in sfx]
        self.gb_ih = [G[prefix + 'bias_ih_l0' + s] for s in sfx]
        self.gb_hh = [G[prefix + 'bias_hh_l0' + s] for s in sfx]
        self.H = self.w_hh[0].shape[1]
        self.Cin = self.w_ih[0].shape[1]
        self.sids = [next_sid() for _ in range(4)]
        H, Cin = self.H, self.Cin
        if H % 8:
            raise ValueError('GRU hidden size must be a multiple of 8 (got %d)' % H)
        dev, tdt = ctx.device, ctx.tdt
        self.G6 = 6 * H
        self.g6_pad = rup(6 * H, ctx.kc)
        kc = ctx.kc
        self.cin_pad = rup(Cin, kc)
        self.ih_ldw, self.ih_npad = self.cin_pad, rup(6 * H, 128)
        self.wih_f = torch.zeros(self.ih_npad * self.ih_ldw + SLACK, dtype=tdt, device=dev)
        self.ih_ldw_d, self.ih_npad_d = self.g6_pad, rup(Cin, 128)
        self.wih_d = torch.zeros(self.ih_npad_d * self.ih_ldw_d + SLACK, dtype=tdt, device=dev)
        self.bih = torch.zeros(6 * H, dtype=torch.float32, device=dev)
        self.hh_ldw, self.hh_npad = rup(H, kc), rup(3 * H, 128)
        self.whh_f = torch.zeros(2 * self.hh_npad * self.hh_ldw + SLACK, dtype=tdt, device=dev)
        self.hh_ldw_t, self.hh_npad_t = rup(3 * H, kc), rup(H, 128)
        self.whh_t = torch.zeros(2 * self.hh_npad_t * self.hh_ldw_t + SLACK, dtype=tdt, device=dev)
        self.bhh = torch.zeros(2 * 3 * H, dtype=torch.float32, device=dev)
        self.fast = (H % 32 == 0)
        self.perm = None
        if self.fast:
            n = torch.arange(3 * H)
            hc, rem = n // 96, n % 96
            self.perm = ((rem // 32) * H + hc * 32 + (rem % 32)).to(torch.int32).to(dev)

    def operands(self):
        c, H, Cin = self.ctx, self.H, self.Cin
        w, v = [], []
        for d in range(2):
            w.append(weight_operand(self.w_ih[d], 3 * H, Cin, 1, (Cin, 1, 0), [
                weight_view(self.wih_f, 0, self.cin_pad, self.ih_ldw, 3 * H, self.ih_ldw, row_offset=3 * H * d),
                weight_view(self.wih_d, 1, 3 * H, self.ih_ldw_d, self.ih_npad_d, 3 * H, col_offset=3 * H * d)]))
            w.append(weight_operand(self.w_hh[d], 3 * H, H, 1, (H, 1, 0), [
                weight_view(self.whh_f, 0, rup(H, c.kc), self.hh_ldw, (3 * H if self.fast else self.hh_npad), self.hh_ldw,
                            dst_off=d * self.hh_npad * self.hh_ldw, row_perm=self.perm),
                weight_view(self.whh_t, 1, rup(3 * H, c.kc), self.hh_ldw_t, self.hh_npad_t, self.hh_ldw_t,
                            dst_off=d * self.hh_npad_t * self.hh_ldw_t)]))
            v.append(vector_operand(self.b_ih[d], [dict(dst=self.bih, dst_off=3 * H * d, n=3 * H, src_offset=0, src_stride=1)]))
            v.append(vector_operand(self.b_hh[d], [dict(dst=self.bhh, dst_off=3 * H * d, n=3 * H, src_offset=0, src_stride=1)]))
        return w, v

    def pack(self):
        pack_operands(self.ctx, *self.operands())

    def _work(self, B):
        n = L.lib().zs_gru_work_bytes(B, self.H)
        return self.ctx.f32('gru_work_%s' % self.name, (n + 3) // 4)

    def fwd(self, X, out, out_col, gi, gates, bcast=None, lengths=None):
        c, H = self.ctx, self.H
        if lengths is not None and gates is not None:
            raise L.ZsError('GruLayer.fwd: ragged batches are an inference feature (no tape)')
        L.call('zs_gemm_conv', 'ZsGemmConv', c.stream, dtype=c.dt, A=X.ptr(), lda=X.ld, a_batch_stride=X.T * X.ld, B=X.B,
               T_in=X.T, T_out=X.T, taps=1, stride=1, pad_left=0, pad_mode=L.ZS_PAD_ZERO, gather=0, cin_pad=self.cin_pad,
               W=L.ptr(self.wih_f), ldw=self.ih_ldw, N=6 * H, n_pad=self.ih_npad, bias=L.ptr(self.bih), act=L.ZS_ACT_NONE,
               out=gi.ptr(), ldc=gi.ld, out_cols=min(gi.cols, rup(6 * H, 32)), groups=1)
        if lengths is not None:
            L.call('zs_rows_reverse', 'ZsRowsReverse', c.stream, dtype=c.dt, x=gi.ptr(), ld=gi.ld, col0=3 * H, cols=3 * H, B=X.B, T=X.T,
                   lengths=L.ptr(lengths))
        work = self._work(X.B)
        L.call('zs_gru_fwd', 'ZsGruFwd', c.stream, dtype=c.dt, B=X.B, T=X.T, H=H, gi=gi.ptr(), ldgi=gi.ld,
               whh=L.ptr(self.whh_f), ldw=self.hh_ldw, n_pad=self.hh_npad, w_gstride=self.hh_npad * self.hh_ldw,
               bhh=L.ptr(self.bhh), bhh_gstride=3 * H, out=out.ptr(), ldo=out.ld, out_col=out_col,
               gates=L.ptr(gates) if gates is not None else None, work=L.ptr(work), work_bytes=work.numel() * 4,
               whh_interleaved=int(self.fast), status=L.ptr(c.status),
               bcast_vec=(L.ptr(bcast[0]) if bcast else None), bcast_ld=(bcast[0].shape[1] if bcast else 0),
               bcast_idx=(L.ptr(bcast[1]) if bcast else None), bcast_col=(bcast[2] if bcast else 0),
               dir1_forward=int(lengths is not None))
        if lengths is not None:
            L.call('zs_rows_reverse', 'ZsRowsReverse', c.stream, dtype=c.dt, x=out.ptr(), ld=out.ld, col0=out_col + H, cols=H, B=X.B, T=X.T,
                   lengths=L.ptr(lengths))

    def check(self, B):
        L.check(L.lib().zs_gru_check(L.ptr(self._work(B)), B, self.H, self.ctx.stream), 'zs_gru_check')

    def bwd(self, dout, dout_col, out, out_col, gates, X, dgi, dgh, dX, add_src=None, colsum=None, param_grads=True):
        c, H = self.ctx, self.H
        B, T = X.B, X.T
        work = self._work(B)
        L.call('zs_gru_bwd', 'ZsGruBwd', c.stream, dtype=c.dt, B=B, T=T, H=H, dout=dout.ptr(), ldd=dout.ld, dout_col=dout_col,
               out=out.ptr(), ldo=out.ld, out_col=out_col, gates=L.ptr(gates), whh_t=L.ptr(self.whh_t), ldw=self.hh_ldw_t,
               n_pad=self.hh_npad_t, w_gstride=self.hh_npad_t * self.hh_ldw_t, dgi=dgi.ptr(), ldgi=dgi.ld, dgh=dgh.ptr(),
               ldgh=dgh.ld, work=L.ptr(work), work_bytes=work.numel() * 4, status=L.ptr(c.status))
        for d in (range(2) if param_grads else ()):
            wgrad_call(c, dict(dtype=c.dt, dY=dgh.ptr(3 * H * d), ldy=dgh.ld, y_cols=3 * H, X=out.ptr(out_col + d * H),
                               ldx=out.ld, x_batch_stride=T * out.ld, x_cols=H, B=B, T_in=T, T_out=T, taps=1, stride=1,
                               pad_left=(1 if d == 0 else -1), pad_mode=L.ZS_PAD_ZERO, Cout=3 * H, Cin=H,
                               dW=L.ptr(self.gw_hh[d]), so=H, si=1, sj=0, db=L.ptr(self.gb_hh[d]), co_split2=0,
                               accumulate=0, splits=0), self.sids[2 * d])
            wgrad_call(c, dict(dtype=c.dt, dY=dgi.ptr(3 * H * d), ldy=dgi.ld, y_cols=3 * H, X=X.ptr(), ldx=X.ld,
                               x_batch_stride=T * X.ld, x_cols=min(X.cols, rup(self.Cin, 16 // c.es)), B=B, T_in=T, T_out=T,
                               taps=1, stride=1, pad_left=0, pad_mode=L.ZS_PAD_ZERO, Cout=3 * H, Cin=self.Cin,
                               dW=L.ptr(self.gw_ih[d]), so=self.Cin, si=1, sj=0, db=L.ptr(self.gb_ih[d]), co_split2=0,
                               accumulate=0, splits=0), self.sids[2 * d + 1])
        kw = dict(dtype=c.dt, A=dgi.ptr(), lda=dgi.ld, a_batch_stride=T * dgi.ld, B=B, T_in=T, T_out=T, taps=1, stride=1,
                  pad_left=0, pad_mode=L.ZS_PAD_ZERO, gather=0, cin_pad=self.g6_pad, W=L.ptr(self.wih_d), ldw=self.ih_ldw_d,
                  N=self.Cin, n_pad=self.ih_npad_d, act=L.ZS_ACT_NONE, out=dX.ptr(), ldc=dX.ld,
                  out_cols=min(dX.cols, rup(self.Cin, 32)), groups=1)
        if add_src is not None:
            kw.update(add_src=add_src.ptr(), add_ld=add_src.ld, add_f32=0)
        if colsum is not None:
            kw.update(colsum=colsum[0], colsum_ld=colsum[1], colsum_col0=colsum[2])
        L.call('zs_gemm_conv', 'ZsGemmConv', c.stream, **kw)
```

Before: 3.144 million frames/s.

## Store leaky-ReLU sign bits instead of bf16 activations for decoder backward

```diff
diff --git a/include/zs_amd.h b/include/zs_amd.h
--- a/include/zs_amd.h
+++ b/include/zs_amd.h
@@ -42,6 +42,8 @@
   int32_t colsum_post;
   const int32_t* lengths; int32_t pad_right;
   int32_t w_in, w_out, taps_h;
+  uint8_t* sign_out; int64_t sign_ld;
+  const uint8_t* dact_bits; int64_t dact_bits_ld;
 } ZsGemmConv;
 int zs_gemm_conv(const ZsGemmConv* p, void* stream);
 enum { ZS_GEMM_PATH_P8 = 0, ZS_GEMM_PATH_RING_PP = 1, ZS_GEMM_PATH_RING = 2, ZS_GEMM_PATH_DMA64 = 3, ZS_GEMM_PATH_DMA128 = 4,
@@ -140,6 +142,7 @@
   int32_t res_mode; const void* res; int64_t ldres;
   const void* dact_src; int64_t dact_ld; float slope;
   void* out; int64_t ldo; int32_t unshuffle;
+  const uint8_t* dact_bits; int64_t dact_bits_ld;
 } ZsGradCombine;
 int zs_grad_combine(const ZsGradCombine* p, void* stream);
 int zs_norm_decomposition(int32_t kernel, int32_t dtype, int32_t T, int32_t C);
diff --git a/zerospeech-tts-without-t_amd/csrc/zs_gemm.hip b/zerospeech-tts-without-t_amd/csrc/zs_gemm.hip
--- a/zerospeech-tts-without-t_amd/csrc/zs_gemm.hip
+++ b/zerospeech-tts-without-t_amd/csrc/zs_gemm.hip
@@ -87,6 +87,11 @@
 
 constexpr int CPITCH = 132;
 constexpr int EPI_LDS_BYTES = BM * CPITCH * 4;
+
+template <typename T> __device__ __forceinline__ bool sign_pos(float v);
+template <> __device__ __forceinline__ bool sign_pos<float>(float v) { return v > 0.f; }
+template <> __device__ __forceinline__ bool sign_pos<bf16_t>(float v) { return bf2f(f2bf(v)) > 0.f; }
+__device__ __forceinline__ float dbit_f(unsigned bits, int j, float slope) { return ((bits >> j) & 1u) ? 1.f : slope; }
 
 template <typename T, typename OT>
 __device__ __forceinline__ void store_group(OT* base, int64_t row, int64_t ld, int col, int limit, bool aligned,
@@ -115,11 +120,12 @@
     const float* q = sC + r0 * CPITCH + col;
     float a0 = 0.f, a1 = 0.f, a2 = 0.f, a3 = 0.f;
     int r = 0;
-    if (p.colsum_post && (p.dact_src || p.add_src)) {
+    if (p.colsum_post && (p.dact_src || p.dact_bits || p.add_src)) {
       for (; r < p.T_out; ++r) {
         float v = q[r * CPITCH];
         const int64_t mm = (int64_t)m + r;
         if (p.dact_src) v *= dlrelu_f(p.dtype == ZS_F32 ? ((const float*)p.dact_src)[mm * p.dact_ld + n] : bf2f(((const bf16_t*)p.dact_src)[mm * p.dact_ld + n]), p.slope);
+        if (p.dact_bits) v *= dbit_f(p.dact_bits[mm * p.dact_bits_ld + (n >> 3)], n & 7, p.slope);
         if (p.add_src) v += (p.add_f32 || p.dtype == ZS_F32) ? ((const float*)p.add_src)[mm * p.add_ld + n] : bf2f(((const bf16_t*)p.add_src)[mm * p.add_ld + n]);
         a0 += v;
       }
@@ -202,6 +208,17 @@
     } else if (p.act == ZS_ACT_TANH) {
 #pragma unroll
       for (int j = 0; j < 8; ++j) v[j] = tanhf(v[j]);
+    }
+    if (p.sign_out && n < p.N) {
+      unsigned bits = 0;
+#pragma unroll
+      for (int j = 0; j < 8; ++j) bits |= (sign_pos<T>(v[j]) ? 1u : 0u) << j;
+      p.sign_out[(int64_t)m * p.sign_ld + (n >> 3)] = (uint8_t)bits;
+    }
+    if (p.dact_bits && n < p.N) {
+      const unsigned bits = p.dact_bits[(int64_t)m * p.dact_bits_ld + (n >> 3)];
+#pragma unroll
+      for (int j = 0; j < 8; ++j) v[j] *= dbit_f(bits, j, p.slope);
     }
     if (p.dact_src) {
       const T* dp = (const T*)p.dact_src + (int64_t)m * p.dact_ld + n;
@@ -795,12 +812,14 @@
   const int half = p.N >> 1;
   const bool split = (p.out && p.store_mode == ZS_STORE_SPLIT2) || (p.out2 && p.store_mode2 == ZS_STORE_SPLIT2);
   return (p.out == nullptr || (!p.out_f32 && al16(p.out, p.ldc * 2) && ((p.out_gstride * 2) & 15) == 0 && (p.out_cols & 7) == 0)) &&
-         (p.out2 == nullptr || (al16(p.out2, p.ldc2 * 2) && (p.out2_cols & 7) == 0 && p.dact_src == nullptr && p.add_src == nullptr)) &&
+         (p.out2 == nullptr || (al16(p.out2, p.ldc2 * 2) && (p.out2_cols & 7) == 0 && p.dact_src == nullptr && p.dact_bits == nullptr &&
+                                p.add_src == nullptr)) &&
          (p.dact_src == nullptr || al16(p.dact_src, p.dact_ld * 2)) &&
          (p.add_src == nullptr || (!p.add_f32 && al16(p.add_src, p.add_ld * 2))) &&
          ((p.pre_vec == nullptr && p.vec2 == nullptr) || (p.T_out & 15) == 0) && (!split || (half & 7) == 0) &&
          (p.act == ZS_ACT_NONE || p.act == ZS_ACT_LRELU) &&
-         (p.colsum == nullptr || ((PBM % p.T_out) == 0 && p.out2 == nullptr));
+         (p.colsum == nullptr || ((PBM % p.T_out) == 0 && p.out2 == nullptr)) &&
+         (p.sign_out == nullptr || (p.out == nullptr && p.out2 != nullptr));
 }
 
 template <bool HAS2>
@@ -811,6 +830,8 @@
   const int colb = wc * 64 + (lane & 15);
   const int rbase = wr * 128 + 4 * (lane >> 4);
   const int half = p.N >> 1;
+  const bool SIGN = HAS2 && p.sign_out != nullptr;
+  const bool OUT1 = !HAS2 || p.out != nullptr || !SIGN;
   int64_t bsel[2][4];
   const bool need_b = p.pre_vec != nullptr || p.vec2 != nullptr;
 #pragma unroll
@@ -849,12 +870,47 @@
             if (p.act == ZS_ACT_LRELU) v = lrelu_f(v, p.slope);
             if (!cval) v = 0.f;
             if constexpr (HAS2) c[mq][nq][mt][nt][i4] = v;
-            sT[(rbase + mq * 64 + mt * 16 + i4) * PT + col] = f2bf(v);
+            if (OUT1) sT[(rbase + mq * 64 + mt * 16 + i4) * PT + col] = f2bf(v);
           }
     }
+  if (SIGN) {
+    const int cw = n0 + wc * 64;
+    const int nb = min(8, max(0, (p.N - cw) >> 3));
+    const int sh = 16 * (lane & 3);
+    uint8_t* sp = p.sign_out + (cw >> 3) + (int64_t)(m0 + wr * 128 + 4 * (lane & 3)) * p.sign_ld;
+    const int mrow = m0 + wr * 128 + 4 * (lane & 3);
+#pragma unroll
+    for (int mq = 0; mq < 2; ++mq)
+#pragma unroll
+      for (int mt = 0; mt < 4; ++mt)
+#pragma unroll
+        for (int i4 = 0; i4 < 4; ++i4) {
+          unsigned long long bal[4];
+#pragma unroll
+          for (int k = 0; k < 4; ++k) bal[k] = __ballot(sign_pos<bf16_t>(c[mq][k >> 1][mt][k & 1][i4]));
+          const unsigned lo = ((unsigned)(bal[0] >> sh) & 0xffffu) | ((unsigned)(bal[1] >> sh) << 16);
+          const unsigned hi = ((unsigned)(bal[2] >> sh) & 0xffffu) | ((unsigned)(bal[3] >> sh) << 16);
+          const int ro = mq * 64 + mt * 16 + i4;
+          if (lane < 4 && mrow + ro < M) {
+            uint8_t* d = sp + (int64_t)ro * p.sign_ld;
+            if (nb == 8) {
+              reinterpret_cast<unsigned*>(d)[0] = lo;
+              reinterpret_cast<unsigned*>(d)[1] = hi;
+            } else {
+              const unsigned long long w = (unsigned long long)lo | ((unsigned long long)hi << 32);
+#pragma unroll 1
+              for (int j = 0; j < nb; ++j) d[j] = (uint8_t)(w >> (8 * j));
+            }
+          }
+          __builtin_amdgcn_sched_barrier(0);
+        }
+  }
+  const int c8 = (tid & 31) * 8, r0 = tid >> 5;
+  const int n = n0 + c8;
+  if (OUT1) {
   __syncthreads();
 
-  const bool cs_post = !HAS2 && p.colsum != nullptr && p.colsum_post && (p.dact_src != nullptr || p.add_src != nullptr);
+  const bool cs_post = !HAS2 && p.colsum != nullptr && p.colsum_post && (p.dact_src != nullptr || p.dact_bits != nullptr || p.add_src != nullptr);
   auto colsum_pass = [&]() {
     const int ns = PBM / p.T_out;
     const int col = tid & 255, n = n0 + col, hs = tid >> 8;
@@ -877,15 +933,13 @@
   };
   if (!HAS2 && p.colsum != nullptr && !cs_post) colsum_pass();
 
-  const int c8 = (tid & 31) * 8, r0 = tid >> 5;
-  const int n = n0 + c8;
   if (p.out != nullptr) {
     unsigned short* outp = (unsigned short*)p.out + (int64_t)g * p.out_gstride;
     const bool sp = p.store_mode == ZS_STORE_SPLIT2;
     const int hi = sp ? (n >= half) : 0;
     const int oc = n - hi * half;
     const bool cok = sp ? (n < p.N) : (n < p.out_cols);
-    const bool second = p.dact_src != nullptr || p.add_src != nullptr;
+    const bool second = p.dact_src != nullptr || p.dact_bits != nullptr || p.add_src != nullptr;
     if (cok && !second) {
 #pragma unroll 8
       for (int it = 0; it < 16; ++it) {
@@ -900,16 +954,19 @@
     } else if (!HAS2 && cok) {
       const bf16_t* dsrc = (const bf16_t*)p.dact_src;
       const bf16_t* asrc = (const bf16_t*)p.add_src;
+      const uint8_t* dbits = n < p.N ? p.dact_bits : nullptr;
       const bool tail = n + 8 > p.N;
 #pragma unroll 1
       for (int it0 = 0; it0 < 16; it0 += 8) {
         Raw8<bf16_t> rd[8], ra[8];
+        unsigned db[8];
         uint4 w[8];
 #pragma unroll
         for (int u = 0; u < 8; ++u) {
           const int row = r0 + 16 * (it0 + u);
           const int m = min(m0 + row, M - 1);
           if (dsrc) rd[u].ld(dsrc + (int64_t)m * p.dact_ld + n);
+          if (dbits) db[u] = dbits[(int64_t)m * p.dact_bits_ld + (n >> 3)];
           if (asrc) ra[u].ld(asrc + (int64_t)m * p.add_ld + n);
           w[u] = *reinterpret_cast<const uint4*>(sT + row * PT + c8);
         }
@@ -925,6 +982,10 @@
 #pragma unroll
               for (int j = 0; j < 8; ++j) v[j] *= dlrelu_f(y[j], p.slope);
             }
+            if (dbits) {
+#pragma unroll
+              for (int j = 0; j < 8; ++j) v[j] *= dbit_f(db[u], j, p.slope);
+            }
             if (asrc) {
               ra[u].cvt(y);
 #pragma unroll
@@ -946,8 +1007,9 @@
     __syncthreads();
     colsum_pass();
   }
+  }
   if constexpr (HAS2) {
-    __syncthreads();
+    if (OUT1) __syncthreads();
     const bool sp = p.store_mode2 == ZS_STORE_SPLIT2;
 #pragma unroll
     for (int nq = 0; nq < 2; ++nq)
@@ -2078,6 +2140,15 @@
              "zs_gemm_conv: colsum needs T_out (%d) to divide 128, 0 <= colsum_col0 < N and no bias / pre_vec / activation / groups", p->T_out);
   ZS_REQUIRE(!p->lengths || (p->gather == 0 && p->B < 65536 && p->T_in < 32768 && p->pad_right >= 0 && p->colsum == nullptr),
              "zs_gemm_conv: lengths (ragged batch) needs gather 0, B < 65536, T_in < 32768, pad_right >= 0 and no colsum");
+  ZS_REQUIRE(!(p->dact_src && p->dact_bits), "zs_gemm_conv: dact_src and dact_bits are mutually exclusive");
+  ZS_REQUIRE(!p->sign_out || (p->N % 8 == 0 && ((uintptr_t)p->sign_out & 3) == 0 && p->sign_ld % 4 == 0 && p->sign_ld >= p->N / 8 &&
+                              p->groups <= 1 && !p->lengths && !p->out_f32),
+             "zs_gemm_conv: sign_out needs N %% 8 == 0 (N %d), a 4-byte aligned pointer, sign_ld (%lld) a multiple of 4 and >= N / 8, "
+             "no groups, no lengths and no out_f32", p->N, (long long)p->sign_ld);
+  ZS_REQUIRE(!p->dact_bits || (p->N % 8 == 0 && ((uintptr_t)p->dact_bits & 3) == 0 && p->dact_bits_ld % 4 == 0 &&
+                               p->dact_bits_ld >= p->N / 8 && p->groups <= 1),
+             "zs_gemm_conv: dact_bits needs N %% 8 == 0 (N %d), a 4-byte aligned pointer, dact_bits_ld (%lld) a multiple of 4 and "
+             ">= N / 8 and no groups", p->N, (long long)p->dact_bits_ld);
   pl.groups = p->groups > 0 ? p->groups : 1;
   pl.regs = 0;
   const int64_t M = (int64_t)p->B * p->T_out;
diff --git a/zerospeech-tts-without-t_amd/csrc/zs_norm.hip b/zerospeech-tts-without-t_amd/csrc/zs_norm.hip
--- a/zerospeech-tts-without-t_amd/csrc/zs_norm.hip
+++ b/zerospeech-tts-without-t_amd/csrc/zs_norm.hip
@@ -317,6 +317,11 @@
 #pragma unroll
       for (int k = 0; k < 8; ++k) o[k] *= dlrelu_f(y[k], p.slope);
     }
+    if (p.dact_bits) {
+      const unsigned bits = p.dact_bits[orow * p.dact_bits_ld + (ocol >> 3)];
+#pragma unroll
+      for (int k = 0; k < 8; ++k) o[k] *= ((bits >> k) & 1u) ? 1.f : p.slope;
+    }
     store8<T>((T*)p.out + orow * p.ldo + ocol, o);
   }
 }
@@ -387,6 +392,11 @@
   }
   ZS_REQUIRE(!p->unshuffle || (p->T % 2 == 0 && (p->C * es) % 16 == 0), "zs_grad_combine: unshuffle");
   ZS_REQUIRE(!p->dact_src || (al16(p->dact_src) && (p->dact_ld * es) % 16 == 0), "zs_grad_combine: dact");
+  ZS_REQUIRE(!(p->dact_src && p->dact_bits), "zs_grad_combine: dact_src and dact_bits are mutually exclusive");
+  ZS_REQUIRE(!p->dact_bits || ((((uintptr_t)p->dact_bits) & 3) == 0 && p->dact_bits_ld % 4 == 0 &&
+                               p->dact_bits_ld >= (p->unshuffle ? 2 : 1) * p->C / 8),
+             "zs_grad_combine: dact_bits needs a 4-byte aligned pointer and dact_bits_ld (%lld) a multiple of 4 that covers the row",
+             (long long)p->dact_bits_ld);
   ZS_NORM_LAUNCH(grad_combine_kernel, g_norm_lim2.get());
   return zs_check_launch("zs_grad_combine");
 }
diff --git a/zerospeech-tts-without-t_amd/engine.py b/zerospeech-tts-without-t_amd/engine.py
--- a/zerospeech-tts-without-t_amd/engine.py
+++ b/zerospeech-tts-without-t_amd/engine.py
@@ -3,7 +3,7 @@
 import torch
 
 from . import _lib as L
-from .layers import (Act, ConvLayer, GruLayer, cast_rows, colsum_ok, fork_side, grad_combine, instnorm_bwd, instnorm_fwd, join_side,
+from .layers import (Act, Bits, ConvLayer, GruLayer, cast_rows, colsum_ok, fork_side, grad_combine, instnorm_bwd, instnorm_fwd, join_side,
                      next_uid, pack_operands, rup, weight_operand)
 
 LRELU = L.ZS_ACT_LRELU
@@ -308,7 +308,13 @@
             l.wgrad(dcat.sub(i * self.c1, self.c1), xin)
 
 
+def _dact(y):
+    return 'dact_bits' if isinstance(y, Bits) else None
+
+
 class DecoderEngine(object):
+    sign_tape = True
+
     def __init__(self, ctx, P, G, c_in, c_out, c_h, c_a, ns, seg_len, output_mask=False):
         self.ctx = ctx
         self.uid = next_uid()
@@ -356,9 +362,11 @@
         self.input_emb.fwd(bits, out=x, out2=xe, vec2=emb[0], idx=cidx)
         T = T0
         for i, (la, lb) in enumerate(self.convs):
-            ya = c.act('d_ya%d' % i + tag, B, T, 2 * ch) if training else None
+            bits_a = training and self.sign_tape
+            ya = None if not training else (c.bits('d_ba%d' % i + tag, B * T, 2 * ch) if bits_a else c.act('d_ya%d' % i + tag, B, T, 2 * ch))
             s = c.act('d_s%d' % i + tag, B, 2 * T, ch)
-            la.fwd(xe, out=ya, act=LRELU, slope=ns, out2=s, vec2=emb[i], idx=cidx, store_mode2=L.ZS_STORE_SPLIT2, lengths=Ls[i])
+            la.fwd(xe, out=(None if bits_a else ya), sign_out=(ya if bits_a else None), act=LRELU, slope=ns, out2=s, vec2=emb[i],
+                   idx=cidx, store_mode2=L.ZS_STORE_SPLIT2, lengths=Ls[i])
             yb = c.act('d_yb%d' % i + tag, B, 2 * T, ch)
             lb.fwd(s, out=yb, act=LRELU, slope=ns, lengths=Ls[i + 1])
             xn = c.act('d_x%d' % (i + 1) + tag, B, 2 * T, ch)
@@ -376,9 +384,11 @@
         ed, er = self.e_dense, self.e_rnn
         cat3 = c.act('d_cat3' + tag, B, T, 3 * ch)
         for j, (la, lb) in enumerate(self.dense):
-            y1 = c.act('d_y1%d' % j + tag, B, T, ch)
+            bits_1 = training and self.sign_tape
+            y1 = c.bits('d_b1%d' % j + tag, B * T, ch) if bits_1 else c.act('d_y1%d' % j + tag, B, T, ch)
             y1e = c.act('d_y1e%d' % j + tag, B, T, ch)
-            la.fwd(xe, out=y1, act=LRELU, slope=ns, out2=y1e, vec2=emb[ed], idx=cidx)
+            la.fwd(xe, out=(None if bits_1 else y1), sign_out=(y1 if bits_1 else None), act=LRELU, slope=ns, out2=y1e, vec2=emb[ed],
+                   idx=cidx)
             y2 = c.act('d_y2%d' % j + tag, B, T, ch)
             lb.fwd(y1e, out=y2, act=LRELU, slope=ns)
             xn = c.act('d_dx%d' % j + tag, B, T, ch) if j == 0 else Act(cat3.t, B, T, ch, cat3.ld, 0, ch)
@@ -456,10 +466,10 @@
             lb.wgrad(dz2, y1e)
             dz1 = c.act('d_dz1%d' % j + tag, B, T, ch)
             if fuse:
-                lb.dgrad(dz2, T, dz1, dact_src=y1, slope=ns, colsum=slot(ed))
+                lb.dgrad(dz2, T, dz1, slope=ns, colsum=slot(ed), **{_dact(y1) or 'dact_src': y1})
             else:
                 lb.dgrad(dz2, T, gpv)
-                grad_combine(c, gpv, T, 0, 0, self.pad_mode, ch, dz1, ns, emb_sum=esum(ed), dact=y1)
+                grad_combine(c, gpv, T, 0, 0, self.pad_mode, ch, dz1, ns, emb_sum=esum(ed), **{_dact(y1) or 'dact': y1})
             la.wgrad(dz1, xe)
             dn = c.act('d_dxD%d' % j + tag, B, T, ch)
             if fuse:
@@ -485,7 +495,8 @@
             gp2 = Act(gp.t, B, T2 + 2, ch, gp.ld)
             lb.dgrad(dzb, T2, gp2)
             dza = c.act('d_dza%d' % i + tag, B, Ti, 2 * ch)
-            grad_combine(c, gp2, T2, 1, 1, self.pad_mode, ch, dza, ns, emb_sum=esum, dact=ya, unshuffle=1)
+            grad_combine(c, gp2, T2, 1, 1, self.pad_mode, ch, dza, ns, emb_sum=esum, unshuffle=1,
+                         **{_dact(ya) or 'dact': ya})
             la.wgrad(dza, xe)
             gp1 = Act(gp.t, B, Ti + 2, ch, gp.ld)
             la.dgrad(dza, Ti, gp1)
diff --git a/zerospeech-tts-without-t_amd/layers.py b/zerospeech-tts-without-t_amd/layers.py
--- a/zerospeech-tts-without-t_amd/layers.py
+++ b/zerospeech-tts-without-t_amd/layers.py
@@ -43,6 +43,35 @@
     def valid(self):
         base = self.t[self.off:self.off + (self.rows - 1) * self.ld + self.C]
         return torch.as_strided(base, (self.B, self.T, self.C), (self.T * self.ld, self.ld, 1))
+
+
+class Bits(object):
+    __slots__ = ('t', 'rows', 'cols', 'ld')
+
+    def __init__(self, t, rows, cols, ld):
+        self.t, self.rows, self.cols, self.ld = t, rows, cols, ld
+
+    def ptr(self):
+        return self.t.data_ptr()
+
+    def view2d(self):
+        return self.t[:self.rows * self.ld].view(self.rows, self.ld)
+
+
+def pack_sign_bits(pos, ld=None):
+    rows, cols = pos.shape
+    ld = ld if ld is not None else rup(cols // 8, 4)
+    w = (1 << torch.arange(8, device=pos.device, dtype=torch.int32))
+    by = (pos.reshape(rows, cols // 8, 8).to(torch.int32) * w).sum(-1).to(torch.uint8)
+    out = torch.zeros(rows, ld, dtype=torch.uint8, device=pos.device)
+    out[:, :cols // 8] = by
+    return out
+
+
+def unpack_sign_bits(bits, cols):
+    w = (1 << torch.arange(8, device=bits.device, dtype=torch.int32))
+    b = (bits[:, :cols // 8].to(torch.int32).unsqueeze(-1) & w) != 0
+    return b.reshape(bits.shape[0], cols)
 
 
 _SIDE = {}
@@ -168,6 +197,10 @@
 
     def f32(self, name, n):
         return self.raw(name, n, torch.float32)
+
+    def bits(self, name, rows, cols):
+        ld = rup(cols // 8, 4)
+        return Bits(self.raw(name, rows * ld, torch.uint8), rows, cols, ld)
 
     def workspace(self, nbytes):
         if self._ws is None or self._ws.numel() < nbytes:
@@ -284,7 +317,7 @@
         return (T_in + self.pad_l + self.pad_r - self.k) // self.stride + 1
 
     def fwd(self, A, out=None, act=L.ZS_ACT_NONE, slope=0.0, out_f32=False, out_cols=None, store_mode=L.ZS_STORE_ROWS,
-            out2=None, vec2=None, idx=None, store_mode2=L.ZS_STORE_ROWS, out2_cols=None, pre_vec=None, bias=True, lengths=None):
+            out2=None, vec2=None, idx=None, store_mode2=L.ZS_STORE_ROWS, out2_cols=None, pre_vec=None, bias=True, lengths=None, sign_out=None):
         c = self.ctx
         T_out = self.t_out(A.T)
         kw = dict(dtype=c.dt, A=A.ptr(), lda=A.ld, a_batch_stride=A.T * A.ld, B=A.B, T_in=A.T, T_out=T_out, taps=self.k,
@@ -303,15 +336,17 @@
                       out2_cols=out2_cols if out2_cols is not None else (min(out2.cols, rup(self.Cout, 32)) if store_mode2 == L.ZS_STORE_ROWS else self.Cout // 2))
             if vec2 is not None:
                 kw.update(vec2=L.ptr(vec2), vec2_ld=vec2.shape[1], vec_idx=L.ptr(idx))
+        if sign_out is not None:
+            kw.update(sign_out=sign_out.ptr(), sign_ld=sign_out.ld)
         L.call('zs_gemm_conv', 'ZsGemmConv', c.stream, **kw)
         return T_out
 
     def dgrad(self, dY, T_x, out, dact_src=None, slope=0.0, add_src=None, out_f32=False, add_f32=False, colsum=None, out_cols=None,
-              n_cols=None, n_off=0, colsum_post=False):
+              n_cols=None, n_off=0, colsum_post=False, dact_bits=None):
         c = self.ctx
         Tp = T_x + self.pad_l + self.pad_r
         if self.parity:
-            if dact_src is not None or add_src is not None or colsum is not None or n_cols is not None or n_off:
+            if dact_src is not None or dact_bits is not None or add_src is not None or colsum is not None or n_cols is not None or n_off:
                 raise ValueError('stride-2 dgrad: dact_src, add_src, colsum, n_cols and n_off are not supported')
             return self._dgrad_parity(dY, Tp, out, out_f32, out_cols)
         N, n_pad = self.Cin, self.n_pad_d
@@ -327,6 +362,8 @@
                   store_mode=L.ZS_STORE_ROWS, groups=1, out_f32=int(out_f32))
         if dact_src is not None:
             kw.update(dact_src=dact_src.ptr(), dact_ld=dact_src.ld)
+        if dact_bits is not None:
+            kw.update(dact_bits=dact_bits.ptr(), dact_bits_ld=dact_bits.ld)
         if add_src is not None:
             kw.update(add_src=add_src.ptr(), add_ld=add_src.ld, add_f32=int(add_f32))
         if colsum is not None:
@@ -525,13 +562,15 @@
 
 
 def grad_combine(ctx, gp, T, pad_l, pad_r, pad_mode, C, out, slope, res_mode=L.ZS_RES_NONE, res=None, dact=None, emb_sum=None,
-                 unshuffle=0):
+                 unshuffle=0, dact_bits=None):
     L.call('zs_grad_combine', 'ZsGradCombine', ctx.stream, dtype=ctx.dt, gp=gp.ptr(), ldg=gp.ld, pad_left=pad_l, pad_right=pad_r,
            pad_mode=pad_mode, B=gp.B, T=T, C=C, emb_sum=emb_sum, emb_ld=(C if emb_sum is not None else 0),
            emb_cols=(C if emb_sum is not None else 0), res_mode=res_mode, res=(res.ptr() if res is not None else None),
            ldres=(res.ld if res is not None else 0), dact_src=(dact.ptr() if dact is not None else None),
            dact_ld=(dact.ld if dact is not None else 0), slope=slope, out=(out.ptr() if out is not None else None),
-           ldo=(out.ld if out is not None else 0), unshuffle=unshuffle)
+           ldo=(out.ld if out is not None else 0), unshuffle=unshuffle,
+           dact_bits=(dact_bits.ptr() if dact_bits is not None else None),
+           dact_bits_ld=(dact_bits.ld if dact_bits is not None else 0))
 
 
 def cast_rows(ctx, src, ld_src, dst, dst_f32=False, dst2=None, col_off2=0, act2=L.ZS_ACT_NONE, slope2=0.0):
```

Result: slower. 3.024 million frames/s (-3.8%).
